# WPCLab/OpenSeg3D

Measured on AMD Instinct MI355X. Metric: points/sec fwd+bwd, Waymo 1-sweep ~180k pts @0.1m voxel; logit parity, higher is better.
Workload: dtype f32 storage/accumulate, bf16x3 products; 1 GPU; waymo_one_sweep (BASELINE configs[1]): synthetic scene, 174633 pts/step/GPU, voxel [0.1, 0.1, 0.1], grid [1440, 1440, 64], fwd (attention dropout p=0.1, DropPath) + criterion (ohem_ce+lovasz on 3 heads) + bwd + SGD step; mode=fwdbwd, segmentor=segformer, voxels=108690, parallelism=dp1

## Files before the change

### __graft_entry__.py

```python
import os
import subprocess
import sys

ROOT = os.path.dirname(os.path.abspath(__file__))
CSRC = os.path.join(ROOT, "openseg3d_amd", "csrc")
LIB = os.path.join(CSRC, "libseg3d_hip.so")
HIP_SOURCES = ["scan.hip", "voxelize.hip", "group.hip", "rulebook.hip", "spconv.hip", "spconv_split.hip", "linear_stream.hip", "linear_x6.hip", "spconv_dma.hip", "spconv_tile.hip", "wgrad_split.hip", "wgrad_dense.hip", "wgrad_dense_lds.hip", "window.hip",
               "attention.hip", "attention_fused.hip", "attention_fused_bwd.hip", "attention_small.hip", "rownorm.hip", "segment.hip", "knn.hip", "knn_attention.hip", "class_context.hip", "loss.hip", "lovasz.hip", "eval.hip"]
HIPCC_FLAGS = ["--offload-arch=gfx950", "-O3", "-std=c++17", "-fPIC", "-ffp-contract=off",
               "-fhip-fp32-correctly-rounded-divide-sqrt", "-Wall", "-Wno-unused-function"]


def _stale(target, deps):
    if not os.path.exists(target):
        return True
    t = os.path.getmtime(target)
    return any(os.path.getmtime(d) > t for d in deps)


def build_hip(force=False, verbose=False):
    hipcc = os.environ.get("HIPCC", "/opt/rocm/bin/hipcc")
    common = [os.path.join(CSRC, "common.hpp"), os.path.join(CSRC, "attn_common.hpp"), os.path.join(CSRC, "attn_dropout.hpp"), os.path.join(CSRC, "attn_fused.hpp"),
              os.path.join(ROOT, "include", "seg3d_hip.h")]
    objs = []
    procs = []
    for src in HIP_SOURCES:
        s = os.path.join(CSRC, src)
        o = os.path.join(CSRC, src.replace(".hip", ".o"))
        objs.append(o)
        if force or _stale(o, [s] + common):
            cmd = [hipcc] + HIPCC_FLAGS + ["-c", s, "-o", o]
            if verbose:
                print(" ".join(cmd))
            procs.append((src, subprocess.Popen(cmd, stdout=subprocess.PIPE, stderr=subprocess.STDOUT)))
    failed = False
    for src, p in procs:
        out, _ = p.communicate()
        if p.returncode != 0:
            failed = True
            sys.stderr.write(f"--- hipcc failed on {src}\n{out.decode()}\n")
        elif verbose and out.strip():
            print(out.decode())
    if failed:
        raise RuntimeError("hipcc failed")
    if force or procs or _stale(LIB, objs):
        subprocess.check_call([hipcc, "--offload-arch=gfx950", "-shared", "-fPIC", "-o", LIB] + objs)
    return LIB


def build():
    build_hip()
    subprocess.check_call(["make", "-C", os.path.join(ROOT, "oracle")], stdout=subprocess.DEVNULL)
    sys.path.insert(0, ROOT)
    import openseg3d_amd
    from openseg3d_amd import _lib
    _lib.load()


def smoke():
    sys.path.insert(0, ROOT)
    from openseg3d_amd import selfcheck
    selfcheck.run_smoke()


if __name__ == "__main__":
    build_hip(force="--force" in sys.argv, verbose=True)
```

### include/seg3d_hip.h

```cpp
#ifndef SEG3D_HIP_H
#define SEG3D_HIP_H

#include <stddef.h>
#include <stdint.h>

#ifdef __cplusplus
extern "C" {
#endif

#define SEG3D_OK 0
#define SEG3D_EINVAL (-1)
#define SEG3D_EWORKSPACE (-2)
#define SEG3D_ELAUNCH (-3)

#define SEG3D_REDUCE_SUM 0
#define SEG3D_REDUCE_MEAN 1
#define SEG3D_REDUCE_MAX 2

int seg3d_abi_version(void);

const char* seg3d_last_error(void);

int seg3d_grid_size(const float* voxel_size, const float* range, int32_t* grid_xyz);

size_t seg3d_voxelize_workspace_bytes(int64_t n_points);
int seg3d_voxelize_f32(const float* points, int64_t n_points, int32_t row_stride, int32_t xyz_col,
                       int32_t batch_col, const float* voxel_size, const float* range,
                       int32_t* voxel_coords, int32_t* point_voxel_ids, int32_t* n_voxels,
                       void* workspace, size_t workspace_bytes, void* stream);
int seg3d_voxelize_f64(const double* points, int64_t n_points, int32_t row_stride, int32_t xyz_col,
                       int32_t batch_col, const float* voxel_size, const float* range,
                       int32_t* voxel_coords, int32_t* point_voxel_ids, int32_t* n_voxels,
                       void* workspace, size_t workspace_bytes, void* stream);

size_t seg3d_voxelize_host_workspace_bytes(int64_t n_points);
int seg3d_voxelize_host_f32(const float* points, int64_t n_points, int32_t row_stride, int32_t xyz_col,
                            int32_t batch_col, const float* voxel_size, const float* range,
                            int32_t* voxel_coords, int32_t* point_voxel_ids, int32_t* n_voxels,
                            void* workspace, size_t workspace_bytes);
int seg3d_voxelize_host_f64(const double* points, int64_t n_points, int32_t row_stride, int32_t xyz_col,
                            int32_t batch_col, const float* voxel_size, const float* range,
                            int32_t* voxel_coords, int32_t* point_voxel_ids, int32_t* n_voxels,
                            void* workspace, size_t workspace_bytes);

int seg3d_cart2polar_f32(const float* points, int64_t n_points, int32_t row_stride, int32_t xyz_col,
                         float* out , void* stream);
int seg3d_cart2polar_f64(const double* points, int64_t n_points, int32_t row_stride, int32_t xyz_col,
                         double* out , void* stream);

size_t seg3d_group_index_workspace_bytes(int64_t n, int64_t n_groups);
int seg3d_group_index(const int32_t* group_ids, int64_t n, int64_t n_groups, int32_t* rank,
                      int32_t* order, int32_t* offsets, void* workspace, size_t workspace_bytes,
                      void* stream);

size_t seg3d_coord_hash_bytes(int64_t m);
int seg3d_coord_hash_build(const int32_t* coords, int64_t m, const int32_t* shape_zyx ,
                           void* table, size_t table_bytes, void* stream);
int seg3d_rulebook_subm(const int32_t* coords, int64_t m, const int32_t* shape_zyx ,
                        const void* table, size_t table_bytes, int32_t* nbr, void* stream);
size_t seg3d_downsample_workspace_bytes(int32_t batch_size, const int32_t* shape_in_zyx );
int seg3d_downsample_coords(const int32_t* coords_in, int64_t m_in,
                            const int32_t* m_in_dev ,
                            int32_t batch_size, const int32_t* shape_in_zyx , int32_t* coords_out,
                            int64_t cap_out, int32_t* m_out , void* workspace, size_t workspace_bytes,
                            void* stream);
int seg3d_rulebook_strided(const int32_t* coords_out, int64_t m_out, int64_t m_in,
                           const int32_t* shape_in_zyx , const void* table_in,
                           size_t table_bytes, int32_t* nbr_fwd, int32_t* nbr_inv, void* stream);

size_t seg3d_spconv_packed_bytes(int32_t cin, int32_t cout, int32_t flags);
int seg3d_spconv_pack_weight(const float* weight, int32_t cin, int32_t cout, int32_t flags,
                             void* w_packed, void* stream);
int seg3d_spconv_fwd(const float* x, const int32_t* nbr, int64_t m_out, int64_t m_in,
                     const void* w_packed, int32_t pack_flags, const float* bias ,
                     int32_t cin, int32_t cout, float* y,
                     const int32_t* row_order ,
                     void* stream);
int seg3d_spconv_fwd_act(const float* x, const int32_t* nbr, int64_t m_out, int64_t m_in, const void* w_packed,
                         int32_t pack_flags, const float* bias , const float* addend ,
                         int32_t relu, int32_t cin, int32_t cout, float* y, const int32_t* row_order ,
                         void* stream);
int seg3d_spconv_fwd_act_bf16(const void* x, int32_t x_bf16, const int32_t* nbr, int64_t m_out, int64_t m_in,
                              const void* w_packed, int32_t pack_flags, const float* bias,
                              const void* addend_bf16, int32_t relu, int32_t cin, int32_t cout, void* y_bf16,
                              const int32_t* row_order, void* stream);
size_t seg3d_spconv_presplit_bytes(int64_t m_in, int32_t cin);
int seg3d_spconv_presplit(const float* x, int64_t m_in, int32_t cin, void* xs, void* stream);
int seg3d_spconv_fwd_presplit(const void* xs, const int32_t* nbr, int64_t m_out, int64_t m_in, const void* w_packed,
                              int32_t pack_flags, const float* bias , const float* addend ,
                              int32_t relu, int32_t cin, int32_t cout, float* y,
                              const int32_t* row_order , void* stream);
size_t seg3d_conv_plan_bytes(int64_t m_out);
size_t seg3d_conv_plan_workspace_bytes(int64_t m_out);
int seg3d_conv_plan_build(const int32_t* coords, const int32_t* nbr, int64_t m_out, void* plan, void* workspace,
                          size_t workspace_bytes, void* stream);
int32_t seg3d_spconv_tiled_supported(int32_t cin, int32_t cout);
int seg3d_spconv_fwd_tiled(const float* x, const int32_t* nbr, const void* plan, int64_t m_out, int64_t m_in,
                           const void* w_packed, int32_t pack_flags, const float* bias ,
                           const float* addend , int32_t relu, int32_t cin, int32_t cout, float* y, void* stream);
int seg3d_spconv_fwd_tiled_bf16(const void* x, int32_t x_bf16, const int32_t* nbr, const void* plan, int64_t m_out,
                                int64_t m_in, const void* w_packed, int32_t pack_flags, const float* bias ,
                                const void* addend_bf16 , int32_t relu, int32_t cin, int32_t cout, void* y_bf16,
                                void* stream);
int seg3d_debug_set_conv_nbt(int32_t nbt);
int seg3d_debug_set_linear_stream(int32_t on);
size_t seg3d_spconv_wgrad_workspace_bytes(int64_t m_out, int32_t cin, int32_t cout);
int seg3d_spconv_wgrad(const float* x, const float* dy, const int32_t* nbr, int64_t m_out,
                       int64_t m_in, int32_t cin, int32_t cout, int32_t flags ,
                       float* dw, void* workspace, size_t workspace_bytes, void* stream);

int seg3d_spconv_wgrad_partials(const float* x, const float* dy, const int32_t* nbr, int64_t m_out, int64_t m_in,
                                int32_t cin, int32_t cout, void* workspace, size_t workspace_bytes, int32_t* chunks,
                                void* stream);
int seg3d_spconv_wgrad_partials_xbf16(const uint16_t* x_bf16, const float* dy, const int32_t* nbr, int64_t m_out,
                                      int64_t m_in, int32_t cin, int32_t cout, void* workspace, size_t workspace_bytes,
                                      int32_t* chunks, void* stream);

size_t seg3d_linear_wgrad_workspace_bytes(int64_t m, int32_t cin, int32_t cout);
int seg3d_linear_wgrad(const float* x, const float* dy, int64_t m, int32_t cin, int32_t cout, float* dw,
                       float* db , void* workspace, size_t workspace_bytes, void* stream);
int seg3d_linear_wgrad_partials(const float* x, const float* dy, int64_t m, int32_t cin, int32_t cout, int32_t with_bias,
                                void* workspace, size_t workspace_bytes, int32_t* chunks, void* stream);
int seg3d_linear_wgrad_partials_xbf16(const uint16_t* x_bf16, const float* dy, int64_t m, int32_t cin, int32_t cout,
                                      int32_t with_bias, void* workspace, size_t workspace_bytes, int32_t* chunks,
                                      void* stream);
int seg3d_debug_set_wgrad_lds(int32_t on);
int seg3d_reduce_partials(const float* part, int32_t chunks, int64_t n, int64_t nw, float* dw, float* db, void* stream);
int seg3d_reduce_partials_batched(const void* jobs, int32_t n_jobs, int64_t total_blocks, void* stream);
size_t seg3d_linear_packed_bytes_f32(int32_t cin, int32_t cout);
int seg3d_linear_pack_weight_f32(const float* weight, int32_t cin, int32_t cout, int32_t transpose,
                                 void* w_packed, void* stream);
int seg3d_linear_fwd_f32(const float* x, int64_t m, const void* w_packed, const float* bias ,
                         int32_t cin, int32_t cout, float* y, void* stream);
size_t seg3d_linear_packed_bytes_x6(int32_t cin, int32_t cout);
int seg3d_linear_pack_weight_x6(const float* weight, int32_t cin, int32_t cout, int32_t transpose, void* w_packed,
                                void* stream);
int seg3d_linear_fwd_x6(const float* x, int64_t m, const void* w_packed, const float* bias ,
                        const float* scale , const float* shift , int32_t relu, int32_t cin,
                        int32_t cout, float* y, void* stream);

typedef struct {
  const float* src;
  void* dst;
  int32_t cin, cout;
  int32_t kk, transpose, flip, reserved;
  int64_t first_block;
} seg3d_pack_job;
int seg3d_pack_weights_batched(const void* jobs, int32_t n_jobs, int64_t total_blocks, void* stream);

size_t seg3d_linear_packed_bytes(int32_t cin, int32_t cout, int32_t transpose);
int seg3d_linear_pack_weight(const float* weight, int32_t cin, int32_t cout, int32_t transpose,
                             void* w_packed, void* stream);
int seg3d_linear_fwd(const float* x, int64_t m, const void* w_packed, const float* bias ,
                     const float* addend , int32_t cin, int32_t cout,
                     float* y, void* stream);
int seg3d_linear_fwd_sum(const float* x, const float* x_add, int64_t m, const void* w_packed, const float* bias,
                         int32_t cin, int32_t cout, float* y, void* stream);
int seg3d_linear_layernorm_fwd(const float* x, int64_t m, const void* w_packed, const float* bias, const float* res,
                               const float* gamma, const float* beta, float eps, int32_t cin, int32_t cout, float* y,
                               void* stream);
int seg3d_linear_fwd_mul(const float* x, int64_t m, const void* w_packed, const float* factor, int32_t cin, int32_t cout,
                         float* y, void* stream);

size_t seg3d_window_partition_workspace_bytes(int64_t m, int32_t batch_size, const int32_t* nwin_xyz);
int seg3d_window_partition(const int32_t* coords, int64_t m, int32_t batch_size,
                           const int32_t* win_xyz, const int32_t* nwin_xyz, const int32_t* shift_xyz,
                           int32_t n_levels, const int32_t* level_lo, const int32_t* level_hi,
                           const int32_t* level_cap, int32_t* win_id, int32_t* in_win, int32_t* rank,
                           int32_t* level, int32_t* slot, int32_t* tok, int32_t* win_start,
                           int32_t* win_count, int32_t* win_tile0, int32_t* tile_item,
                           int32_t* qg_item, int32_t* counts, void* workspace,
                           size_t workspace_bytes, void* stream);

int seg3d_pos_embed(const int32_t* in_win, int64_t m, const int32_t* win_xyz ,
                    const float* inv_freq, int32_t c, float* pos, void* stream);

int seg3d_window_attn_supported(int32_t heads, int32_t dh);
size_t seg3d_window_attn_workspace_bytes(int64_t m, int32_t n_tiles, int32_t heads, int32_t dh);
int seg3d_window_attn_fwd(const float* q, const float* k, const float* v, int32_t ldq, int32_t ldk,
                          int32_t ldv, const int32_t* tok, const int32_t* win_start,
                          const int32_t* win_count, const int32_t* win_tile0,
                          const int32_t* tile_item, int32_t n_tiles, const int32_t* qg_item,
                          int32_t n_qgroups, int64_t m, int32_t n_windows, int32_t heads, int32_t dh,
                          const float* tau, float tau_min, float dropout_p, uint64_t dropout_seed, float* out,
                          float* lse, void* workspace, size_t workspace_bytes, void* stream);
int seg3d_window_attn_bwd(const float* q, const float* k, const float* v, int32_t ldq, int32_t ldk,
                          int32_t ldv, const float* out, const float* dout, const float* lse,
                          const int32_t* tok, const int32_t* win_start, const int32_t* win_count,
                          const int32_t* win_tile0, const int32_t* tile_item, int32_t n_tiles,
                          const int32_t* qg_item, int32_t n_qgroups, int64_t m, int32_t n_windows,
                          int32_t heads, int32_t dh, const float* tau,
                          float tau_min, float dropout_p, uint64_t dropout_seed, float* dq, float* dk,
                          float* dv, int32_t lddq, int32_t lddk,
                          int32_t lddv, float* dtau, void* workspace, size_t workspace_bytes,
                          void* stream);

int seg3d_layernorm_fwd(const float* x, const float* res, const float* gamma, const float* beta,
                        const float* rowscale, float eps, int64_t m, int32_t c, float* y, float* mean,
                        float* rstd, void* stream);
size_t seg3d_layernorm_bwd_workspace_bytes(int64_t m, int32_t c);
int seg3d_layernorm_bwd(const float* dy, const float* x, const float* mean, const float* rstd,
                        const float* gamma, const float* rowscale, int64_t m, int32_t c, float* dx,
                        float* dgamma, float* dbeta, void* workspace, size_t workspace_bytes, void* stream);
int seg3d_layernorm_bwd_partials(const float* dy, const float* x, const float* mean, const float* rstd,
                                 const float* gamma, const float* rowscale, int64_t m, int32_t c, float* dx,
                                 void* workspace, size_t workspace_bytes, int32_t* nblocks, void* stream);
size_t seg3d_batchnorm_workspace_bytes(int64_t m, int32_t c);
int seg3d_colstats(const float* x, int64_t m, int32_t c, float* sums, void* workspace, size_t workspace_bytes,
                   void* stream);
int seg3d_batchnorm_stats(const float* x, int64_t m, int32_t c, float eps, const float* gamma, const float* beta,
                          float momentum, float* running_mean, float* running_var, float* stats, void* workspace,
                          size_t workspace_bytes, void* stream);
int seg3d_gelu_fwd(const float* h, int64_t n, float* g, float* gp, void* stream);
int seg3d_affine_act(const float* x, const float* res, const float* scale, const float* shift, int32_t relu,
                     int64_t m, int32_t c, float* y, void* stream);
int seg3d_batchnorm_bwd(const float* dy, const float* y, const float* x, const float* mean, const float* rstd,
                        const float* gamma, int32_t relu, int64_t m, int32_t c, float* dx, float* dres,
                        float* sums, void* workspace, size_t workspace_bytes, void* stream);
int seg3d_batchnorm_bwd_reduce(const float* dy, const float* y, const float* x, const float* mean,
                               const float* rstd, int32_t relu, int64_t m, int32_t c, float* sums,
                               void* workspace, size_t workspace_bytes, void* stream);
int seg3d_batchnorm_bwd_apply(const float* dy, const float* y, const float* x, const float* mean,
                              const float* rstd, const float* gamma, const float* sums, const float* inv_count,
                              int32_t relu, int64_t m, int32_t c, float* dx, float* dres, void* stream);

int seg3d_segment_reduce_fwd(const float* x, int32_t c, const int32_t* order, const int32_t* offsets,
                             int64_t n_seg, int32_t mode, float* out, int32_t* argmax, void* stream);
int seg3d_segment_reduce_bwd(const float* dout, int32_t c, const int32_t* seg_of_row, int64_t n,
                             const int32_t* offsets, const int32_t* argmax, int64_t n_seg,
                             int32_t mode, float* dx, void* stream);

int seg3d_knn_attention_fwd(const float* q, const float* k, const float* v, const int32_t* idx,
                            const uint8_t* invalid, const float* keep, int64_t n, int64_t n_src,
                            int32_t n_neighbors, int32_t d, float scale, float* out, float* prob, void* stream);
int seg3d_knn_attention_bwd(const float* q, const float* k, const float* v, const int32_t* idx, const float* keep,
                            const float* prob, const float* dout, const int32_t* pair_order,
                            const int32_t* pair_offsets, int64_t n, int64_t n_src, int32_t n_neighbors, int32_t d,
                            float scale, float* dq, float* dk, float* dv, float* scratch, void* stream);

int seg3d_class_context_fwd(const float* feats, const float* probs, const int32_t* offsets, const int32_t* chunks,
                            const int32_t* chunk_offsets, int32_t n_chunks, int32_t batch, int64_t m,
                            int32_t classes, int32_t c, float scale, float* weights, float* partials, float* stats,
                            float* context, void* stream);
int seg3d_class_context_bwd(const float* feats, const float* weights, const float* dcontext,
                            const int32_t* offsets, const int32_t* chunks, const int32_t* chunk_offsets,
                            int32_t n_chunks, int32_t batch, int64_t m, int32_t classes, int32_t c, float scale,
                            float* dfeats, float* dprobs, float* scratch, void* stream);

int seg3d_gather_rows(const float* feats, const int32_t* ids, int64_t n, int32_t c, float* out,
                      void* stream);

int seg3d_knn_query(const float* xyz, int64_t n, const float* new_xyz, int64_t m, const int32_t* offset,
                    const int32_t* new_offset, int32_t batch_size, int32_t k, int32_t* idx, float* dist2,
                    void* stream);

size_t seg3d_knn_level_workspace_bytes(int64_t n);
int seg3d_knn_level_build(const float* xyz, int64_t n, const int32_t* offset, int32_t batch_size, float cell,
                          float* sorted_xyz, int32_t* src_index, int32_t* cell_end, void* table_keys, int32_t* table_vals,
                          int64_t capacity, void* workspace, size_t workspace_bytes, void* stream);
int seg3d_knn_query_order(const float* new_xyz, int64_t m, const int32_t* new_offset, int32_t batch_size, float cell,
                          int32_t* order, void* workspace, size_t workspace_bytes, void* stream);
int seg3d_parity_order(const int32_t* coords, int64_t m, int32_t* order, void* workspace, size_t workspace_bytes,
                       void* stream);
typedef struct {
  const float* sorted_xyz;
  const int32_t* src_index;
  const int32_t* cell_end;
  const void* table_keys;
  const int32_t* table_vals;
  int64_t capacity;
// ... 52 lines not shown
```

### openseg3d_amd/_lib.py

```python
import ctypes
import os
import re

_HERE = os.path.dirname(os.path.abspath(__file__))
LIB_PATH = os.path.join(_HERE, "csrc", "libseg3d_hip.so")
HEADER_PATH = os.path.join(os.path.dirname(_HERE), "include", "seg3d_hip.h")

OK, EINVAL, EWORKSPACE, ELAUNCH = 0, -1, -2, -3
REDUCE_SUM, REDUCE_MEAN, REDUCE_MAX = 0, 1, 2
ABI_VERSION = 41

_p, _i32, _i64, _sz, _f = ctypes.c_void_p, ctypes.c_int32, ctypes.c_int64, ctypes.c_size_t, ctypes.c_float
_u64 = ctypes.c_uint64

SIGNATURES = {
    "seg3d_abi_version": (ctypes.c_int, []),
    "seg3d_last_error": (ctypes.c_char_p, []),
    "seg3d_grid_size": (ctypes.c_int, [_p, _p, _p]),
    "seg3d_voxelize_workspace_bytes": (_sz, [_i64]),
    "seg3d_voxelize_f32": (ctypes.c_int, [_p, _i64, _i32, _i32, _i32, _p, _p, _p, _p, _p, _p, _sz, _p]),
    "seg3d_voxelize_f64": (ctypes.c_int, [_p, _i64, _i32, _i32, _i32, _p, _p, _p, _p, _p, _p, _sz, _p]),
    "seg3d_voxelize_host_workspace_bytes": (_sz, [_i64]),
    "seg3d_voxelize_host_f32": (ctypes.c_int, [_p, _i64, _i32, _i32, _i32, _p, _p, _p, _p, _p, _p, _sz]),
    "seg3d_voxelize_host_f64": (ctypes.c_int, [_p, _i64, _i32, _i32, _i32, _p, _p, _p, _p, _p, _p, _sz]),
    "seg3d_cart2polar_f32": (ctypes.c_int, [_p, _i64, _i32, _i32, _p, _p]),
    "seg3d_cart2polar_f64": (ctypes.c_int, [_p, _i64, _i32, _i32, _p, _p]),
    "seg3d_group_index_workspace_bytes": (_sz, [_i64, _i64]),
    "seg3d_group_index": (ctypes.c_int, [_p, _i64, _i64, _p, _p, _p, _p, _sz, _p]),
    "seg3d_coord_hash_bytes": (_sz, [_i64]),
    "seg3d_coord_hash_build": (ctypes.c_int, [_p, _i64, _p, _p, _sz, _p]),
    "seg3d_rulebook_subm": (ctypes.c_int, [_p, _i64, _p, _p, _sz, _p, _p]),
    "seg3d_downsample_workspace_bytes": (_sz, [_i32, _p]),
    "seg3d_downsample_coords": (ctypes.c_int, [_p, _i64, _p, _i32, _p, _p, _i64, _p, _p, _sz, _p]),
    "seg3d_rulebook_strided": (ctypes.c_int, [_p, _i64, _i64, _p, _p, _sz, _p, _p, _p]),
    "seg3d_spconv_packed_bytes": (_sz, [_i32, _i32, _i32]),
    "seg3d_spconv_pack_weight": (ctypes.c_int, [_p, _i32, _i32, _i32, _p, _p]),
    "seg3d_spconv_fwd": (ctypes.c_int, [_p, _p, _i64, _i64, _p, _i32, _p, _i32, _i32, _p, _p, _p]),
    "seg3d_spconv_fwd_act": (ctypes.c_int, [_p, _p, _i64, _i64, _p, _i32, _p, _p, _i32, _i32, _i32, _p, _p, _p]),
    "seg3d_spconv_fwd_act_bf16": (ctypes.c_int, [_p, _i32, _p, _i64, _i64, _p, _i32, _p, _p, _i32, _i32, _i32, _p, _p, _p]),
    "seg3d_spconv_presplit_bytes": (_sz, [_i64, _i32]),
    "seg3d_spconv_presplit": (ctypes.c_int, [_p, _i64, _i32, _p, _p]),
    "seg3d_spconv_fwd_presplit": (ctypes.c_int, [_p, _p, _i64, _i64, _p, _i32, _p, _p, _i32, _i32, _i32, _p, _p, _p]),
    "seg3d_conv_plan_bytes": (_sz, [_i64]),
    "seg3d_conv_plan_workspace_bytes": (_sz, [_i64]),
    "seg3d_conv_plan_build": (ctypes.c_int, [_p, _p, _i64, _p, _p, _sz, _p]),
    "seg3d_spconv_tiled_supported": (_i32, [_i32, _i32]),
    "seg3d_spconv_fwd_tiled": (ctypes.c_int, [_p, _p, _p, _i64, _i64, _p, _i32, _p, _p, _i32, _i32, _i32, _p, _p]),
    "seg3d_spconv_fwd_tiled_bf16": (ctypes.c_int, [_p, _i32, _p, _p, _i64, _i64, _p, _i32, _p, _p, _i32, _i32, _i32, _p, _p]),
    "seg3d_debug_set_conv_nbt": (ctypes.c_int, [_i32]),
    "seg3d_debug_set_linear_stream": (ctypes.c_int, [_i32]),
    "seg3d_spconv_wgrad_workspace_bytes": (_sz, [_i64, _i32, _i32]),
    "seg3d_spconv_wgrad": (ctypes.c_int, [_p, _p, _p, _i64, _i64, _i32, _i32, _i32, _p, _p, _sz, _p]),
    "seg3d_spconv_wgrad_partials": (ctypes.c_int, [_p, _p, _p, _i64, _i64, _i32, _i32, _p, _sz, _p, _p]),
    "seg3d_spconv_wgrad_partials_xbf16": (ctypes.c_int, [_p, _p, _p, _i64, _i64, _i32, _i32, _p, _sz, _p, _p]),
    "seg3d_linear_wgrad_partials_xbf16": (ctypes.c_int, [_p, _p, _i64, _i32, _i32, _i32, _p, ctypes.c_size_t, _p, _p]),
    "seg3d_linear_packed_bytes_f32": (ctypes.c_size_t, [_i32, _i32]),
    "seg3d_linear_pack_weight_f32": (ctypes.c_int, [_p, _i32, _i32, _i32, _p, _p]),
    "seg3d_linear_fwd_f32": (ctypes.c_int, [_p, _i64, _p, _p, _i32, _i32, _p, _p]),
    "seg3d_debug_set_wgrad_lds": (ctypes.c_int, [_i32]),
    "seg3d_linear_packed_bytes_x6": (ctypes.c_size_t, [_i32, _i32]),
    "seg3d_linear_pack_weight_x6": (ctypes.c_int, [_p, _i32, _i32, _i32, _p, _p]),
    "seg3d_linear_fwd_x6": (ctypes.c_int, [_p, _i64, _p, _p, _p, _p, _i32, _i32, _i32, _p, _p]),
    "seg3d_pack_weights_batched": (ctypes.c_int, [_p, _i32, _i64, _p]),
    "seg3d_linear_wgrad_workspace_bytes": (ctypes.c_size_t, [_i64, _i32, _i32]),
    "seg3d_linear_wgrad": (ctypes.c_int, [_p, _p, _i64, _i32, _i32, _p, _p, _p, ctypes.c_size_t, _p]),
    "seg3d_linear_wgrad_partials": (ctypes.c_int, [_p, _p, _i64, _i32, _i32, _i32, _p, ctypes.c_size_t, _p, _p]),
    "seg3d_reduce_partials": (ctypes.c_int, [_p, _i32, _i64, _i64, _p, _p, _p]),
    "seg3d_reduce_partials_batched": (ctypes.c_int, [_p, _i32, _i64, _p]),
    "seg3d_linear_packed_bytes": (_sz, [_i32, _i32, _i32]),
    "seg3d_linear_pack_weight": (ctypes.c_int, [_p, _i32, _i32, _i32, _p, _p]),
    "seg3d_linear_fwd": (ctypes.c_int, [_p, _i64, _p, _p, _p, _i32, _i32, _p, _p]),
    "seg3d_linear_fwd_sum": (ctypes.c_int, [_p, _p, _i64, _p, _p, _i32, _i32, _p, _p]),
    "seg3d_linear_fwd_mul": (ctypes.c_int, [_p, _i64, _p, _p, _i32, _i32, _p, _p]),
    "seg3d_linear_layernorm_fwd": (ctypes.c_int, [_p, _i64, _p, _p, _p, _p, _p, ctypes.c_float, _i32, _i32, _p, _p]),
    "seg3d_window_partition_workspace_bytes": (_sz, [_i64, _i32, _p]),
    "seg3d_window_partition": (ctypes.c_int, [_p, _i64, _i32, _p, _p, _p, _i32, _p, _p, _p,
                                              _p, _p, _p, _p, _p, _p, _p, _p, _p, _p, _p, _p, _p, _sz, _p]),
    "seg3d_pos_embed": (ctypes.c_int, [_p, _i64, _p, _p, _i32, _p, _p]),
    "seg3d_window_attn_supported": (ctypes.c_int, [_i32, _i32]),
    "seg3d_window_attn_workspace_bytes": (_sz, [_i64, _i32, _i32, _i32]),
    "seg3d_window_attn_fwd": (ctypes.c_int, [_p, _p, _p, _i32, _i32, _i32, _p, _p, _p, _p, _p, _i32, _p, _i32,
                                             _i64, _i32, _i32, _i32, _p, _f, _f, _u64, _p, _p, _p, _sz, _p]),
    "seg3d_window_attn_bwd": (ctypes.c_int, [_p, _p, _p, _i32, _i32, _i32, _p, _p, _p, _p, _p, _p, _p, _p, _i32, _p,
                                             _i32, _i64, _i32, _i32, _i32, _p, _f, _f, _u64, _p, _p, _p, _i32, _i32, _i32,
                                             _p, _p, _sz, _p]),
    "seg3d_layernorm_fwd": (ctypes.c_int, [_p, _p, _p, _p, _p, _f, _i64, _i32, _p, _p, _p, _p]),
    "seg3d_layernorm_bwd_workspace_bytes": (ctypes.c_size_t, [_i64, _i32]),
    "seg3d_layernorm_bwd": (ctypes.c_int, [_p, _p, _p, _p, _p, _p, _i64, _i32, _p, _p, _p, _p, ctypes.c_size_t, _p]),
    "seg3d_layernorm_bwd_partials": (ctypes.c_int, [_p, _p, _p, _p, _p, _p, _i64, _i32, _p, _p, ctypes.c_size_t, _p, _p]),
    "seg3d_batchnorm_workspace_bytes": (ctypes.c_size_t, [_i64, _i32]),
    "seg3d_colstats": (ctypes.c_int, [_p, _i64, _i32, _p, _p, ctypes.c_size_t, _p]),
    "seg3d_batchnorm_stats": (ctypes.c_int, [_p, _i64, _i32, _f, _p, _p, _f, _p, _p, _p, _p, ctypes.c_size_t, _p]),
    "seg3d_affine_act": (ctypes.c_int, [_p, _p, _p, _p, _i32, _i64, _i32, _p, _p]),
    "seg3d_gelu_fwd": (ctypes.c_int, [_p, _i64, _p, _p, _p]),
    "seg3d_batchnorm_bwd": (ctypes.c_int, [_p, _p, _p, _p, _p, _p, _i32, _i64, _i32, _p, _p, _p, _p, ctypes.c_size_t, _p]),
    "seg3d_batchnorm_bwd_reduce": (ctypes.c_int, [_p, _p, _p, _p, _p, _i32, _i64, _i32, _p, _p, ctypes.c_size_t, _p]),
    "seg3d_batchnorm_bwd_apply": (ctypes.c_int, [_p, _p, _p, _p, _p, _p, _p, _p, _i32, _i64, _i32, _p, _p, _p]),
    "seg3d_segment_reduce_fwd": (ctypes.c_int, [_p, _i32, _p, _p, _i64, _i32, _p, _p, _p]),
    "seg3d_segment_reduce_bwd": (ctypes.c_int, [_p, _i32, _p, _i64, _p, _p, _i64, _i32, _p, _p]),
    "seg3d_voxel_majority_labels": (ctypes.c_int, [_p, _p, _p, _i64, _i32, _p, _p]),
    "seg3d_cross_entropy_workspace_bytes": (ctypes.c_size_t, [_i64]),
    "seg3d_cross_entropy_fwd": (ctypes.c_int, [_p, _p, _i64, _i32, _i64, _f, _p, _p, _p, ctypes.c_size_t, _p]),
    "seg3d_cross_entropy_bwd": (ctypes.c_int, [_p, _p, _p, _p, _p, _i64, _i32, _p, _p]),
    "seg3d_lovasz_workspace_bytes": (ctypes.c_size_t, [_i64, _i32]),
    "seg3d_lovasz_softmax_fwd": (ctypes.c_int, [_p, _p, _i64, _i32, _i64, _i32, _p, _p, _p, _p, _p, ctypes.c_size_t, _p]),
    "seg3d_lovasz_softmax_bwd": (ctypes.c_int, [_p, _p, _p, _p, _i64, _i32, _p, _p]),
    "seg3d_knn_level_workspace_bytes": (ctypes.c_size_t, [_i64]),
    "seg3d_knn_level_build": (ctypes.c_int, [_p, _i64, _p, _i32, _f, _p, _p, _p, _p, _p, _i64, _p, ctypes.c_size_t, _p]),
    "seg3d_parity_order": (ctypes.c_int, [_p, _i64, _p, _p, ctypes.c_size_t, _p]),
    "seg3d_knn_query_order": (ctypes.c_int, [_p, _i64, _p, _i32, _f, _p, _p, ctypes.c_size_t, _p]),
    "seg3d_knn_grid_query": (ctypes.c_int, [_p, _i32, _p, _p, _i64, _p, _p, _i32, _i32, _p, _p, _p]),
    "seg3d_knn_query": (ctypes.c_int, [_p, _i64, _p, _i64, _p, _p, _i32, _i32, _p, _p, _p]),
    "seg3d_gather_rows": (ctypes.c_int, [_p, _p, _i64, _i32, _p, _p]),
    "seg3d_class_context_fwd": (ctypes.c_int, [_p, _p, _p, _p, _p, _i32, _i32, _i64, _i32, _i32, _f, _p, _p, _p, _p, _p]),
    "seg3d_class_context_bwd": (ctypes.c_int, [_p, _p, _p, _p, _p, _p, _i32, _i32, _i64, _i32, _i32, _f, _p, _p, _p, _p]),
    "seg3d_knn_attention_fwd": (ctypes.c_int, [_p, _p, _p, _p, _p, _p, _i64, _i64, _i32, _i32, _f, _p, _p, _p]),
    "seg3d_knn_attention_bwd": (ctypes.c_int, [_p, _p, _p, _p, _p, _p, _p, _p, _p, _i64, _i64, _i32, _i32, _f, _p, _p, _p, _p, _p]),
    "seg3d_tta_views_f32": (ctypes.c_int, [_p, _i64, _i32, _p, _p, _p]),
    "seg3d_tta_views_host_f32": (ctypes.c_int, [_p, _i64, _i32, _p, _p]),
    "seg3d_softmax_accumulate_f32": (ctypes.c_int, [_p, _i64, _i32, _i32, _i32, _p, _p]),
    "seg3d_argmax_confusion": (ctypes.c_int, [_p, _p, _i64, _i32, _i32, _p, _i32, _p, _p, _p]),
}

_ERR = {EINVAL: "SEG3D_EINVAL (bad argument)", EWORKSPACE: "SEG3D_EWORKSPACE (workspace too small)",
        ELAUNCH: "SEG3D_ELAUNCH (HIP launch/runtime error)"}

_lib = None


class Seg3dError(RuntimeError):
    pass


def header_symbols():
    with open(HEADER_PATH) as f:
        text = f.read()
    text = re.sub(r"/\*.*?\*/", "", text, flags=re.S)
    return sorted(set(re.findall(r"\b(seg3d_[a-z0-9_]+)\s*\(", text)))


def load():
    global _lib
    if _lib is not None:
        return _lib
    if not os.path.exists(LIB_PATH):
        raise Seg3dError(
            f"{LIB_PATH} not found: the HIP library is required (no CPU fallback). "
            "Build it with `python __graft_entry__.py`.")
    import torch
    lib = ctypes.CDLL(LIB_PATH)
    for name, (res, args) in SIGNATURES.items():
        fn = getattr(lib, name)
        fn.restype = res
        fn.argtypes = args
    if lib.seg3d_abi_version() != ABI_VERSION:
        raise Seg3dError(f"libseg3d_hip.so ABI {lib.seg3d_abi_version()} != binding {ABI_VERSION}")
    _lib = lib
    return lib


def call(name, *args):
    lib = load()
    rc = getattr(lib, name)(*args)
    if rc != OK:
        detail = ""
        if rc == ELAUNCH:
            text = lib.seg3d_last_error()
            detail = f": {text.decode(errors='replace')}" if text else ""
        raise Seg3dError(f"{name} failed: {_ERR.get(rc, rc)}{detail}")


def query(name, *args):
    return int(getattr(load(), name)(*args))
```

### openseg3d_amd/csrc/spconv.hip

```cpp
#include "common.hpp"

size_t spconv_split_packed_bytes(int cin_op, int cout_op, int kk);
int spconv_split_pack(const float* weight, int cin, int cout, int kk, int transpose, int flip, void* w_packed,
                      hipStream_t st);
int spconv_split_fwd_io(const void* x, const int32_t* nbr, int64_t m_out, const void* wp, const float* bias,
                        const void* addend, const int32_t* row_order, int cin, int cout, void* y, int relu, int io,
                        hipStream_t st, const float* x_add);
int spconv_split_fwd(const float* x, const int32_t* nbr, int64_t m_out, const void* wp, const float* bias,
                     const float* addend, const int32_t* row_order, int cin, int cout, float* y, int relu, hipStream_t st);
size_t wgrad_split_sparse_workspace_bytes(int64_t m_out, int cin, int cout);
int wgrad_split_sparse(const void* x, const float* dy, const int32_t* nbr, int64_t m_out, int cin, int cout, float* dw,
                       void* workspace, size_t workspace_bytes, hipStream_t st, int32_t* chunks_out, bool x_bf16);

namespace {

typedef float f32x4 __attribute__((ext_vector_type(4)));

constexpr int kWaves = 4;
constexpr int kThreads = kWaves * 64;
constexpr int kRowsPerWave = 16;
constexpr int kRowsPerBlock = kWaves * kRowsPerWave;

__global__ __launch_bounds__(256) void pack_weight(const float* __restrict__ w, int cin_src, int cout_src, int kk,
                                                   int transpose, int flip, float* __restrict__ wp) {
    const int64_t total = (int64_t)kk * cin_src * cout_src;
    const int64_t t = (int64_t)blockIdx.x * 256 + threadIdx.x;
    if (t >= total) return;
    const int cin_op = transpose ? cout_src : cin_src;
    const int cout_op = transpose ? cin_src : cout_src;
    const int cb_n = cin_op / 16, nb_n = cout_op / 16;
    int64_t r = t;
    const int j = (int)(r & 3); r >>= 2;
    const int lane = (int)(r & 63); r >>= 6;
    const int nb = (int)(r % nb_n); r /= nb_n;
    const int cb = (int)(r % cb_n); r /= cb_n;
    const int kp = (int)r;
    const int ci_op = cb * 16 + (lane >> 4) * 4 + j;
    const int co_op = nb * 16 + (lane & 15);
    const int k = flip ? kk - 1 - kp : kp;
    const int ci = transpose ? co_op : ci_op;
    const int co = transpose ? ci_op : co_op;
    wp[t] = w[((int64_t)co * kk + k) * cin_src + ci];
}

template <int NBT, bool DENSE>
__global__ __launch_bounds__(kThreads) void spconv_fwd_kernel(const float* __restrict__ x, const int32_t* __restrict__ nbr,
                                                              int64_t m_out, const float* __restrict__ wp,
                                                              const float* __restrict__ bias, int cin, int cout,
                                                              float* __restrict__ y) {
    const int lane = threadIdx.x & 63;
    const int wave = threadIdx.x >> 6;
    const int64_t row0 = (int64_t)blockIdx.x * kRowsPerBlock + wave * kRowsPerWave;
    if (row0 >= m_out) return;
    const int nb0 = blockIdx.y * NBT;
    const int cb_n = cin >> 4, nb_n = cout >> 4;
    const int64_t my_row = row0 + (lane & 15);
    const bool row_ok = my_row < m_out;
    const int64_t my_row_c = row_ok ? my_row : m_out - 1;

    f32x4 acc[NBT];
#pragma unroll
    for (int n = 0; n < NBT; ++n) {
        const float b = bias ? bias[(nb0 + n) * 16 + (lane & 15)] : 0.0f;
        acc[n] = (f32x4){b, b, b, b};
    }

    for (int k = 0; k < (DENSE ? 1 : 27); ++k) {
        const int32_t raw = DENSE ? (int32_t)my_row_c : nbr[(int64_t)k * m_out + my_row_c];
        const int32_t idx = row_ok ? raw : -1;
        if (__ballot(idx >= 0) == 0ull) continue;
        const float* xrow = x + (int64_t)(idx >= 0 ? idx : 0) * cin + (lane >> 4) * 4;
        const float* wk = wp + ((int64_t)k * cb_n * nb_n + nb0) * 256 + lane * 4;
        for (int cb = 0; cb < cb_n; ++cb) {
            const f32x4 ld = *reinterpret_cast<const f32x4*>(xrow + cb * 16);
            const f32x4 a = idx >= 0 ? ld : (f32x4){0.f, 0.f, 0.f, 0.f};
            f32x4 b[NBT];
#pragma unroll
            for (int n = 0; n < NBT; ++n)
                b[n] = *reinterpret_cast<const f32x4*>(wk + ((int64_t)cb * nb_n + n) * 256);
#pragma unroll
            for (int j = 0; j < 4; ++j) {
#pragma unroll
                for (int n = 0; n < NBT; ++n)
                    acc[n] = __builtin_amdgcn_mfma_f32_16x16x4f32(a[j], b[n][j], acc[n], 0, 0, 0);
            }
        }
    }

#pragma unroll
    for (int r = 0; r < 4; ++r) {
        const int64_t orow = row0 + (lane >> 4) * 4 + r;
        if (orow < m_out) {
            float* yr = y + orow * cout + nb0 * 16 + (lane & 15);
#pragma unroll
            for (int n = 0; n < NBT; ++n) yr[n * 16] = acc[n][r];
        }
    }
}

template <int NBT>
int launch_fwd(const float* x, const int32_t* nbr, int64_t m_out, const float* wp, const float* bias, int cin, int cout,
               float* y, hipStream_t st) {
    dim3 grid((unsigned)ceil_div64(m_out, kRowsPerBlock), (unsigned)((cout / 16) / NBT));
    if (nbr == nullptr)
        hipLaunchKernelGGL((spconv_fwd_kernel<NBT, true>), grid, dim3(kThreads), 0, st, x, nbr, m_out, wp, bias, cin, cout, y);
    else
        hipLaunchKernelGGL((spconv_fwd_kernel<NBT, false>), grid, dim3(kThreads), 0, st, x, nbr, m_out, wp, bias, cin, cout, y);
    SEG3D_CHECK_LAUNCH();
    return SEG3D_OK;
}

template <int J>
struct VecLoad;
template <>
struct VecLoad<1> {
    static __device__ __forceinline__ void load(const float* p, float* v) { v[0] = p[0]; }
};
template <>
struct VecLoad<2> {
    static __device__ __forceinline__ void load(const float* p, float* v) {
        const float2 t = *reinterpret_cast<const float2*>(p);
        v[0] = t.x; v[1] = t.y;
    }
};
template <>
struct VecLoad<3> {
    static __device__ __forceinline__ void load(const float* p, float* v) { v[0] = p[0]; v[1] = p[1]; v[2] = p[2]; }
};
template <>
struct VecLoad<4> {
    static __device__ __forceinline__ void load(const float* p, float* v) {
        const float4 t = *reinterpret_cast<const float4*>(p);
        v[0] = t.x; v[1] = t.y; v[2] = t.z; v[3] = t.w;
    }
};

constexpr int kWgradRowsPerWave = 512;

template <int JA, int JB>
__global__ __launch_bounds__(kThreads) void spconv_wgrad_kernel(const float* __restrict__ x, const float* __restrict__ dy,
                                                                const int32_t* __restrict__ nbr, int64_t m_out, int cin,
                                                                int cout, float* __restrict__ dw) {
    __shared__ int32_t pair_row[kWaves][64];
    __shared__ int32_t pair_in[kWaves][64];
    __shared__ float stage[kWaves][16 * JB * (16 * JA + 1)];
    const int lane = threadIdx.x & 63;
    const int wave = threadIdx.x >> 6;
    const int k = blockIdx.y;
    const int ca_n = cin / (16 * JA);
    const int ca = blockIdx.z % ca_n, cbk = blockIdx.z / ca_n;
    const int ci0 = ca * 16 * JA, co0 = cbk * 16 * JB;
    const int64_t r_begin = ((int64_t)blockIdx.x * kWaves + wave) * kWgradRowsPerWave;
    if (r_begin >= m_out) return;
    const int64_t r_end = r_begin + kWgradRowsPerWave < m_out ? r_begin + kWgradRowsPerWave : m_out;

    f32x4 acc[JA][JB];
#pragma unroll
    for (int a = 0; a < JA; ++a)
#pragma unroll
        for (int b = 0; b < JB; ++b) acc[a][b] = (f32x4){0.f, 0.f, 0.f, 0.f};

    const int32_t* nk = nbr + (int64_t)k * m_out;
    for (int64_t r0 = r_begin; r0 < r_end; r0 += 64) {
        const int64_t r = r0 + lane;
        const int32_t idx = r < r_end ? nk[r] : -1;
// ... 57 lines not shown

template <int JA, int JB>
int launch_wgrad(const float* x, const float* dy, const int32_t* nbr, int64_t m_out, int cin, int cout, float* dw,
                 hipStream_t st) {
    dim3 grid((unsigned)ceil_div64(m_out, (int64_t)kWaves * kWgradRowsPerWave), 27,
              (unsigned)((cin / (16 * JA)) * (cout / (16 * JB))));
    hipLaunchKernelGGL((spconv_wgrad_kernel<JA, JB>), grid, dim3(kThreads), 0, st, x, dy, nbr, m_out, cin, cout, dw);
    SEG3D_CHECK_LAUNCH();
    return SEG3D_OK;
}

template <int JA>
int launch_wgrad_b(int jb, const float* x, const float* dy, const int32_t* nbr, int64_t m_out, int cin, int cout,
                   float* dw, hipStream_t st) {
    switch (jb) {
        case 4: return launch_wgrad<JA, 4>(x, dy, nbr, m_out, cin, cout, dw, st);
        case 3: return launch_wgrad<JA, 3>(x, dy, nbr, m_out, cin, cout, dw, st);
        case 2: return launch_wgrad<JA, 2>(x, dy, nbr, m_out, cin, cout, dw, st);
        default: return launch_wgrad<JA, 1>(x, dy, nbr, m_out, cin, cout, dw, st);
    }
}

int dispatch_fwd_f32(const float* x, const int32_t* nbr, int64_t m_out, const float* w_packed, const float* bias, int cin,
                     int cout, float* y, hipStream_t st) {
    const int nb = cout / 16;
    if (nb % 12 == 0) return launch_fwd<12>(x, nbr, m_out, w_packed, bias, cin, cout, y, st);
    if (nb % 8 == 0) return launch_fwd<8>(x, nbr, m_out, w_packed, bias, cin, cout, y, st);
    if (nb % 6 == 0) return launch_fwd<6>(x, nbr, m_out, w_packed, bias, cin, cout, y, st);
    if (nb % 4 == 0) return launch_fwd<4>(x, nbr, m_out, w_packed, bias, cin, cout, y, st);
    if (nb % 3 == 0) return launch_fwd<3>(x, nbr, m_out, w_packed, bias, cin, cout, y, st);
    if (nb % 2 == 0) return launch_fwd<2>(x, nbr, m_out, w_packed, bias, cin, cout, y, st);
    return launch_fwd<1>(x, nbr, m_out, w_packed, bias, cin, cout, y, st);
}

}

extern "C" {

size_t seg3d_spconv_packed_bytes(int32_t cin, int32_t cout, int32_t flags) {
    if (cin <= 0 || cout <= 0) return 0;
    const int cin_op = (flags & 1) ? cout : cin, cout_op = (flags & 1) ? cin : cout;
    if (flags & 4) return spconv_split_packed_bytes(cin_op, cout_op, 27);
    return (size_t)27 * cin * cout * sizeof(float);
}

int seg3d_spconv_pack_weight(const float* weight, int32_t cin, int32_t cout, int32_t flags, void* w_packed,
                             void* stream) {
    if (!weight || !w_packed || cin <= 0 || cout <= 0 || (cin & 15) || (cout & 15)) return SEG3D_EINVAL;
    hipStream_t st = as_stream(stream);
    if (flags & 4) return spconv_split_pack(weight, cin, cout, 27, flags & 1, (flags >> 1) & 1, w_packed, st);
    const int64_t total = (int64_t)27 * cin * cout;
    hipLaunchKernelGGL(pack_weight, dim3((unsigned)ceil_div64(total, 256)), dim3(256), 0, st, weight, cin, cout, 27,
                       flags & 1, (flags >> 1) & 1, static_cast<float*>(w_packed));
    SEG3D_CHECK_LAUNCH();
    return SEG3D_OK;
}

int seg3d_spconv_fwd(const float* x, const int32_t* nbr, int64_t m_out, int64_t m_in, const void* w_packed_v,
                     int32_t pack_flags, const float* bias, int32_t cin, int32_t cout, float* y, const int32_t* row_order,
                     void* stream) {
    if (m_out < 0 || m_in < 0 || cin <= 0 || cout <= 0 || (cin & 15) || (cout & 15) || !w_packed_v) return SEG3D_EINVAL;
    if (m_out == 0) return SEG3D_OK;
    if (!x || !nbr || !y) return SEG3D_EINVAL;
    hipStream_t st = as_stream(stream);
    if (pack_flags & 4) return spconv_split_fwd(x, nbr, m_out, w_packed_v, bias, nullptr, row_order, cin, cout, y, 0, st);
    return dispatch_fwd_f32(x, nbr, m_out, static_cast<const float*>(w_packed_v), bias, cin, cout, y, st);
}

int seg3d_spconv_fwd_act(const float* x, const int32_t* nbr, int64_t m_out, int64_t m_in, const void* w_packed_v,
                         int32_t pack_flags, const float* bias, const float* addend, int32_t relu, int32_t cin,
                         int32_t cout, float* y, const int32_t* row_order, void* stream) {
    if (m_out < 0 || m_in < 0 || cin <= 0 || cout <= 0 || (cin & 15) || (cout & 15) || !w_packed_v || !(pack_flags & 4))
        return SEG3D_EINVAL;
    if (m_out == 0) return SEG3D_OK;
    if (!x || !nbr || !y) return SEG3D_EINVAL;
    return spconv_split_fwd(x, nbr, m_out, w_packed_v, bias, addend, row_order, cin, cout, y, relu ? 1 : 0, as_stream(stream));
}

int seg3d_spconv_fwd_act_bf16(const void* x, int32_t x_bf16, const int32_t* nbr, int64_t m_out, int64_t m_in,
                              const void* w_packed_v, int32_t pack_flags, const float* bias, const void* addend_bf16,
                              int32_t relu, int32_t cin, int32_t cout, void* y_bf16, const int32_t* row_order,
                              void* stream) {
    if (m_out < 0 || m_in < 0 || cin <= 0 || cout <= 0 || (cin & 15) || (cout & 15) || !w_packed_v || !(pack_flags & 4))
        return SEG3D_EINVAL;
    if (m_out == 0) return SEG3D_OK;
    if (!x || !nbr || !y_bf16) return SEG3D_EINVAL;
    return spconv_split_fwd_io(x, nbr, m_out, w_packed_v, bias, addend_bf16, row_order, cin, cout, y_bf16, relu ? 1 : 0,
                               x_bf16 ? 2 : 1, as_stream(stream), nullptr);
}

size_t seg3d_linear_packed_bytes_f32(int32_t cin, int32_t cout) {
    return cin > 0 && cout > 0 ? (size_t)cin * cout * sizeof(float) : 0;
}

int seg3d_linear_pack_weight_f32(const float* weight, int32_t cin, int32_t cout, int32_t transpose, void* w_packed,
                                 void* stream) {
    if (!weight || !w_packed || cin <= 0 || cout <= 0 || (cin & 15) || (cout & 15)) return SEG3D_EINVAL;
    const int64_t total = (int64_t)cin * cout;
    hipLaunchKernelGGL(pack_weight, dim3((unsigned)ceil_div64(total, 256)), dim3(256), 0, as_stream(stream), weight, cin,
                       cout, 1, transpose ? 1 : 0, 0, static_cast<float*>(w_packed));
    SEG3D_CHECK_LAUNCH();
    return SEG3D_OK;
}

int seg3d_linear_fwd_f32(const float* x, int64_t m, const void* w_packed, const float* bias, int32_t cin, int32_t cout,
                         float* y, void* stream) {
    if (m < 0 || cin <= 0 || cout <= 0 || (cin & 15) || (cout & 15) || !w_packed) return SEG3D_EINVAL;
    if (m == 0) return SEG3D_OK;
    if (!x || !y) return SEG3D_EINVAL;
    return dispatch_fwd_f32(x, nullptr, m, static_cast<const float*>(w_packed), bias, cin, cout, y, as_stream(stream));
}

size_t seg3d_spconv_wgrad_workspace_bytes(int64_t m_out, int32_t cin, int32_t cout) {
    if (m_out < 0 || cin <= 0 || cout <= 0) return 0;
    return wgrad_split_sparse_workspace_bytes(m_out, cin, cout);
}

int seg3d_spconv_wgrad(const float* x, const float* dy, const int32_t* nbr, int64_t m_out, int64_t m_in, int32_t cin,
                       int32_t cout, int32_t flags, float* dw, void* workspace, size_t workspace_bytes, void* stream) {
    if (m_out < 0 || m_in < 0 || cin <= 0 || cout <= 0 || (cin & 15) || (cout & 15) || !dw) return SEG3D_EINVAL;
    hipStream_t st = as_stream(stream);
    if (m_out > 0 && (!x || !dy || !nbr)) return SEG3D_EINVAL;
    if (m_out > 0 && (flags & 4)) return wgrad_split_sparse(x, dy, nbr, m_out, cin, cout, dw, workspace, workspace_bytes, st, nullptr, false);
    SEG3D_CHECK_HIP(hipMemsetAsync(dw, 0, (size_t)27 * cin * cout * sizeof(float), st));
    if (m_out == 0) return SEG3D_OK;
    const int ja = pick_j(cin), jb = pick_j(cout);
    switch (ja) {
        case 4: return launch_wgrad_b<4>(jb, x, dy, nbr, m_out, cin, cout, dw, st);
        case 3: return launch_wgrad_b<3>(jb, x, dy, nbr, m_out, cin, cout, dw, st);
        case 2: return launch_wgrad_b<2>(jb, x, dy, nbr, m_out, cin, cout, dw, st);
        default: return launch_wgrad_b<1>(jb, x, dy, nbr, m_out, cin, cout, dw, st);
    }
}

int seg3d_spconv_wgrad_partials(const float* x, const float* dy, const int32_t* nbr, int64_t m_out, int64_t m_in, int32_t cin,
                                int32_t cout, void* workspace, size_t workspace_bytes, int32_t* chunks, void* stream) {
    if (m_out < 0 || m_in < 0 || cin <= 0 || cout <= 0 || (cin & 15) || (cout & 15) || !chunks) return SEG3D_EINVAL;
    *chunks = 0;
    if (m_out == 0) return SEG3D_OK;
    if (!x || !dy || !nbr) return SEG3D_EINVAL;
    return wgrad_split_sparse(x, dy, nbr, m_out, cin, cout, nullptr, workspace, workspace_bytes, as_stream(stream), chunks, false);
}

int seg3d_spconv_wgrad_partials_xbf16(const uint16_t* x_bf16, const float* dy, const int32_t* nbr, int64_t m_out, int64_t m_in,
                                      int32_t cin, int32_t cout, void* workspace, size_t workspace_bytes, int32_t* chunks,
                                      void* stream) {
    if (m_out < 0 || m_in < 0 || cin <= 0 || cout <= 0 || (cin & 15) || (cout & 15) || !chunks) return SEG3D_EINVAL;
    *chunks = 0;
    if (m_out == 0) return SEG3D_OK;
    if (!x_bf16 || !dy || !nbr) return SEG3D_EINVAL;
    return wgrad_split_sparse(x_bf16, dy, nbr, m_out, cin, cout, nullptr, workspace, workspace_bytes, as_stream(stream), chunks, true);
}

}
```

### openseg3d_amd/csrc/voxelize.hip

```cpp
#include <cstdio>

#include "common.hpp"

namespace {

constexpr int kThreads = 256;

struct VoxParams {
    int32_t grid[3];
    int32_t row_stride, xyz_col, batch_col;
};

template <typename T>
struct VoxConst {
    T lo[3];
    T vs[3];
};

__device__ __forceinline__ float floor_t(float v) { return floorf(v); }
__device__ __forceinline__ double floor_t(double v) { return floor(v); }

template <typename T>
__global__ __launch_bounds__(kThreads) void vox_insert(const T* __restrict__ pts, int64_t n, VoxParams p,
                                                       VoxConst<T> c, HashView h, uint32_t* __restrict__ slot_of) {
// ... 97 lines not shown
                  int32_t* n_voxels, void* workspace, size_t workspace_bytes, void* stream) {
    if (n < 0 || n >= (int64_t)0x7F000000 || !voxel_size || !range || !voxel_coords || !n_voxels || !workspace ||
        row_stride < 3 || xyz_col < 0 || xyz_col + 3 > row_stride || batch_col >= row_stride)
        return SEG3D_EINVAL;
    if (n > 0 && (!points || !point_voxel_ids)) return SEG3D_EINVAL;
    if (workspace_bytes < ws_bytes(n)) return SEG3D_EWORKSPACE;
    hipStream_t st = as_stream(stream);
    VoxParams p;
    if (seg3d_grid_size(voxel_size, range, p.grid) != SEG3D_OK) return SEG3D_EINVAL;
    p.row_stride = row_stride;
    p.xyz_col = xyz_col;
    p.batch_col = batch_col;
    VoxConst<T> c;
    for (int j = 0; j < 3; ++j) {
        c.lo[j] = (T)range[j];
        c.vs[j] = (T)voxel_size[j];
    }
    VoxWs w = carve(workspace, n);
    HashView h = hash_view(w.table, w.cap);
    SEG3D_CHECK_HIP(hipMemsetAsync(h.keys, 0xFF, w.cap * 8, st));
    SEG3D_CHECK_HIP(hipMemsetAsync(h.vals, 0x7F, w.cap * 4, st));
    if (n == 0) {
        SEG3D_CHECK_HIP(hipMemsetAsync(n_voxels, 0, 4, st));
        return SEG3D_OK;
    }
    const unsigned nb = (unsigned)ceil_div64(n, kThreads);
    hipLaunchKernelGGL(vox_insert<T>, dim3(nb), dim3(kThreads), 0, st, points, n, p, c, h, w.slot_of);
    SEG3D_CHECK_LAUNCH();
    hipLaunchKernelGGL(vox_flag, dim3(nb), dim3(kThreads), 0, st, w.slot_of, n, h, w.flag);
    SEG3D_CHECK_LAUNCH();
    int rc = scan_exclusive_u32(w.flag, w.rank, n, reinterpret_cast<uint32_t*>(n_voxels), w.tmp, st);
    if (rc != SEG3D_OK) return rc;
    hipLaunchKernelGGL(vox_emit, dim3(nb), dim3(kThreads), 0, st, w.slot_of, w.rank, n, h, p, voxel_coords,
                       point_voxel_ids);
    SEG3D_CHECK_LAUNCH();
    return SEG3D_OK;
}

__device__ __forceinline__ float atan2_t(float y, float x) { return (float)atan2((double)y, (double)x); }
__device__ __forceinline__ double atan2_t(double y, double x) { return atan2(y, x); }
__device__ __forceinline__ float sqrt_t(float v) { return sqrtf(v); }
__device__ __forceinline__ double sqrt_t(double v) { return sqrt(v); }

template <typename T>
__global__ __launch_bounds__(kThreads) void cart2polar_rows(const T* __restrict__ pts, int64_t n, int row_stride, int xyz_col,
                                                            T* __restrict__ out) {
    const int64_t i = (int64_t)blockIdx.x * kThreads + threadIdx.x;
    if (i >= n) return;
    const T* row = pts + i * row_stride;
    T* o = out + i * (row_stride + 2);
    for (int j = 0; j < xyz_col; ++j) o[j] = row[j];
    const T x = row[xyz_col], y = row[xyz_col + 1], z = row[xyz_col + 2];
    o[xyz_col] = sqrt_t(x * x + y * y);
    o[xyz_col + 1] = atan2_t(y, x);
    o[xyz_col + 2] = z;
    o[xyz_col + 3] = x;
    o[xyz_col + 4] = y;
    for (int j = xyz_col + 3; j < row_stride; ++j) o[j + 2] = row[j];
}

template <typename T>
int cart2polar_impl(const T* points, int64_t n, int32_t row_stride, int32_t xyz_col, T* out, void* stream) {
    if (n < 0 || row_stride < 3 || xyz_col < 0 || xyz_col + 3 > row_stride) return SEG3D_EINVAL;
    if (n == 0) return SEG3D_OK;
    if (!points || !out) return SEG3D_EINVAL;
    hipLaunchKernelGGL(cart2polar_rows<T>, dim3((unsigned)ceil_div64(n, kThreads)), dim3(kThreads), 0, as_stream(stream), points, n,
                       row_stride, xyz_col, out);
    SEG3D_CHECK_LAUNCH();
    return SEG3D_OK;
}


inline float floor_h(float v) { return __builtin_floorf(v); }
inline double floor_h(double v) { return __builtin_floor(v); }

inline uint64_t host_capacity(int64_t n) {
    uint64_t cap = 64;
    while (cap < (uint64_t)(2 * n + 2)) cap <<= 1;
    return cap;
}

template <typename T>
int voxelize_host_impl(const T* points, int64_t n, int32_t row_stride, int32_t xyz_col, int32_t batch_col,
                       const float* voxel_size, const float* range, int32_t* voxel_coords, int32_t* point_voxel_ids,
                       int32_t* n_voxels, void* workspace, size_t workspace_bytes) {
    if (n < 0 || n >= (int64_t)0x7F000000 || !voxel_size || !range || !n_voxels || row_stride < 3 || xyz_col < 0 ||
        xyz_col + 3 > row_stride || batch_col >= row_stride)
        return SEG3D_EINVAL;
    if (n > 0 && (!points || !point_voxel_ids || !voxel_coords || !workspace)) return SEG3D_EINVAL;
    const uint64_t cap = host_capacity(n);
    if (n > 0 && workspace_bytes < cap * 12) return SEG3D_EWORKSPACE;
    int32_t grid[3];
    if (seg3d_grid_size(voxel_size, range, grid) != SEG3D_OK) return SEG3D_EINVAL;
    *n_voxels = 0;
    if (n == 0) return SEG3D_OK;
    uint64_t* keys = static_cast<uint64_t*>(workspace);
    int32_t* vals = reinterpret_cast<int32_t*>(keys + cap);
    for (uint64_t s = 0; s < cap; ++s) keys[s] = ~0ull;
    T lo[3], vs[3];
    for (int j = 0; j < 3; ++j) {
        lo[j] = (T)range[j];
        vs[j] = (T)voxel_size[j];
    }
    int32_t count = 0;
    for (int64_t i = 0; i < n; ++i) {
        const T* row = points + i * row_stride;
        int32_t cc[3];
        bool ok = true;
        for (int j = 0; j < 3 && ok; ++j) {
            volatile T d = row[xyz_col + j] - lo[j];
            volatile T q = d / vs[j];
            const T v = floor_h((T)q);
            if (!(v >= (T)0) || v >= (T)grid[j]) ok = false;
            else cc[j] = (int32_t)v;
        }
        if (!ok) {
            point_voxel_ids[i] = -1;
            continue;
        }
        const int64_t b = batch_col >= 0 ? (int64_t)row[batch_col] : 0;
        const uint64_t key = (uint64_t)(((b * grid[2] + cc[2]) * grid[1] + cc[1]) * (int64_t)grid[0] + cc[0]);
        uint64_t h = key * 0x9E3779B97F4A7C15ull;
        uint64_t s = (h ^ (h >> 29)) & (cap - 1);
        while (keys[s] != key && keys[s] != ~0ull) s = (s + 1) & (cap - 1);
        if (keys[s] == ~0ull) {
            keys[s] = key;
            vals[s] = count;
            int32_t* o = voxel_coords + 4 * (int64_t)count;
            o[0] = (int32_t)b;
            o[1] = cc[2];
            o[2] = cc[1];
            o[3] = cc[0];
            ++count;
        }
        point_voxel_ids[i] = vals[s];
    }
    *n_voxels = count;
    return SEG3D_OK;
}

}

extern "C" {

int seg3d_cart2polar_f32(const float* points, int64_t n_points, int32_t row_stride, int32_t xyz_col, float* out, void* stream) {
    return cart2polar_impl<float>(points, n_points, row_stride, xyz_col, out, stream);
}

int seg3d_cart2polar_f64(const double* points, int64_t n_points, int32_t row_stride, int32_t xyz_col, double* out,
                         void* stream) {
    return cart2polar_impl<double>(points, n_points, row_stride, xyz_col, out, stream);
}

int seg3d_abi_version(void) { return 41; }

namespace {
thread_local char g_last_error[320] = "";
}

const char* seg3d_last_error(void) { return g_last_error; }

int seg3d_grid_size(const float* voxel_size, const float* range, int32_t* grid_xyz) {
    if (!voxel_size || !range || !grid_xyz) return SEG3D_EINVAL;
    for (int j = 0; j < 3; ++j) {
        volatile float span = range[3 + j] - range[j];
        volatile float g = span / voxel_size[j];
        grid_xyz[j] = (int32_t)__builtin_rintf(g);
        if (grid_xyz[j] <= 0) return SEG3D_EINVAL;
    }
    return SEG3D_OK;
}

size_t seg3d_voxelize_workspace_bytes(int64_t n_points) { return ws_bytes(n_points < 0 ? 0 : n_points); }

int seg3d_voxelize_f32(const float* points, int64_t n_points, int32_t row_stride, int32_t xyz_col, int32_t batch_col,
                       const float* voxel_size, const float* range, int32_t* voxel_coords, int32_t* point_voxel_ids,
                       int32_t* n_voxels, void* workspace, size_t workspace_bytes, void* stream) {
    return voxelize_impl<float>(points, n_points, row_stride, xyz_col, batch_col, voxel_size, range, voxel_coords,
                                point_voxel_ids, n_voxels, workspace, workspace_bytes, stream);
}

int seg3d_voxelize_f64(const double* points, int64_t n_points, int32_t row_stride, int32_t xyz_col, int32_t batch_col,
                       const float* voxel_size, const float* range, int32_t* voxel_coords, int32_t* point_voxel_ids,
                       int32_t* n_voxels, void* workspace, size_t workspace_bytes, void* stream) {
    return voxelize_impl<double>(points, n_points, row_stride, xyz_col, batch_col, voxel_size, range, voxel_coords,
                                 point_voxel_ids, n_voxels, workspace, workspace_bytes, stream);
}

size_t seg3d_voxelize_host_workspace_bytes(int64_t n_points) { return (size_t)host_capacity(n_points < 0 ? 0 : n_points) * 12; }

int seg3d_voxelize_host_f32(const float* points, int64_t n_points, int32_t row_stride, int32_t xyz_col, int32_t batch_col,
                            const float* voxel_size, const float* range, int32_t* voxel_coords, int32_t* point_voxel_ids,
                            int32_t* n_voxels, void* workspace, size_t workspace_bytes) {
    return voxelize_host_impl<float>(points, n_points, row_stride, xyz_col, batch_col, voxel_size, range, voxel_coords,
                                     point_voxel_ids, n_voxels, workspace, workspace_bytes);
}

int seg3d_voxelize_host_f64(const double* points, int64_t n_points, int32_t row_stride, int32_t xyz_col, int32_t batch_col,
                            const float* voxel_size, const float* range, int32_t* voxel_coords, int32_t* point_voxel_ids,
                            int32_t* n_voxels, void* workspace, size_t workspace_bytes) {
    return voxelize_host_impl<double>(points, n_points, row_stride, xyz_col, batch_col, voxel_size, range, voxel_coords,
                                      point_voxel_ids, n_voxels, workspace, workspace_bytes);
}

}

void seg3d_note_hip_error(int code, const char* file, int line) {
    const char* base = file;
    for (const char* p = file; *p; ++p)
        if (*p == '/') base = p + 1;
    snprintf(g_last_error, sizeof(g_last_error), "%s (%s) at %s:%d", hipGetErrorString((hipError_t)code),
             hipGetErrorName((hipError_t)code), base, line);
}
```

### openseg3d_amd/csrc/wgrad_split.hip

```cpp
#include <cstdlib>

#include "attn_common.hpp"

int wgrad_chunk_reduce(const float* part, int chunks, int64_t n, int64_t nw, float* dw, float* db, hipStream_t st);

#ifdef SEG3D_WGRAD_STAMP
__device__ unsigned long long* g_wgrad_stamp_buf = nullptr;
extern "C" int seg3d_debug_wgrad_stamps(void* buf) {
    unsigned long long* p = static_cast<unsigned long long*>(buf);
    return hipMemcpyToSymbol(HIP_SYMBOL(g_wgrad_stamp_buf), &p, sizeof(p)) == hipSuccess ? 0 : 2;
}
#define WSTAMP(i)                                                    \
    do {                                                             \
        __builtin_amdgcn_sched_barrier(0);                           \
        const unsigned long long t_ = __builtin_amdgcn_s_memtime();  \
        __builtin_amdgcn_sched_barrier(0);                           \
        st_acc[i] += t_ - st_last;                                   \
        st_last = t_;                                                \
    } while (0)
#else
#define WSTAMP(i) do {} while (0)
#endif

namespace {

using namespace attn;

constexpr int kWaves = 4;
constexpr int kThreads = 64 * kWaves;
constexpr int kRing = 128;

__device__ __forceinline__ bf16x8 frag_from_bf16_rows(const uint2* q, int comp) {
    u32x4 h;
#pragma unroll
    for (int j = 0; j < 4; ++j) {
        const uint32_t a = (comp & 2) ? q[2 * j].y : q[2 * j].x, b = (comp & 2) ? q[2 * j + 1].y : q[2 * j + 1].x;
        h[j] = (comp & 1) ? ((a >> 16) | (b & 0xFFFF0000u)) : ((a & 0xFFFFu) | (b << 16));
    }
    return __builtin_bit_cast(bf16x8, h);
}

__device__ __forceinline__ f32x4 mfma2(const bf16x8& a_hi, const bf16x8& a_lo, const bf16x8& b, f32x4 acc) {
    acc = __builtin_amdgcn_mfma_f32_16x16x32_bf16(a_lo, b, acc, 0, 0, 0);
    acc = __builtin_amdgcn_mfma_f32_16x16x32_bf16(a_hi, b, acc, 0, 0, 0);
    return acc;
}

struct Plan {
    int nbo, nbi;
    int chunks;
    int64_t rows;
};

__device__ __forceinline__ void unit_to_chunk_offset(int unit, int n_chunks, int* chunk, int* k) {
    if (unit < n_chunks) {
        *chunk = unit;
        *k = 13;
    } else {
        const int u = unit - n_chunks;
        const int kk = u % 26;
        *chunk = u / 26;
        *k = kk + (kk >= 13 ? 1 : 0);
    }
}

Plan plan(int64_t m, int cin, int cout) {
    Plan p{(cout + 63) / 64, (cin + 63) / 64, 0, 64};
    if (m <= 0) return p;
    const int tiles = p.nbo * p.nbi;
    static const int rows_target = [] {
        const char* e = getenv("SEG3D_WGRAD_SPARSE_ROWS");
        const int v = e ? atoi(e) : 3072;
        return v >= 64 ? v : 3072;
    }();
    int64_t chunks = m / rows_target;
    const int64_t need = (1024 + 27 * tiles - 1) / (27 * tiles);
    if (chunks < need) chunks = need;
    if (chunks < 1) chunks = 1;
    int64_t rows = (m + chunks - 1) / chunks;
    rows = (rows + 63) / 64 * 64;
    p.rows = rows;
    p.chunks = (int)((m + rows - 1) / rows);
    return p;
}

template <bool XB>
__global__ __launch_bounds__(kThreads, 2) void wgrad_sparse_kernel(const void* __restrict__ x_v, const float* __restrict__ dy,
                                                                    const int32_t* __restrict__ nbr, int64_t m_rows,
                                                                    int cin, int cout, int rows_per_chunk, int nbi,
                                                                    int tiles, int units, float* __restrict__ part,
                                                                    int center_first) {
    const float* x = static_cast<const float*>(x_v);
    __shared__ __attribute__((aligned(16))) float red[64 * 64];
    __shared__ int2 ring[kWaves][kRing];
    const int lane = threadIdx.x & 63, wave = threadIdx.x >> 6;
    const int cq = lane & 15, rg = lane >> 4;
    const int xcd = blockIdx.x & 7, j = blockIdx.x >> 3;
    const int xb = (center_first >> 8) > 0 ? (center_first >> 8) : 1;
    const int qs = j / tiles, tile = j % tiles;
    const int unit = ((qs / xb) * 8 + xcd) * xb + qs % xb;
    if (unit >= units) return;
    int chunk = unit / 27, k = unit % 27;
    if (center_first & 1) unit_to_chunk_offset(unit, units / 27, &chunk, &k);
    const int bi = tile % nbi, bo = tile / nbi;
    const int ci0 = bi * 64, co0 = bo * 64;
    const int64_t r_begin = (int64_t)chunk * rows_per_chunk;
    const int64_t r_end = r_begin + rows_per_chunk < m_rows ? r_begin + rows_per_chunk : m_rows;
    const int32_t* nk = nbr + (int64_t)k * m_rows;
    const float* px = x + (ci0 + 4 * cq < cin ? ci0 + 4 * cq : 0);
    const uint16_t* pxb = static_cast<const uint16_t*>(x_v) + (ci0 + 4 * cq < cin ? ci0 + 4 * cq : 0);
    const float* py = dy + (co0 + 4 * cq < cout ? co0 + 4 * cq : 0);
    int2* my = ring[wave];

    f32x4 acc[4][4];
#pragma unroll
    for (int a = 0; a < 4; ++a)
#pragma unroll
        for (int b = 0; b < 4; ++b) acc[a][b] = (f32x4){0.f, 0.f, 0.f, 0.f};

    constexpr int kAhead = 4;
    int head = 0, tail = 0;
    int64_t g_row = r_begin + 64 * (int64_t)wave;
    int32_t idxq[kAhead];
#pragma unroll
    for (int j = 0; j < kAhead; ++j) {
        const int64_t r = g_row + (int64_t)j * 64 * kWaves + lane;
        idxq[j] = r < r_end ? nk[r] : -1;
    }
    auto scan_group = [&]() {
        const int32_t idx = idxq[0];
        const int64_t row = g_row + lane;
        g_row += 64 * kWaves;
#pragma unroll
        for (int j = 0; j + 1 < kAhead; ++j) idxq[j] = idxq[j + 1];
        const int64_t rn = g_row + (int64_t)(kAhead - 1) * 64 * kWaves + lane;
        idxq[kAhead - 1] = rn < r_end ? nk[rn] : -1;
        const unsigned long long mask = __ballot(idx >= 0);
        if (idx >= 0) {
            const int p = tail + __popcll(mask & ((1ull << lane) - 1ull));
            my[p & (kRing - 1)] = make_int2(idx, (int)row);
        }
        tail += __popcll(mask);
    };
    auto refill = [&]() {
        while (tail - head < 32 && g_row < r_end) scan_group();
        __builtin_amdgcn_wave_barrier();
    };

    f32x4 xr[XB ? 1 : 8], yr[8];
    uint2 xq[XB ? 8 : 1];
    bf16x8 b_hi[4], b_lo[XB ? 1 : 4];
    auto load_x = [&](int h0, int valid) {
#pragma unroll
        for (int i = 0; i < 8; ++i) {
            const int e = 8 * rg + i;
            const int2 p = my[(h0 + (e < valid ? e : 0)) & (kRing - 1)];
            if constexpr (XB) xq[i] = *reinterpret_cast<const uint2*>(pxb + (int64_t)p.x * cin);
            else xr[i] = *reinterpret_cast<const f32x4*>(px + (int64_t)p.x * cin);
        }
        if (valid < 32) {
#pragma unroll
            for (int i = 0; i < 8; ++i)
                if (8 * rg + i >= valid) {
                    if constexpr (XB) xq[i] = make_uint2(0u, 0u);
                    else xr[i] = (f32x4){0.f, 0.f, 0.f, 0.f};
                }
        }
    };
    auto load_y = [&](int h0, int valid) {
#pragma unroll
        for (int i = 0; i < 8; ++i) {
            const int e = 8 * rg + i;
            const int2 p = my[(h0 + (e < valid ? e : 0)) & (kRing - 1)];
            yr[i] = *reinterpret_cast<const f32x4*>(py + (int64_t)p.y * cout);
        }
        if (valid < 32) {
#pragma unroll
            for (int i = 0; i < 8; ++i)
                if (8 * rg + i >= valid) yr[i] = (f32x4){0.f, 0.f, 0.f, 0.f};
        }
    };
    auto make_b = [&]() {
#pragma unroll
        for (int b = 0; b < 4; ++b) {
            if constexpr (XB) {
                b_hi[b] = frag_from_bf16_rows(xq, b);
            } else {
                float v[8];
#pragma unroll
                for (int i = 0; i < 8; ++i) v[i] = xr[i][b];
                split_frag(v, &b_hi[b], &b_lo[b]);
            }
        }
    };
    auto multiply = [&]() {
#pragma unroll
        for (int a = 0; a < 4; ++a) {
            float v[8];
#pragma unroll
            for (int i = 0; i < 8; ++i) v[i] = yr[i][a];
            bf16x8 a_hi, a_lo;
            split_frag(v, &a_hi, &a_lo);
#pragma unroll
            for (int b = 0; b < 4; ++b) {
                if constexpr (XB) acc[a][b] = mfma2(a_hi, a_lo, b_hi[b], acc[a][b]);
                else acc[a][b] = mfma3(a_hi, a_lo, b_hi[b], b_lo[b], acc[a][b]);
            }
        }
    };

    refill();
    int valid = tail - head < 32 ? tail - head : 32;
    if (valid > 0) {
        load_x(head, valid);
        load_y(head, valid);
    }
    while (valid > 0) {
        head += valid;
        refill();
        const int next = tail - head < 32 ? tail - head : 32;
        make_b();
        if (next > 0) load_x(head, next);
        multiply();
        if (next > 0) load_y(head, next);
        valid = next;
    }

    for (int w = 0; w < kWaves; ++w) {
        if (wave == w) {
#pragma unroll
            for (int a = 0; a < 4; ++a)
#pragma unroll
                for (int r = 0; r < 4; ++r) {
                    f32x4* slot = reinterpret_cast<f32x4*>(&red[(4 * (4 * rg + r) + a) * 64 + 4 * cq]);
                    f32x4 v = {acc[a][0][r], acc[a][1][r], acc[a][2][r], acc[a][3][r]};
                    if (w > 0) v += *slot;
                    *slot = v;
                }
        }
        __syncthreads();
    }
    float* pw = part + (int64_t)chunk * ((int64_t)cout * 27 * cin);
    for (int e = threadIdx.x; e < 64 * 16; e += kThreads) {
        const int row = e >> 4, q = e & 15;
        const int co = co0 + row, ci = ci0 + 4 * q;
        if (co < cout && ci < cin)
            *reinterpret_cast<f32x4*>(pw + ((int64_t)co * 27 + k) * cin + ci) =
                *reinterpret_cast<const f32x4*>(&red[row * 64 + 4 * q]);
    }
}

constexpr int kRing2 = 512;

template <bool XB, int DEPTH, bool SB = false>
__global__ __launch_bounds__(kThreads, SB ? 3 : 2) void wgrad_sparse_wide_kernel(const void* __restrict__ x_v, const float* __restrict__ dy,
                                                                         const int32_t* __restrict__ nbr, int64_t m_rows,
                                                                         int cin, int cout, int rows_per_chunk, int nbi,
                                                                         int tiles, int units, float* __restrict__ part,
                                                                         int center_first) {
    const float* x = static_cast<const float*>(x_v);
    __shared__ __attribute__((aligned(16))) uint4 img[SB ? 1 : 2][4][2][4][64];
    __shared__ int2 ring[kRing2];
    __shared__ int wave_cnt[2][kWaves];
    const int lane = threadIdx.x & 63, wave = threadIdx.x >> 6;
    const int cq = lane & 15, rg = lane >> 4;
    const int wa = wave >> 1, wb = wave & 1;
    const int xcd = blockIdx.x & 7, j = blockIdx.x >> 3;
    const int xb = (center_first >> 8) > 0 ? (center_first >> 8) : 1;
    const int qs = j / tiles, tile = j % tiles;
    const int unit = ((qs / xb) * 8 + xcd) * xb + qs % xb;
    if (unit >= units) return;
    int chunk = unit / 27, k = unit % 27;
    if (center_first & 1) unit_to_chunk_offset(unit, units / 27, &chunk, &k);
    const int bi = tile % nbi, bo = tile / nbi;
    const int ci0 = bi * 128, co0 = bo * 128;
    const int64_t r_begin = (int64_t)chunk * rows_per_chunk;
    const int64_t r_end = r_begin + rows_per_chunk < m_rows ? r_begin + rows_per_chunk : m_rows;
    const int32_t* nk = nbr + (int64_t)k * m_rows;
    const bool stage_dy = wave < 2;
    const int ld = stage_dy ? cout : cin;
    const int ch = (stage_dy ? co0 : ci0) + 64 * (wave & 1) + 4 * cq;
    const float* src = (stage_dy ? dy : x) + (ch < ld ? ch : 0);
    const uint16_t* srcb = static_cast<const uint16_t*>(x_v) + (ch < ld ? ch : 0);

    f32x4 acc[4][4];
#pragma unroll
    for (int a = 0; a < 4; ++a)
#pragma unroll
        for (int b = 0; b < 4; ++b) acc[a][b] = (f32x4){0.f, 0.f, 0.f, 0.f};

    int head = 0, tail = 0, round = 0;
    int64_t g_row = r_begin;
    int32_t idx_n1 = g_row + 64 * wave + lane < r_end ? nk[g_row + 64 * wave + lane] : -1;
    int32_t idx_n2 = g_row + 64 * (kWaves + wave) + lane < r_end ? nk[g_row + 64 * (kWaves + wave) + lane] : -1;
    auto scan_round = [&]() {
        const int64_t row = g_row + 64 * wave + lane;
        const int32_t idx = idx_n1;
        idx_n1 = idx_n2;
        {
            const int64_t rn = row + 2 * 64 * kWaves;
            idx_n2 = rn < r_end ? nk[rn] : -1;
        }
        const unsigned long long mask = __ballot(idx >= 0);
        const int mine = __popcll(mask);
        int* cnt = wave_cnt[round & 1];
        if (lane == 0) cnt[wave] = mine;
        __syncthreads();
        int before = 0, total = 0;
#pragma unroll
        for (int w = 0; w < kWaves; ++w) {
            const int c = cnt[w];
            before += w < wave ? c : 0;
            total += c;
        }
        if (idx >= 0) {
            const int p = tail + before + __popcll(mask & ((1ull << lane) - 1ull));
            ring[p & (kRing2 - 1)] = make_int2(idx, (int)row);
        }
        tail += total;
        g_row += 64 * kWaves;
        ++round;
    };
    auto refill = [&]() {
        while (tail - head < 32 && g_row < r_end) scan_round();
        __syncthreads();
    };

    f32x4 raw[8], raw2[DEPTH == 2 ? 8 : 1];
    uint2 rawb[XB ? 8 : 1], rawb2[(XB && DEPTH == 2) ? 8 : 1];
    auto load_into = [&](f32x4* r, uint2* rb, int h0, int valid) {
        int32_t rows[8];
#pragma unroll
        for (int i = 0; i < 8; ++i) {
            const int e = 8 * rg + i;
            const int2 p = ring[(h0 + (e < valid ? e : 0)) & (kRing2 - 1)];
            rows[i] = stage_dy ? p.y : p.x;
        }
        if (XB && !stage_dy) {
            if constexpr (XB) {
#pragma unroll
                for (int i = 0; i < 8; ++i) rb[i] = *reinterpret_cast<const uint2*>(srcb + (int64_t)rows[i] * ld);
                if (valid < 32) {
#pragma unroll
                    for (int i = 0; i < 8; ++i)
                        if (8 * rg + i >= valid) rb[i] = make_uint2(0u, 0u);
                }
            }
        } else {
#pragma unroll
            for (int i = 0; i < 8; ++i) r[i] = *reinterpret_cast<const f32x4*>(src + (int64_t)rows[i] * ld);
            if (valid < 32) {
#pragma unroll
                for (int i = 0; i < 8; ++i)
                    if (8 * rg + i >= valid) r[i] = (f32x4){0.f, 0.f, 0.f, 0.f};
            }
        }
    };
    auto stash_from = [&](const f32x4* r, const uint2* rb, int buf) {
        if (XB && !stage_dy) {
            if constexpr (XB) {
#pragma unroll
                for (int jj = 0; jj < 4; ++jj)
                    img[buf][wave][0][rg][jj * 16 + cq] = __builtin_bit_cast(uint4, frag_from_bf16_rows(rb, jj));
            }
            return;
        }
#pragma unroll
        for (int jj = 0; jj < 4; ++jj) {
            float v[8];
#pragma unroll
            for (int i = 0; i < 8; ++i) v[i] = r[i][jj];
            bf16x8 hi, lo;
            split_frag(v, &hi, &lo);
            img[buf][wave][0][rg][jj * 16 + cq] = __builtin_bit_cast(uint4, hi);
            img[buf][wave][1][rg][jj * 16 + cq] = __builtin_bit_cast(uint4, lo);
        }
    };
    auto load_slab = [&](int h0, int valid) { load_into(raw, rawb, h0, valid); };
    auto stash = [&](int buf) { stash_from(raw, rawb, buf); };
    auto multiply = [&](int buf) {
        bf16x8 b_hi[4], b_lo[XB ? 1 : 4];
#pragma unroll
        for (int b = 0; b < 4; ++b) {
            b_hi[b] = __builtin_bit_cast(bf16x8, img[buf][2 + wb][0][rg][b * 16 + cq]);
            if constexpr (!XB) b_lo[b] = __builtin_bit_cast(bf16x8, img[buf][2 + wb][1][rg][b * 16 + cq]);
        }
#pragma unroll
        for (int a = 0; a < 4; ++a) {
            const bf16x8 a_hi = __builtin_bit_cast(bf16x8, img[buf][wa][0][rg][a * 16 + cq]);
            const bf16x8 a_lo = __builtin_bit_cast(bf16x8, img[buf][wa][1][rg][a * 16 + cq]);
#pragma unroll
            for (int b = 0; b < 4; ++b) {
                if constexpr (XB) acc[a][b] = mfma2(a_hi, a_lo, b_hi[b], acc[a][b]);
                else acc[a][b] = mfma3(a_hi, a_lo, b_hi[b], b_lo[b], acc[a][b]);
            }
        }
    };

    int buf = 0;
#ifdef SEG3D_WGRAD_STAMP
    unsigned long long st_acc[8] = {0, 0, 0, 0, 0, 0, 0, 0};
    unsigned long long st_last = __builtin_amdgcn_s_memtime();
    const unsigned long long st_begin = st_last;
#endif
    if constexpr (DEPTH == 1) {
        refill();
        int valid = tail - head < 32 ? tail - head : 32;
        if (valid > 0) {
            load_slab(head, valid);
            stash(0);
        }
        WSTAMP(7);
        while (valid > 0) {
            head += valid;
            refill();
            WSTAMP(0);
            const int next = tail - head < 32 ? tail - head : 32;
            if (next > 0) load_slab(head, next);
            WSTAMP(1);
            multiply(buf);
            WSTAMP(2);
            if constexpr (SB) {
                __syncthreads();
                if (next > 0) stash(0);
            } else {
                if (next > 0) stash(buf ^ 1);
                buf ^= 1;
            }
            WSTAMP(3);
            valid = next;
#ifdef SEG3D_WGRAD_STAMP
            st_acc[5] += 1;
#endif
        }
    } else {
        auto fetch = [&](f32x4* r, uint2* rb) {
            refill();
            const int v = tail - head < 32 ? tail - head : 32;
            if (v > 0) load_into(r, rb, head, v);
            head += v;
            return v;
        };
        int va = fetch(raw, rawb);
        int vb = va > 0 ? fetch(raw2, rawb2) : 0;
        if (va > 0) stash_from(raw, rawb, 0);
        while (va > 0) {
            va = vb > 0 ? fetch(raw, rawb) : (refill(), 0);
            multiply(buf);
            if (vb > 0) stash_from(raw2, rawb2, buf ^ 1);
            buf ^= 1;
            if (vb == 0) break;
            vb = va > 0 ? fetch(raw2, rawb2) : (refill(), 0);
            multiply(buf);
            if (va > 0) stash_from(raw, rawb, buf ^ 1);
            buf ^= 1;
        }
    }
    __syncthreads();

    if constexpr (SB) {
        float* pw = part + (int64_t)chunk * ((int64_t)cout * 27 * cin);
#pragma unroll
        for (int a = 0; a < 4; ++a)
#pragma unroll
            for (int r = 0; r < 4; ++r) {
                const int co = co0 + 64 * wa + 4 * (4 * rg + r) + a, ci = ci0 + 64 * wb + 4 * cq;
                if (co < cout && ci < cin)
                    *reinterpret_cast<f32x4*>(pw + ((int64_t)co * 27 + k) * cin + ci) =
                        (f32x4){acc[a][0][r], acc[a][1][r], acc[a][2][r], acc[a][3][r]};
            }
        return;
    }
    float* st = reinterpret_cast<float*>(&img[0][0][0][0][0]) + wave * 4096;
#pragma unroll
    for (int a = 0; a < 4; ++a)
#pragma unroll
        for (int r = 0; r < 4; ++r)
            *reinterpret_cast<f32x4*>(&st[(4 * (4 * rg + r) + a) * 64 + 4 * cq]) =
                (f32x4){acc[a][0][r], acc[a][1][r], acc[a][2][r], acc[a][3][r]};
    __builtin_amdgcn_wave_barrier();
    float* pw = part + (int64_t)chunk * ((int64_t)cout * 27 * cin);
    for (int e = lane; e < 64 * 16; e += 64) {
        const int row = e >> 4, q = e & 15;
        const int co = co0 + 64 * wa + row, ci = ci0 + 64 * wb + 4 * q;
        if (co < cout && ci < cin)
            *reinterpret_cast<f32x4*>(pw + ((int64_t)co * 27 + k) * cin + ci) =
                *reinterpret_cast<const f32x4*>(&st[row * 64 + 4 * q]);
    }
#ifdef SEG3D_WGRAD_STAMP
    if constexpr (DEPTH == 1) {
        asm volatile("s_waitcnt vmcnt(0)" ::: "memory");
        WSTAMP(4);
        if (g_wgrad_stamp_buf && lane == 0) {
            st_acc[6] = __builtin_amdgcn_s_memtime() - st_begin;
            unsigned long long* o = g_wgrad_stamp_buf + (k == 13 ? 8 : 0);
            for (int i = 0; i < 8; ++i) atomicAdd(o + i, st_acc[i]);
            atomicAdd(g_wgrad_stamp_buf + 16 + (k == 13 ? 1 : 0), 1ull);
        }
    }
#endif
}

}

size_t wgrad_split_sparse_workspace_bytes(int64_t m_out, int cin, int cout) {
    const Plan p = plan(m_out, cin, cout);
    return ((size_t)p.chunks * 27 * (size_t)cin * cout + 64) * sizeof(float);
}

int wgrad_split_sparse(const void* x, const float* dy, const int32_t* nbr, int64_t m_out, int cin, int cout, float* dw,
                       void* workspace, size_t workspace_bytes, hipStream_t st, int32_t* chunks_out, bool x_bf16) {
    if (workspace_bytes < wgrad_split_sparse_workspace_bytes(m_out, cin, cout) || !workspace) return SEG3D_EINVAL;
    const Plan p = plan(m_out, cin, cout);
    float* part = static_cast<float*>(workspace);
    const int units = p.chunks * 27;
    static const bool narrow_only = getenv("SEG3D_WGRAD_NARROW") != nullptr;
    static const int center_first = [] {
        const char* e = getenv("SEG3D_WGRAD_CENTER_FIRST");
        const int cf = (e && atoi(e) == 0) ? 0 : 1;
        const char* b = getenv("SEG3D_WGRAD_XCD_BLOCK");
        int xb = b ? atoi(b) : 1;
        if (xb < 1 || xb > 64) xb = 1;
        return cf | (xb << 8);
    }();
    const int xcd_block = center_first >> 8;
    const int unit_slots = (units + 8 * xcd_block - 1) / (8 * xcd_block) * (8 * xcd_block);
    const bool fits128 = ((cin + 127) / 128) * 2 == (cin + 63) / 64 && ((cout + 127) / 128) * 2 == (cout + 63) / 64;
    static const int wide_min = [] {
        const char* e = getenv("SEG3D_WGRAD_WIDE_MIN");
        return e ? atoi(e) : 0;
    }();
    const int cmin = cin < cout ? cin : cout, cmax = cin < cout ? cout : cin;
    const bool wide_padded = (wide_min > 0 && cmin >= wide_min) || (cin != cout && cmin >= 96 && cmax >= 192);
    if ((fits128 || wide_padded) && !narrow_only) {
        const int nbo = (cout + 127) / 128, nbi = (cin + 127) / 128, tiles = nbo * nbi;
        const unsigned blocks = (unsigned)unit_slots * (unsigned)tiles;
        static const int depth = [] {
            const char* e = getenv("SEG3D_WGRAD_DEPTH");
            const int v = e ? atoi(e) : 1;
            return v == 2 ? 2 : 1;
        }();
#define SEG3D_LAUNCH_WIDE(XB_, D_)                                                                                             \
    hipLaunchKernelGGL((wgrad_sparse_wide_kernel<XB_, D_>), dim3(blocks), dim3(kThreads), 0, st, x, dy, nbr, m_out, cin, cout, \
                       (int)p.rows, nbi, tiles, units, part, center_first)
        static const bool single = [] {
            const char* e = getenv("SEG3D_WGRAD_SB");
            return !(e && atoi(e) == 0);
        }();
#define SEG3D_LAUNCH_WIDE_SB(XB_)                                                                                                   \
    hipLaunchKernelGGL((wgrad_sparse_wide_kernel<XB_, 1, true>), dim3(blocks), dim3(kThreads), 0, st, x, dy, nbr, m_out, cin, cout, \
                       (int)p.rows, nbi, tiles, units, part, center_first)
        if (single && depth == 1) {
            if (x_bf16) SEG3D_LAUNCH_WIDE_SB(true);
            else SEG3D_LAUNCH_WIDE_SB(false);
        } else if (x_bf16) {
            SEG3D_LAUNCH_WIDE(true, 1);
        } else {
            if (depth == 2) SEG3D_LAUNCH_WIDE(false, 2);
            else SEG3D_LAUNCH_WIDE(false, 1);
        }
#undef SEG3D_LAUNCH_WIDE_SB
#undef SEG3D_LAUNCH_WIDE
    } else {
        const int tiles = p.nbo * p.nbi;
        const unsigned blocks = (unsigned)unit_slots * (unsigned)tiles;
        if (x_bf16)
            hipLaunchKernelGGL(wgrad_sparse_kernel<true>, dim3(blocks), dim3(kThreads), 0, st, x, dy, nbr, m_out, cin, cout,
                               (int)p.rows, p.nbi, tiles, units, part, center_first);
        else
            hipLaunchKernelGGL(wgrad_sparse_kernel<false>, dim3(blocks), dim3(kThreads), 0, st, x, dy, nbr, m_out, cin, cout,
                               (int)p.rows, p.nbi, tiles, units, part, center_first);
    }
    SEG3D_CHECK_LAUNCH();
    if (chunks_out) *chunks_out = p.chunks;
    if (!dw) return SEG3D_OK;
    const int64_t n = (int64_t)27 * cin * cout;
    return wgrad_chunk_reduce(part, p.chunks, n, n, dw, nullptr, st);
}
```

### openseg3d_amd/ops.py

```python
import ctypes
import weakref
import os

import numpy as np
import torch

from . import _lib
from ._lib import REDUCE_MAX, REDUCE_MEAN, REDUCE_SUM

_F3 = ctypes.c_float * 3
_F6 = ctypes.c_float * 6
_I3 = ctypes.c_int32 * 3


def _need_gpu(*tensors):
    for t in tensors:
        if t is not None and not t.is_cuda:
            raise _lib.Seg3dError("openseg3d_amd ops run on the GPU only (no CPU fallback); got a CPU tensor")


def _ptr(t):
    return None if t is None else ctypes.c_void_p(t.data_ptr())


# ... 297 lines not shown
            ok = all(a is not None and torch.equal(a, b) for a, b in zip(got, want))
    except Exception as e:
        ok = False
        import warnings
        warnings.warn(f"openseg3d_amd: deferred weight-gradient join probe raised {type(e).__name__}: {e}")
    pr["ok"] = bool(ok)
    if not ok:
        WGRAD_DEFER = False
        import warnings
        warnings.warn("openseg3d_amd: the deferred weight-gradient join did not reproduce the joined gradients on this "
                      "torch build; falling back to per-function joins (SEG3D_WGRAD_DEFER=0)")
    return pr["ok"]


def _i3(v):
    return _I3(*[int(x) for x in v])


def _f32c(t):
    return t.contiguous() if t.dtype == torch.float32 else t.float().contiguous()


def _i32c(t):
    return t.contiguous() if t.dtype == torch.int32 else t.to(torch.int32).contiguous()


def grid_size(voxel_size, point_cloud_range):
    out = _I3()
    _lib.call("seg3d_grid_size", _F3(*[float(v) for v in voxel_size]),
              _F6(*[float(v) for v in point_cloud_range]), out)
    return [int(v) for v in out]


def voxelize(points, voxel_size, point_cloud_range, xyz_col=0, batch_col=-1):
    _need_gpu(points)
    if points.dim() != 2 or points.dtype not in (torch.float32, torch.float64):
        raise _lib.Seg3dError("points must be a float32/float64 [N, D] tensor")
    points = points.contiguous()
    n, d = points.shape
    dev = points.device
    coords = torch.empty((max(n, 1), 4), dtype=torch.int32, device=dev)
    ids = torch.empty((n,), dtype=torch.int32, device=dev)
    count = torch.zeros((1,), dtype=torch.int32, device=dev)
    nbytes = _lib.query("seg3d_voxelize_workspace_bytes", n)
    ws = _workspace(nbytes, dev)
    fn = "seg3d_voxelize_f32" if points.dtype == torch.float32 else "seg3d_voxelize_f64"
    _lib.call(fn, _ptr(points), n, d, int(xyz_col), int(batch_col), _F3(*[float(v) for v in voxel_size]),
              _F6(*[float(v) for v in point_cloud_range]), _ptr(coords), _ptr(ids), _ptr(count), _ptr(ws),
              ws.numel(), _stream())
    m = int(count.item())
    return coords[:m], ids


def voxelize_host(points, voxel_size, point_cloud_range, xyz_col=0, batch_col=-1):
    import numpy as np
    pts = np.ascontiguousarray(points)
    if pts.ndim != 2 or pts.dtype not in (np.float32, np.float64):
        raise _lib.Seg3dError("points must be a float32/float64 [N, D] array")
    n, d = pts.shape
    coords = np.empty((max(n, 1), 4), dtype=np.int32)
    ids = np.empty((n,), dtype=np.int32)
    count = np.zeros((1,), dtype=np.int32)
    ws = np.empty((max(int(_lib.query("seg3d_voxelize_host_workspace_bytes", n)), 8),), dtype=np.uint8)

    def host(a):
        return ctypes.c_void_p(a.ctypes.data)

    fn = "seg3d_voxelize_host_f32" if pts.dtype == np.float32 else "seg3d_voxelize_host_f64"
    _lib.call(fn, host(pts), n, d, int(xyz_col), int(batch_col), _F3(*[float(v) for v in voxel_size]),
              _F6(*[float(v) for v in point_cloud_range]), host(coords), host(ids), host(count), host(ws), ws.size)
    return coords[: int(count[0])], ids


def cart2polar(points, xyz_col=0):
    _need_gpu(points)
    if points.dim() != 2 or points.dtype not in (torch.float32, torch.float64):
        raise _lib.Seg3dError("points must be a float32/float64 [N, D] tensor")
    points = points.contiguous()
    n, d = points.shape
    out = torch.empty((n, d + 2), dtype=points.dtype, device=points.device)
    fn = "seg3d_cart2polar_f32" if points.dtype == torch.float32 else "seg3d_cart2polar_f64"
    _lib.call(fn, _ptr(points), n, d, int(xyz_col), _ptr(out), _stream())
    return out


def group_index(group_ids, n_groups, rank=True, order=True, offsets=True):
    _need_gpu(group_ids)
    g = _i32c(group_ids)
    n, dev = g.shape[0], g.device
    r = torch.empty((n,), dtype=torch.int32, device=dev) if rank else None
    o = torch.empty((n,), dtype=torch.int32, device=dev) if order else None
    off = torch.empty((n_groups + 1,), dtype=torch.int32, device=dev) if offsets else None
    ws = _workspace(_lib.query("seg3d_group_index_workspace_bytes", n, n_groups), dev)
    _lib.call("seg3d_group_index", _ptr(g), n, int(n_groups), _ptr(r), _ptr(o), _ptr(off), _ptr(ws), ws.numel(),
              _stream())
    return r, o, off


def get_inner_win_inds(group_inds):
    _need_gpu(group_inds)
    if group_inds.numel() == 0:
        return torch.zeros_like(group_inds)
    ng = int(group_inds.max().item()) + 1
    r, _, _ = group_index(group_inds.to(torch.int32), ng, rank=True, order=False, offsets=False)
    return r.to(group_inds.dtype)


class SegmentIndex:

    def __init__(self, ids, n_segments):
        self.ids = _i32c(ids)
        self.n_segments = int(n_segments)
        _, self.order, self.offsets = group_index(self.ids, self.n_segments, rank=False)


class CoordHash:
    def __init__(self, coords, spatial_shape):
        _need_gpu(coords)
        self.coords = _i32c(coords)
        self.shape = [int(s) for s in spatial_shape]
        m = self.coords.shape[0]
        self.table = _workspace(_lib.query("seg3d_coord_hash_bytes", m), coords.device)
        _lib.call("seg3d_coord_hash_build", _ptr(self.coords), m, _i3(self.shape), _ptr(self.table),
                  self.table.numel(), _stream())


def rulebook_subm(h):
    m = h.coords.shape[0]
    nbr = torch.empty((27, m), dtype=torch.int32, device=h.coords.device)
    _lib.call("seg3d_rulebook_subm", _ptr(h.coords), m, _i3(h.shape), _ptr(h.table), h.table.numel(), _ptr(nbr),
              _stream())
    return nbr


CONV_TILED = os.environ.get("SEG3D_CONV_TILED", "1") != "0"
CONV_TILED_MIN_C = int(os.environ.get("SEG3D_CONV_TILED_MIN_C", "0"))


class ConvPlan:

    def __init__(self, coords, nbr):
        _need_gpu(coords, nbr)
        coords = _i32c(coords)
        m = nbr.shape[1]
        if coords.shape[0] != m or nbr.shape[0] != 27 or nbr.dtype != torch.int32 or not nbr.is_contiguous():
            raise _lib.Seg3dError("ConvPlan: coords [m, 4] and a contiguous int32 table [27, m] of the same sites expected")
        self.nbr, self.m = nbr, m
        self.data = torch.empty((max(_lib.query("seg3d_conv_plan_bytes", m), 1),), dtype=torch.uint8, device=nbr.device)
        ws_bytes = _lib.query("seg3d_conv_plan_workspace_bytes", m)
        ws = torch.empty((max(ws_bytes, 1),), dtype=torch.uint8, device=nbr.device)
        _lib.call("seg3d_conv_plan_build", _ptr(coords), _ptr(nbr), m, _ptr(self.data), _ptr(ws), ws_bytes, _stream())


def _tiled_fits(plan, packed, cin, cout):
    return (plan is not None and CONV_TILED and bool(packed.flags & PACK_SPLIT_BF16) and max(cin, cout) >= CONV_TILED_MIN_C
            and bool(_lib.load().seg3d_spconv_tiled_supported(int(cin), int(cout))))


def _conv_tiled(x, plan, packed, bias, addend, relu, cin, cout, y):
    _lib.call("seg3d_spconv_fwd_tiled", _ptr(x), _ptr(plan.nbr), _ptr(plan.data), plan.m, x.shape[0], _ptr(packed.data),
              packed.flags, _ptr(bias), _ptr(addend), int(bool(relu)), cin, cout, _ptr(y), _stream())
    return y


def downsample_launch(coords, batch_size, spatial_shape, rows_dev=None):
    _need_gpu(coords)
    coords = _i32c(coords)
    m, dev = coords.shape[0], coords.device
    shape_out = [(int(s) + 2 - 3) // 2 + 1 for s in spatial_shape]
    cells = int(batch_size) * shape_out[0] * shape_out[1] * shape_out[2]
    cap = max(min(8 * m, cells), 1)
    out = torch.empty((cap, 4), dtype=torch.int32, device=dev)
    count = torch.zeros((1,), dtype=torch.int32, device=dev)
    ws = _workspace(_lib.query("seg3d_downsample_workspace_bytes", int(batch_size), _i3(spatial_shape)), dev)
    _lib.call("seg3d_downsample_coords", _ptr(coords), m, _ptr(rows_dev), int(batch_size), _i3(spatial_shape), _ptr(out), cap,
              _ptr(count), _ptr(ws), ws.numel(), _stream())
    return out, count, shape_out


def downsample_coords(coords, batch_size, spatial_shape):
    out, count, shape_out = downsample_launch(coords, batch_size, spatial_shape)
    return out[: int(count.item())], shape_out


def downsample_chain(coords, batch_size, spatial_shape, levels):
    bufs, counts, shapes = [], [], []
    cur, cur_shape, rows = coords, spatial_shape, None
    for _ in range(levels):
        out, count, shape_out = downsample_launch(cur, batch_size, cur_shape, rows)
        bufs.append(out), counts.append(count), shapes.append(shape_out)
        cur, cur_shape, rows = out, shape_out, count
    ns = torch.cat(counts).tolist()
    return [(b[: int(n)], sh) for b, n, sh in zip(bufs, ns, shapes)]


def parity_order(coords):
    _need_gpu(coords)
    coords = _i32c(coords)
    m = coords.shape[0]
    order = torch.empty((m,), dtype=torch.int32, device=coords.device)
    ws_bytes = _lib.query("seg3d_knn_level_workspace_bytes", m)
    ws = _workspace(ws_bytes, coords.device)
    _lib.call("seg3d_parity_order", _ptr(coords), m, _ptr(order), _ptr(ws), ws_bytes, _stream())
    return order


def rulebook_strided(h_in, coords_out):
    m_in, m_out = h_in.coords.shape[0], coords_out.shape[0]
    dev = coords_out.device
    fwd = torch.empty((27, m_out), dtype=torch.int32, device=dev)
    inv = torch.empty((27, m_in), dtype=torch.int32, device=dev)
    _lib.call("seg3d_rulebook_strided", _ptr(coords_out), m_out, m_in, _i3(h_in.shape), _ptr(h_in.table),
              h_in.table.numel(), _ptr(fwd), _ptr(inv), _stream())
    return fwd, inv


PACK_FWD, PACK_T, PACK_T_FLIP = 0, 1, 3
PACK_SPLIT_BF16 = 4

CONV_PRECISION = os.environ.get("SEG3D_CONV_PRECISION", "bf16x3")


def _precision_flag():
    if CONV_PRECISION == "bf16x3":
        return PACK_SPLIT_BF16
    if CONV_PRECISION == "fp32":
        return 0
    raise _lib.Seg3dError(f"SEG3D_CONV_PRECISION must be 'bf16x3' or 'fp32', got {CONV_PRECISION!r}")


_WEIGHT_EPOCH = [0]


def invalidate_weight_caches():
    _WEIGHT_EPOCH[0] += 1


def _stamp(t):
    return (t._version, _WEIGHT_EPOCH[0])


def _register_optimizer_hook():
    from torch.optim.optimizer import register_optimizer_step_post_hook
    register_optimizer_step_post_hook(lambda *_: invalidate_weight_caches())


_register_optimizer_hook()


class _PackJob:
    __slots__ = ("owner", "src_ptr", "out", "cin", "cout", "kk", "transpose", "flip", "version", "blocks")


_PACK_JOBS = {}
_PACK_DESC = {}


def _cached_pack(weight, kk, transpose, flip):
    owner = weight._base if weight._base is not None else weight
    key = (id(owner), weight.storage_offset(), tuple(weight.shape), kk, transpose, flip)
    job = _PACK_JOBS.get(key)
    if job is None or job.owner() is not owner or job.src_ptr != weight.data_ptr():
        cout, cin = weight.shape[0], weight.shape[-1]
        job = _PackJob()
        job.owner, job.src_ptr = weakref.ref(owner), weight.data_ptr()
        job.cin, job.cout, job.kk, job.transpose, job.flip = cin, cout, kk, int(transpose), int(flip)
        nbytes = (_lib.query("seg3d_spconv_packed_bytes", cin, cout, 4 | job.transpose) if kk == 27
                  else _lib.query("seg3d_linear_packed_bytes", cin, cout, job.transpose))
        job.out = torch.empty((nbytes,), dtype=torch.uint8, device=weight.device)
        job.blocks = (nbytes // 32 + 255) // 256
        job.version = None
        _PACK_JOBS[key] = job
        _PACK_DESC.clear()
    if job.version != _stamp(owner):
        _refresh_packs(weight.device)
    return job.out


def _refresh_packs(device):
    stale, dead = [], []
    for key, job in _PACK_JOBS.items():
        owner = job.owner()
        if owner is None:
            dead.append(key)
        elif job.version != _stamp(owner) and job.out.device == device:
            stale.append((key, job, owner))
    for key in dead:
        del _PACK_JOBS[key]
    if dead:
        _PACK_DESC.clear()
    if not stale:
        return
    ident = tuple(k for k, _, _ in stale)
    hit = _PACK_DESC.get(ident)
    if hit is None:
        import numpy as np
        rec = np.zeros((len(stale),), dtype=np.dtype([("src", "<u8"), ("dst", "<u8"), ("cin", "<i4"), ("cout", "<i4"),
                                                       ("kk", "<i4"), ("transpose", "<i4"), ("flip", "<i4"),
                                                       ("reserved", "<i4"), ("first_block", "<i8")]))
        first = 0
        for i, (_, job, _) in enumerate(stale):
            rec[i] = (job.src_ptr, job.out.data_ptr(), job.cin, job.cout, job.kk, job.transpose, job.flip, 0, first)
            first += job.blocks
        desc = torch.from_numpy(rec.view(np.uint8).copy()).to(device)
        hit = (desc, first)
        if len(_PACK_DESC) > 8:
            _PACK_DESC.clear()
        _PACK_DESC[ident] = hit
    _lib.call("seg3d_pack_weights_batched", _ptr(hit[0]), len(stale), hit[1], _stream())
    for _, job, owner in stale:
        job.version = _stamp(owner)


def _registry_ok(weight):
    return (CONV_PRECISION == "bf16x3" and weight.is_cuda and weight.dtype == torch.float32 and weight.is_contiguous()
            and not weight.is_inference())


class PackedWeight:
    __slots__ = ("data", "flags")

    def __init__(self, data, flags):
        self.data, self.flags = data, flags


def pack_weight(weight, flags, use_registry=True):
    flags = int(flags) | _precision_flag()
    if use_registry and _registry_ok(weight) and (weight if weight._base is None else weight._base).is_leaf and weight.shape[-1] % 16 == 0:
        return PackedWeight(_cached_pack(weight, 27, flags & 1, (flags >> 1) & 1), flags)
    w = _f32c(weight)
    cout, cin = w.shape[0], w.shape[-1]
    nbytes = _lib.query("seg3d_spconv_packed_bytes", cin, cout, flags)
    out = torch.empty((nbytes,), dtype=torch.uint8, device=w.device)
    _lib.call("seg3d_spconv_pack_weight", _ptr(w), cin, cout, flags, _ptr(out), _stream())
    return PackedWeight(out, flags)


def debug_set_conv_nbt(nbt):
    _lib.call("seg3d_debug_set_conv_nbt", int(nbt))


CONV_DMA = os.environ.get("SEG3D_CONV_DMA", "0") == "1"


def _conv_dma_fits(packed, cin, cout):
    return CONV_DMA and (packed.flags & PACK_SPLIT_BF16) and cin >= 192 and cin % 32 == 0 and cout % 96 == 0


def _conv_dma(x, nbr, packed, bias, addend, relu, cin, cout, order, y):
    m_in, m_out = x.shape[0], nbr.shape[1]
    xs = torch.empty((_lib.query("seg3d_spconv_presplit_bytes", m_in, cin),), dtype=torch.uint8, device=x.device)
    _lib.call("seg3d_spconv_presplit", _ptr(x), m_in, cin, _ptr(xs), _stream())
    _lib.call("seg3d_spconv_fwd_presplit", _ptr(xs), _ptr(nbr), m_out, m_in, _ptr(packed.data), packed.flags, _ptr(bias),
              _ptr(addend), int(bool(relu)), cin, cout, _ptr(y), _ptr(order), _stream())
    return y


def _conv_apply(x, nbr, packed, bias, cin, cout, order=None, plan=None):
    m_out = nbr.shape[1]
    y = torch.empty((m_out, cout), dtype=torch.float32, device=x.device)
    if _tiled_fits(plan, packed, cin, cout):
        return _conv_tiled(x, plan, packed, bias, None, False, cin, cout, y)
    if _conv_dma_fits(packed, cin, cout):
        return _conv_dma(x, nbr, packed, bias, None, False, cin, cout, order, y)
    _lib.call("seg3d_spconv_fwd", _ptr(x), _ptr(nbr), m_out, x.shape[0], _ptr(packed.data), packed.flags, _ptr(bias),
              cin, cout, _ptr(y), _ptr(order), _stream())
    return y


STORAGE = os.environ.get("SEG3D_STORAGE", "fp32")
STORAGE_ROUND_INPUTS = os.environ.get("SEG3D_STORAGE_ROUND_INPUTS", "1") != "0"


TRAIN_STORAGE = os.environ.get("SEG3D_TRAIN_STORAGE", "fp32")


def _saved_rows(x):
    if TRAIN_STORAGE not in ("fp32", "bf16"):
        raise _lib.Seg3dError(f"SEG3D_TRAIN_STORAGE must be 'fp32' or 'bf16', got {TRAIN_STORAGE!r}")
    if not (TRAIN_STORAGE == "bf16" and CONV_PRECISION == "bf16x3" and x.dtype == torch.float32 and x.is_cuda):
        return x
    if not WGRAD_STREAM:
        return x.to(torch.bfloat16)
    main, side = torch.cuda.current_stream(x.device), side_stream(x.device)
    ev = torch.cuda.Event()
    ev.record(main)
    side.wait_event(ev)
    with torch.cuda.stream(side):
        y = x.to(torch.bfloat16)
    x.record_stream(side)
    return y


def conv_storage_bf16():
    if STORAGE not in ("fp32", "bf16"):
        raise _lib.Seg3dError(f"SEG3D_STORAGE must be 'fp32' or 'bf16', got {STORAGE!r}")
    return STORAGE == "bf16" and CONV_PRECISION == "bf16x3" and not torch.is_grad_enabled()


def conv_act(x, nbr, packed, bias, cin, cout, order=None, addend=None, relu=True, plan=None):
    if conv_storage_bf16() and not _conv_dma_fits(packed, cin, cout):
        if x.dtype == torch.float32 and STORAGE_ROUND_INPUTS:
            xin = x.to(torch.bfloat16).contiguous()
        else:
            xin = x.contiguous() if x.dtype in (torch.float32, torch.bfloat16) else x.float().contiguous()
        m_out = nbr.shape[1]
        y = torch.empty((m_out, cout), dtype=torch.bfloat16, device=x.device)
        res = None if addend is None else addend.to(torch.bfloat16).contiguous()
        if _tiled_fits(plan, packed, cin, cout):
            _lib.call("seg3d_spconv_fwd_tiled_bf16", _ptr(xin), int(xin.dtype == torch.bfloat16), _ptr(plan.nbr), _ptr(plan.data),
                      plan.m, xin.shape[0], _ptr(packed.data), packed.flags, _ptr(bias), _ptr(res), int(bool(relu)), cin, cout,
                      _ptr(y), _stream())
            return y
        _lib.call("seg3d_spconv_fwd_act_bf16", _ptr(xin), int(xin.dtype == torch.bfloat16), _ptr(nbr), m_out, xin.shape[0],
                  _ptr(packed.data), packed.flags, _ptr(bias), _ptr(res), int(bool(relu)), cin, cout, _ptr(y), _ptr(order),
                  _stream())
        return y
    x = _f32c(x)
    m_out = nbr.shape[1]
    y = torch.empty((m_out, cout), dtype=torch.float32, device=x.device)
    addend = None if addend is None else _f32c(addend)
    if _tiled_fits(plan, packed, cin, cout):
        return _conv_tiled(x, plan, packed, bias, addend, relu, cin, cout, y)
    if _conv_dma_fits(packed, cin, cout):
        return _conv_dma(x, nbr, packed, bias, addend, relu, cin, cout, order, y)
    _lib.call("seg3d_spconv_fwd_act", _ptr(x), _ptr(nbr), m_out, x.shape[0], _ptr(packed.data), packed.flags, _ptr(bias),
              _ptr(addend), int(bool(relu)), cin, cout, _ptr(y), _ptr(order), _stream())
    return y


class _SparseConvFn(torch.autograd.Function):

    @staticmethod
    def forward(ctx, x, weight, bias, nbr, nbr_t, t_flags, packed, order, order_t, plan=None, plan_t=None):
        x = _f32c(x)
        cout, cin = weight.shape[0], weight.shape[-1]
        if packed is None:
            packed = pack_weight(weight, PACK_FWD)
        y = _conv_apply(x, nbr, packed, None if bias is None else _f32c(bias), cin, cout, order, plan)
        ctx.save_for_backward(_saved_rows(x) if (ctx.needs_input_grad[1] and cin % 16 == 0 and cout % 16 == 0) else x, weight)
        ctx.nbr, ctx.nbr_t, ctx.t_flags, ctx.has_bias, ctx.order_t = nbr, nbr_t, t_flags, bias is not None, order_t
        ctx.plan_t = plan_t
        ctx.bias_param = bias
        return y

    @staticmethod
    def backward(ctx, dy):
        x, weight = ctx.saved_tensors
        dy = _f32c(dy)
        cout, cin = weight.shape[0], weight.shape[-1]
        dx = dw = db = None
        fk = _WgradFork(dy.device)
        if ctx.needs_input_grad[1]:
            dw = torch.empty_like(weight, dtype=torch.float32)
            ws_bytes = _lib.query("seg3d_spconv_wgrad_workspace_bytes", dy.shape[0], cin, cout)
            ws = torch.empty((ws_bytes,), dtype=torch.uint8, device=dy.device)
            if _precision_flag() & PACK_SPLIT_BF16:
                chunks = ctypes.c_int32(0)
                _lib.call("seg3d_spconv_wgrad_partials_xbf16" if x.dtype == torch.bfloat16 else "seg3d_spconv_wgrad_partials",
                          _ptr(x), _ptr(dy), _ptr(ctx.nbr), dy.shape[0], x.shape[0], cin, cout,
                          _ptr(ws), ws_bytes, ctypes.byref(chunks), fk.fork(ws, dy, x, ctx.nbr))
                n = 27 * cin * cout
                fk.add_reduce(ws, chunks.value, n, n, dw.data_ptr(), 0, ws)
            else:
                x = _f32c(x)
                _lib.call("seg3d_spconv_wgrad", _ptr(x), _ptr(dy), _ptr(ctx.nbr), dy.shape[0], x.shape[0], cin, cout,
                          _precision_flag(), _ptr(dw), _ptr(ws), ws_bytes, fk.fork(ws, dy, x, ctx.nbr))
        if ctx.needs_input_grad[0]:
            wt = pack_weight(weight, ctx.t_flags)
            dx = _conv_apply(dy, ctx.nbr_t, wt, None, cout, cin, ctx.order_t, ctx.plan_t)
        if ctx.has_bias and ctx.needs_input_grad[2]:
            if fk.on:
                fk.fork(dy)
                with torch.cuda.stream(fk.side):
                    db = dy.sum(0)
            else:
                db = dy.sum(0)
        fk.join((weight, dw), (ctx.bias_param, db))
        return dx, dw, db, None, None, None, None, None, None, None, None


def sparse_conv(x, weight, bias, nbr, nbr_t, t_flags, packed=None, order=None, order_t=None, plan=None, plan_t=None):
    _need_gpu(x, weight, nbr)
    return _SparseConvFn.apply(x, weight, bias, nbr, nbr_t, t_flags, packed, order, order_t, plan, plan_t)


def _linear_pack(weight, transpose):
    if _registry_ok(weight) and (weight if weight._base is None else weight._base).is_leaf:
        return _cached_pack(weight, 1, int(transpose), 0)
    w = _f32c(weight)
    cout, cin = w.shape
    out = torch.empty((_lib.query("seg3d_linear_packed_bytes", cin, cout, int(transpose)),), dtype=torch.uint8,
                      device=w.device)
    _lib.call("seg3d_linear_pack_weight", _ptr(w), cin, cout, int(transpose), _ptr(out), _stream())
    return out


def _linear_pack_f32(weight, transpose):
    cache = weight.__dict__.setdefault("_seg3d_f32_packs", {})
    hit = cache.get(int(transpose))
    if hit is not None and hit[0] == (_stamp(weight), weight.data_ptr()):
        return hit[1]
    w = _f32c(weight)
    cout, cin = w.shape
    out = torch.empty((_lib.query("seg3d_linear_packed_bytes_f32", cin, cout),), dtype=torch.uint8, device=w.device)
    _lib.call("seg3d_linear_pack_weight_f32", _ptr(w), cin, cout, int(transpose), _ptr(out), _stream())
    cache[int(transpose)] = ((_stamp(weight), weight.data_ptr()), out)
    return out


def _linear_apply_f32(x, packed, bias, cin, cout):
    y = torch.empty((x.shape[0], cout), dtype=torch.float32, device=x.device)
    _lib.call("seg3d_linear_fwd_f32", _ptr(x), x.shape[0], _ptr(packed), _ptr(bias), cin, cout, _ptr(y), _stream())
    return y


POINT_MLP = os.environ.get("SEG3D_POINT_MLP", "x6")


def _x6_fits(cin, cout):
    return POINT_MLP == "x6" and CONV_PRECISION == "bf16x3" and cin % 32 == 0 and cout % 64 == 0


def _linear_pack_x6(weight):
    cache = weight.__dict__.setdefault("_seg3d_x6_packs", {})
    hit = cache.get(0)
    if hit is not None and hit[0] == (_stamp(weight), weight.data_ptr()):
        return hit[1]
    w = _f32c(weight)
    cout, cin = w.shape
    out = torch.empty((_lib.query("seg3d_linear_packed_bytes_x6", cin, cout),), dtype=torch.uint8, device=w.device)
    _lib.call("seg3d_linear_pack_weight_x6", _ptr(w), cin, cout, 0, _ptr(out), _stream())
    cache[0] = ((_stamp(weight), weight.data_ptr()), out)
    return out


def _linear_apply_x6(x, packed, bias, cin, cout, scale=None, shift=None, relu=False):
    y = torch.empty((x.shape[0], cout), dtype=torch.float32, device=x.device)
    _lib.call("seg3d_linear_fwd_x6", _ptr(x), x.shape[0], _ptr(packed), _ptr(bias), _ptr(scale), _ptr(shift), int(relu),
              cin, cout, _ptr(y), _stream())
    return y


LINEAR_LN_FUSED = os.environ.get("SEG3D_LINEAR_LN", "1") != "0"


def _linear_layernorm(x, packed, bias, res, gamma, beta, eps, cin, cout):
    y = torch.empty((x.shape[0], cout), dtype=torch.float32, device=x.device)
    _lib.call("seg3d_linear_layernorm_fwd", _ptr(x), x.shape[0], _ptr(packed), _ptr(bias), _ptr(res), _ptr(gamma), _ptr(beta),
              float(eps), cin, cout, _ptr(y), _stream())
    return y


def _linear_apply(x, packed, bias, cin, cout, addend=None):
    y = torch.empty((x.shape[0], cout), dtype=torch.float32, device=x.device)
    _lib.call("seg3d_linear_fwd", _ptr(x), x.shape[0], _ptr(packed), _ptr(bias), _ptr(addend), cin, cout, _ptr(y), _stream())
    return y


class _LinearFn(torch.autograd.Function):

    @staticmethod
    def forward(ctx, x, weight, bias, exact):
        x = _f32c(x)
        cout, cin = weight.shape
        ctx.save_for_backward(_saved_rows(x) if ctx.needs_input_grad[1] else x, weight)
        ctx.has_bias, ctx.exact = bias is not None, exact
        ctx.bias_param = bias
        if exact:
            if _x6_fits(cin, cout):
                return _linear_apply_x6(x, _linear_pack_x6(weight), None if bias is None else _f32c(bias), cin, cout)
            if cin % 16 == 0 and cout % 16 == 0:
                return _linear_apply_f32(x, _linear_pack_f32(weight, 0), None if bias is None else _f32c(bias), cin, cout)
            return torch.nn.functional.linear(x, weight, bias)
        return _linear_apply(x, _linear_pack(weight, 0), None if bias is None else _f32c(bias), cin, cout)

    @staticmethod
    def backward(ctx, dy):
        x, weight = ctx.saved_tensors
        dy = _f32c(dy)
        cout, cin = weight.shape
        dx = dw = db = None
        fk = _WgradFork(dy.device)
        want_db = ctx.has_bias and ctx.needs_input_grad[2]
        if ctx.needs_input_grad[1]:
            dw = torch.empty_like(weight, memory_format=torch.contiguous_format)
            if want_db:
                db = torch.empty((cout,), dtype=torch.float32, device=dy.device)
            _linear_wgrad_into(fk, x, dy, cin, cout, dw.data_ptr(), db.data_ptr() if want_db else 0)
        elif want_db:
            db = dy.sum(0)
        if ctx.needs_input_grad[0]:
            if cout % 8 == 0 and cin % 16 == 0:
                dx = _linear_apply(dy, _linear_pack(weight, 1), None, cout, cin)
            elif ctx.exact and cout % 16 == 0 and cin % 16 == 0:
                dx = _linear_apply_f32(dy, _linear_pack_f32(weight, 1), None, cout, cin)
            else:
                dx = dy @ weight
        fk.join((weight, dw), (ctx.bias_param, db))
        return dx, dw, db, None


class _LinearOddShapeFn(torch.autograd.Function):

    @staticmethod
    def forward(ctx, x, weight, bias):
        x = _f32c(x)
        ctx.save_for_backward(x, weight)
        ctx.has_bias = bias is not None
        ctx.bias_param = bias
        return torch.nn.functional.linear(x, weight, bias)

    @staticmethod
    def backward(ctx, dy):
        x, weight = ctx.saved_tensors
        dy = _f32c(dy)
        cout, cin = weight.shape
        dx = dw = db = None
        fk = _WgradFork(dy.device)
        want_db = ctx.has_bias and ctx.needs_input_grad[2]
        if ctx.needs_input_grad[1]:
            pi, po = (-cin) % 4, (-cout) % 4
            xp = torch.nn.functional.pad(x, (0, pi)) if pi else x
            dyp = torch.nn.functional.pad(dy, (0, po)) if po else dy
            dwp = torch.empty((cout + po, cin + pi), dtype=torch.float32, device=dy.device)
            dbp = torch.empty((cout + po,), dtype=torch.float32, device=dy.device) if want_db else None
            _linear_wgrad_into(fk, xp, dyp, cin + pi, cout + po, dwp.data_ptr(), dbp.data_ptr() if want_db else 0)
            dw = dwp[:cout, :cin]
            if want_db:
                db = dbp[:cout]
        elif want_db:
            db = dy.sum(0)
        if ctx.needs_input_grad[0]:
            dx = dy @ weight
        if (cin % 4) or (cout % 4):
            fk.join()
        else:
# ... 1139 lines not shown
```

### openseg3d_amd/segformer.py

```python
import os
from collections import OrderedDict
from functools import partial

import torch
import torch.nn as nn

from . import ops
from . import spconv
from .swformer import SparseWindowPartitionLayer, SWFormerBlock


PLAN_FIRST = os.environ.get("SEG3D_PLAN_FIRST", "1") != "0"


def replace_feature(out, new_features):
    return out.replace_feature(new_features)


def conv_module(cin, cout, norm_fn, act_fn, conv_type="subm", indice_key=None):
    if conv_type == "subm":
        conv = spconv.SubMConv3d(cin, cout, 3, padding=1, bias=False, indice_key=indice_key)
    elif conv_type == "spconv":
        conv = spconv.SparseConv3d(cin, cout, 3, stride=2, padding=1, bias=False, indice_key=indice_key)
    elif conv_type == "inverseconv":
        conv = spconv.SparseInverseConv3d(cin, cout, 3, bias=False, indice_key=indice_key)
    else:
        raise NotImplementedError(conv_type)
    return ConvBnAct(conv, norm_fn(cout), act_fn)


class ConvBnAct(spconv.SparseSequential):

    def forward(self, x):
        conv, bn = self._modules["0"], self._modules["1"]
        if conv.fusable_with(bn, x):
            return conv.forward_bn_act(x, bn, relu=True)
        y = conv(x)
        return y.replace_feature(ops.batch_norm_act(y.features, bn, relu=True))


class FusedMLP(nn.Sequential):

    def forward(self, x):
        mods = list(self._modules.values())
        i = 0
        while i < len(mods):
            m = mods[i]
            if isinstance(m, RowLinear) and i + 1 < len(mods) and not self.training \
                    and isinstance(mods[i + 1], nn.BatchNorm1d) and not isinstance(mods[i + 1], NarrowBatchNorm1d):
                relu = i + 2 < len(mods) and isinstance(mods[i + 2], nn.ReLU)
                y = ops.linear_bn_act_eval(x, m, mods[i + 1], relu)
                if y is not None:
                    x = y
                    i += 3 if relu else 2
                    continue
            if isinstance(m, (nn.BatchNorm1d, nn.SyncBatchNorm)) and not isinstance(m, NarrowBatchNorm1d) \
                    and m.num_features % 4 == 0:
                relu = i + 1 < len(mods) and isinstance(mods[i + 1], nn.ReLU)
                x = ops.batch_norm_act(x, m, relu=relu)
                i += 2 if relu else 1
            else:
                x = m(x)
                i += 1
        return x


class VFE(nn.Module):

    def __init__(self, voxel_feature_channel, reduce="mean"):
        super().__init__()
        self.voxel_feature_channel = voxel_feature_channel
        self.reduce = reduce

    def forward(self, features, seg):
        return ops.segment_reduce(features, seg, {"mean": ops.REDUCE_MEAN, "max": ops.REDUCE_MAX}[self.reduce])


class FlattenSELayer(nn.Module):

    def __init__(self, channel, reduction=4):
        super().__init__()
        self.fc = nn.Sequential(nn.Linear(channel, channel // reduction, bias=False), nn.ReLU(inplace=True),
                                nn.Linear(channel // reduction, channel, bias=False), nn.Sigmoid())

    def forward(self, x, indices, row_offsets=None):
        if row_offsets is not None:
            starts = [0] + list(row_offsets[:-1])
            spans = [(s, e) for s, e in zip(starts, row_offsets)]
            pooled = ops.span_mean(x, row_offsets)
            gate = self.fc(pooled)
            return torch.cat([x[s:e] * gate[b] for b, (s, e) in enumerate(spans)], dim=0)
        indices = indices.long()
        pooled = ops.scatter(x, indices, reduce="mean")
        return x * self.fc(pooled)[indices]


class SparseBasicBlock(spconv.SparseModule):
    def __init__(self, inplanes, planes, norm_fn, act_fn, indice_key=None):
        super().__init__()
        self.conv1 = spconv.SubMConv3d(inplanes, planes, 3, padding=1, bias=True, indice_key=indice_key)
        self.bn1 = norm_fn(planes)
        self.act = act_fn
        self.conv2 = spconv.SubMConv3d(planes, planes, 3, padding=1, bias=True, indice_key=indice_key)
        self.bn2 = norm_fn(planes)

    def forward(self, x):
        if self.conv1.fusable_with(self.bn1, x) and self.conv2.fusable_with(self.bn2, x):
            y = self.conv1.forward_bn_act(x, self.bn1, relu=True)
            return self.conv2.forward_bn_act(y, self.bn2, relu=True, res=x.features)
        y = self.conv1(x)
        y = y.replace_feature(ops.batch_norm_act(y.features, self.bn1, relu=True))
        y = self.conv2(y)
        return y.replace_feature(ops.batch_norm_act(y.features, self.bn2, relu=True, res=x.features))


class UpBlock(spconv.SparseModule):
    def __init__(self, inplanes, planes, norm_fn, act_fn, conv_type, layer_id):
        super().__init__()
        self.transform = SparseBasicBlock(inplanes, inplanes, norm_fn, act_fn, indice_key=f"subm{layer_id}")
        self.bottleneck = conv_module(2 * inplanes, inplanes, norm_fn, act_fn, "subm", f"subm{layer_id}")
        key = f"spconv{layer_id}" if conv_type == "inverseconv" else f"subm{layer_id}"
        self.out = conv_module(inplanes, planes, norm_fn, act_fn, conv_type, key)

    def forward(self, x_bottom, x_lateral):
        t = self.transform(x_lateral)
        cat = torch.cat([x_bottom.features, t.features], dim=1)
        m = self.bottleneck(t.replace_feature(cat)).features
        if cat.shape[1] == 2 * m.shape[1]:
            skip = cat[:, 0::2] + cat[:, 1::2]
        else:
            skip = cat.view(cat.shape[0], m.shape[1], -1).sum(dim=2)
        return self.out(t.replace_feature(m + skip))


class PointTransformer(nn.Module):
    def __init__(self, input_channels, output_channels, grid_size, voxel_size, point_cloud_range, batching_info,
                 window_shape, drop_path_rate, depths, num_classes):
        super().__init__()
        self.sparse_shape = [int(g) for g in grid_size][::-1]
        self.voxel_size, self.point_cloud_range = voxel_size, point_cloud_range
        self.depths = list(depths)
        grid_xyz = [float(g) for g in grid_size]
        self.norm_fn = partial(nn.BatchNorm1d, eps=1e-3, momentum=0.01)
        self.act_fn = nn.ReLU(inplace=True)
        norm_fn, act_fn = self.norm_fn, self.act_fn

        self.conv_input = ConvBnAct(
            spconv.SubMConv3d(input_channels, 48, 3, padding=1, bias=False, indice_key="subm1"), norm_fn(48), act_fn)
        dpr = [x.item() for x in torch.linspace(0, drop_path_rate, sum(self.depths))]
        widths = (48, 96, 192, 384)
        for k, c in enumerate(widths):
            lo, hi = sum(self.depths[:k]), sum(self.depths[:k + 1])
            stage = nn.Sequential(
                SparseWindowPartitionLayer(batching_info[k], window_shape, [g / (2 ** k) for g in grid_xyz]),
                SWFormerBlock(c, 8, depth=self.depths[k], drop_path=dpr[lo:hi]))
            setattr(self, f"swformer_block{k + 1}", stage)
        for k in (1, 2, 3):
            setattr(self, f"conv_down{k}", conv_module(widths[k - 1], widths[k], norm_fn, act_fn, "spconv",
                                                       f"spconv{k + 1}"))
        self.up4 = UpBlock(384, 192, norm_fn, act_fn, "inverseconv", 4)
        self.up3 = UpBlock(192, 96, norm_fn, act_fn, "inverseconv", 3)
        self.up2 = UpBlock(96, 48, norm_fn, act_fn, "inverseconv", 2)
        self.up1 = UpBlock(48, output_channels, norm_fn, act_fn, "subm", 1)
        self.aux_voxel_classifier = nn.Sequential(RowLinear(384, num_classes, bias=False))
        self.voxel_classifier = nn.Sequential(RowLinear(output_channels, num_classes, bias=False))

    def prepare(self, batch_dict):
        level = spconv.SiteLevel(batch_dict["voxel_coords"].int(), self.sparse_shape, batch_dict["batch_size"])
        batch_dict["site_level"] = level
        widths = (48, 96, 192, 384)
        level.seed_chain(3)
        launched = []
        for k in range(4):
            level.subm()
            level.mask_order()
            level.subm_plan()
            part = getattr(self, f"swformer_block{k + 1}")[0]
            if part not in level.window_plans:
                level.window_plans[part] = part.launch_plan(level.coords, level.batch_size, widths[k])
                launched.append(level.window_plans[part])
            if k < 3:
                level.parity_order()
                level = level.down()[0]
        if launched:
            SparseWindowPartitionLayer.finish_plans(launched)
        return batch_dict

    def forward(self, batch_dict):
        x = spconv.SparseConvTensor(features=batch_dict["voxel_features"], indices=batch_dict["voxel_coords"].int(),
                                    spatial_shape=self.sparse_shape, batch_size=batch_dict["batch_size"],
                                    _level=batch_dict.get("site_level"))
        x1 = self.conv_input(x)
        x1 = x1.replace_feature(self.swformer_block1(x1))
        x2 = self.conv_down1(x1)
        x2 = x2.replace_feature(self.swformer_block2(x2))
        x3 = self.conv_down2(x2)
        x3 = x3.replace_feature(self.swformer_block3(x3))
        x4 = self.conv_down3(x3)
        x4 = x4.replace_feature(self.swformer_block4(x4))

        batch_dict["aux_voxel_out"] = self.aux_voxel_classifier(x4.features)
        batch_dict["aux_voxel_coords"] = x4.indices

        y = self.up4(x4, x4)
        y = self.up3(y, x3)
        y = self.up2(y, x2)
        y = self.up1(y, x1)
        batch_dict["voxel_features"] = y.features
        batch_dict["voxel_coords"] = y.indices
        batch_dict["voxel_out"] = self.voxel_classifier(y.features)
        return batch_dict


class NarrowBatchNorm1d(nn.BatchNorm1d):

    def forward(self, x):
        if not self.training or not self.track_running_stats:
            return super().forward(x)
        if x.is_cuda and x.dim() == 2 and x.dtype == torch.float32 and self.affine and x.shape[0] >= 2:
            return ops.narrow_batch_norm(x, self)
        var, mean = torch.var_mean(x, dim=0, unbiased=False)
        with torch.no_grad():
            n = x.shape[0]
            self.num_batches_tracked += 1
            mom = self.momentum if self.momentum is not None else 1.0 / float(self.num_batches_tracked)
            self.running_mean.mul_(1 - mom).add_(mean, alpha=mom)
            self.running_var.mul_(1 - mom).add_(var * (n / max(n - 1, 1)), alpha=mom)
        y = (x - mean) * torch.rsqrt(var + self.eps)
        return y * self.weight + self.bias if self.affine else y


class RowLinear(nn.Linear):

    def forward(self, x):
        if x.dtype == torch.bfloat16:
            x = x.float()
        return ops.linear(x, self.weight, self.bias, exact=True)


def _bn_mlp(dims, first_bn=None, last_plain=False):
    mods = [NarrowBatchNorm1d(first_bn)] if first_bn is not None else []
    n = len(dims) - 1
    for i in range(n):
        if last_plain and i == n - 1:
            mods.append(RowLinear(dims[i], dims[i + 1]))
        else:
            mods += [RowLinear(dims[i], dims[i + 1], bias=False), nn.BatchNorm1d(dims[i + 1]), nn.ReLU(inplace=True)]
    return FusedMLP(*mods)


class DeepFusionBlock(nn.Module):

    def __init__(self, lidar_channel, image_channel, hidden_channel, n_neighbors, attn_pdrop=0.3, faithful_stride=True):
        super().__init__()
        self.n_neighbors, self.faithful_stride = n_neighbors, faithful_stride
        self.q_embedding = nn.Linear(lidar_channel, hidden_channel)
        self.k_embedding = nn.Linear(image_channel, hidden_channel)
        self.v_embedding = nn.Linear(image_channel, hidden_channel)
        self.attn_dropout = nn.Dropout(attn_pdrop)
        self.c_proj = nn.Linear(hidden_channel, image_channel)

    def neighbours(self, points, point_id_offset):
        xyz = points.contiguous() if self.faithful_stride else points[:, :3].contiguous()
        knn_ids, _ = ops.knn_query(self.n_neighbors, xyz, xyz, point_id_offset, point_id_offset)
        return knn_ids

    def forward(self, points, point_id_offset, lidar_features, image_features, knn_ids=None):
        q = self.q_embedding(lidar_features)
        k = self.k_embedding(image_features)
        v = self.v_embedding(image_features)
        if knn_ids is None:
            knn_ids = self.neighbours(points, point_id_offset)
        invalid = image_features.sum(dim=1) == 0
        if q.is_cuda and q.shape[1] == 32 and self.n_neighbors <= 16:
            keep = None
            if self.training and self.attn_dropout.p > 0.0:
                keep = self.attn_dropout(torch.ones(knn_ids.shape, dtype=torch.float32, device=q.device))
            return self.c_proj(ops.knn_attention(q, k, v, knn_ids, invalid, keep))
        knn_ids = knn_ids.long()
        attn = (q.unsqueeze(1) * k[knn_ids]).sum(dim=-1) / (q.shape[-1] ** 0.5)
        attn = attn.masked_fill(invalid[knn_ids], float("-inf"))
        attn = torch.nan_to_num(torch.softmax(attn, dim=-1))
        attn = self.attn_dropout(attn)
        return self.c_proj((attn.unsqueeze(-1) * v[knn_ids]).sum(dim=1))


class Segformer(nn.Module):
    def __init__(self, dataset, batching_info, window_shape, depths, drop_path_rate):
        super().__init__()
        dim_point = dataset.dim_point + (2 if dataset.use_cylinder else 0)
        self.use_multi_sweeps = bool(dataset.use_multi_sweeps)
        self.use_image_feature = bool(dataset.use_image_feature)
        self.point_feature_channel = 64
        self.point_encoder = _bn_mlp([dim_point, 64, 128, 256, self.point_feature_channel], first_bn=dim_point,
                                     last_plain=True)
        self.vfe = VFE(dim_point, reduce="mean") if self.use_multi_sweeps else VFE(self.point_feature_channel, "max")
        self.scatter = VFE(3, reduce="mean")
        self.voxel_feature_channel = 32
        self.point_transformer = PointTransformer(
            self.vfe.voxel_feature_channel, self.voxel_feature_channel, dataset.grid_size, dataset.voxel_size,
            dataset.point_cloud_range, batching_info=batching_info, window_shape=window_shape, depths=depths,
            drop_path_rate=drop_path_rate, num_classes=dataset.num_classes)
        self.image_feature_channel = dataset.dim_image_feature if self.use_image_feature else 0
        if self.use_image_feature:
            self.deep_fusion = DeepFusionBlock(self.point_feature_channel + self.voxel_feature_channel,
                                               self.image_feature_channel, 32, 16)
        self.fusion_feature_channel = 64
        self.fusion_encoder = _bn_mlp([self.point_feature_channel + self.voxel_feature_channel
                                       + self.image_feature_channel, 256, 128, self.fusion_feature_channel])
        self.se = FlattenSELayer(self.fusion_feature_channel)
        self.classifier = FusedMLP(RowLinear(self.fusion_feature_channel, 64, bias=False), nn.BatchNorm1d(64),
                                   nn.ReLU(True), nn.Dropout(0.3),
                                   RowLinear(64, dataset.num_classes, bias=False))
        self.weight_initialization()

    def weight_initialization(self):
        for m in self.modules():
            if isinstance(m, nn.Linear):
                nn.init.kaiming_normal_(m.weight)
                if m.bias is not None:
                    nn.init.constant_(m.bias, 0)
            elif isinstance(m, (nn.BatchNorm1d, nn.LayerNorm)):
                nn.init.constant_(m.weight, 1.0)
                nn.init.constant_(m.bias, 0)

    def prepare_batch(self, batch_dict):
        if "site_level" not in batch_dict:
            self.point_transformer.prepare(batch_dict)
        if self.use_image_feature and "fusion_knn" not in batch_dict:
            cur_points, _ = self._current_sweep(batch_dict)
            batch_dict["fusion_knn"] = self.deep_fusion.neighbours(cur_points, batch_dict["point_id_offset"].int())
        return batch_dict

    def _current_sweep(self, batch_dict):
        points = batch_dict["points"][:, 1:]
# ... 79 lines not shown
```

### openseg3d_amd/spconv.py

```python
import math
import os

import torch
import torch.nn as nn

from . import ops


FUSE_EVAL_BN = os.environ.get("SEG3D_FUSE_EVAL_BN", "1") != "0"
SUBM_ORDER_BUCKET = int(os.environ.get("SEG3D_SUBM_ORDER", "0"))


class SiteLevel:

    def __init__(self, coords, spatial_shape, batch_size):
        self.coords = coords if coords.dtype == torch.int32 else coords.to(torch.int32)
        self.coords = self.coords.contiguous()
        self.shape = [int(s) for s in spatial_shape]
        self.batch_size = int(batch_size)
        self._hash = None
        self._subm = None
        self._down = None
        self._parity = None
        self._mask_order = None
        self._subm_plan = None
        self._coarse = None
        self._offsets = False
        self.window_plans = {}

    def sample_offsets(self):
        if self._offsets is False:
            m = self.coords.shape[0]
            if self.batch_size == 1:
                self._offsets = [m]
            else:
                b = self.coords[:, 0]
                cnt = torch.bincount(b, minlength=self.batch_size)
                ordered = bool((b[1:] >= b[:-1]).all()) if m > 1 else True
                self._offsets = torch.cumsum(cnt, 0).tolist() if ordered and cnt.numel() == self.batch_size else None
        return self._offsets

    @property
    def hash(self):
        if self._hash is None:
            self._hash = ops.CoordHash(self.coords, self.shape)
        return self._hash

    def subm(self):
        if self._subm is None:
            self._subm = ops.rulebook_subm(self.hash)
        return self._subm

    def subm_plan(self):
        if not ops.CONV_TILED or ops.CONV_PRECISION != "bf16x3" or self.coords.shape[0] == 0:
            return None
        if self._subm_plan is None:
            self._subm_plan = ops.ConvPlan(self.coords, self.subm())
        return self._subm_plan

    def mask_order(self):
        if SUBM_ORDER_BUCKET == 0:
            return None
        if self._mask_order is None:
            valid = self.subm() >= 0
            m = valid.shape[1]
            bits = (valid.to(torch.int64) << torch.arange(27, device=valid.device, dtype=torch.int64)[:, None]).sum(0)
            if SUBM_ORDER_BUCKET > 0:
                bits = bits | ((torch.arange(m, device=valid.device, dtype=torch.int64) // SUBM_ORDER_BUCKET) << 27)
            self._mask_order = torch.argsort(bits, stable=True).to(torch.int32)
        return self._mask_order

    def parity_order(self):
        if self._parity is None:
            self._parity = ops.parity_order(self.coords)
        return self._parity

    def seed_chain(self, levels):
        if self._down is None and self._coarse is None:
            chain = ops.downsample_chain(self.coords, self.batch_size, self.shape, levels)
            self._coarse = chain

    def down(self):
        if self._down is None:
            if self._coarse:
                (co, shape_out), rest = self._coarse[0], self._coarse[1:]
            else:
                (co, shape_out), rest = ops.downsample_coords(self.coords, self.batch_size, self.shape), None
            fwd, inv = ops.rulebook_strided(self.hash, co)
            coarse = SiteLevel(co, shape_out, self.batch_size)
            coarse._coarse = rest or None
            self._down = (coarse, fwd, inv)
            self._coarse = None
        return self._down


class SparseConvTensor:
    def __init__(self, features, indices, spatial_shape, batch_size, _level=None, _indice_dict=None):
        self.features = features
        self.spatial_shape = [int(s) for s in spatial_shape]
        self.batch_size = int(batch_size)
        self.level = _level if _level is not None else SiteLevel(indices, self.spatial_shape, batch_size)
        self.indices = self.level.coords
        self.indice_dict = _indice_dict if _indice_dict is not None else {}

    def replace_feature(self, new_features):
        return SparseConvTensor(new_features, self.indices, self.spatial_shape, self.batch_size, self.level,
                                self.indice_dict)

    def on_level(self, features, level):
        return SparseConvTensor(features, level.coords, level.shape, self.batch_size, level, self.indice_dict)


class SparseModule(nn.Module):
    """Marker base class: SparseSequential hands these the SparseConvTensor itself."""


class _Conv3x3x3(SparseModule):
    def __init__(self, in_channels, out_channels, kernel_size=3, stride=1, padding=0, dilation=1, bias=True,
                 indice_key=None):
        super().__init__()
        ks = kernel_size if isinstance(kernel_size, int) else kernel_size[0]
        if ks != 3 or dilation != 1:
            raise NotImplementedError("only 3x3x3, dilation 1 is on the OpenSeg3D path")
        if out_channels % 16:
            raise NotImplementedError("output channels must be a multiple of 16 (MFMA 16x16 tiles)")
        self._pad_in = (-in_channels) % 16
        self.in_channels, self.out_channels = in_channels, out_channels
        self.stride, self.padding, self.indice_key = stride, padding, indice_key
        self.weight = nn.Parameter(torch.empty(out_channels, 3, 3, 3, in_channels))
        self.bias = nn.Parameter(torch.empty(out_channels)) if bias else None
        self._packed = None
        self._folded = None
        self.reset_parameters()

    def reset_parameters(self):
        fan_in = 27 * self.in_channels
        nn.init.kaiming_uniform_(self.weight.view(self.out_channels, -1), a=math.sqrt(5))
        if self.bias is not None:
            bound = 1.0 / math.sqrt(fan_in)
            nn.init.uniform_(self.bias, -bound, bound)

    def _packed_weight(self):
        w = self.weight
        key = (ops._stamp(w), w.data_ptr(), ops.CONV_PRECISION)
        if self._packed is None or self._packed[0] != key:
            with torch.no_grad():
                self._packed = (key, ops.pack_weight(w, ops.PACK_FWD))
        return self._packed[1]

    def _apply_tables(self, feats, nbr, nbr_t, t_flags, order=None, order_t=None, plan=None, plan_t=None):
        if self._pad_in:
            feats = torch.nn.functional.pad(feats, (0, self._pad_in))
            weight = torch.nn.functional.pad(self.weight, (0, self._pad_in))
            return ops.sparse_conv(feats, weight, self.bias, nbr, nbr_t, t_flags, None, order, order_t, plan, plan_t)
        return ops.sparse_conv(feats, self.weight, self.bias, nbr, nbr_t, t_flags, self._packed_weight(), order, order_t,
                               plan, plan_t)

    def plans(self, x):
        return None, None

    def tables(self, x):
        raise NotImplementedError

    def forward(self, x):
        nbr, nbr_t, t_flags, order, order_t, level = self.tables(x)
        plan, plan_t = self.plans(x)
        return x.on_level(self._apply_tables(x.features, nbr, nbr_t, t_flags, order, order_t, plan, plan_t), level)

    def fusable_with(self, bn, x):
        return (FUSE_EVAL_BN and not torch.is_grad_enabled() and not bn.training and bn.track_running_stats and bn.affine
                and not self._pad_in and ops.CONV_PRECISION == "bf16x3" and x.features.is_cuda
                and (x.features.dtype == torch.float32 or (x.features.dtype == torch.bfloat16 and ops.conv_storage_bf16())))

    def forward_bn_act(self, x, bn, relu=True, res=None):
        scale, shift, bn_key = ops.bn_eval_affine(bn)
        w = self.weight
        key = (ops._stamp(w), w.data_ptr(), None if self.bias is None else self.bias._version, bn_key)
        if self._folded is None or self._folded[0] != key:
            with torch.no_grad():
                wf = (w * scale.view(-1, 1, 1, 1, 1)).contiguous()
                bf = shift if self.bias is None else shift + self.bias * scale
                self._folded = (key, ops.pack_weight(wf, ops.PACK_FWD, use_registry=False), bf.contiguous())
        _, packed, bias = self._folded
        nbr, _, _, order, _, level = self.tables(x)
        y = ops.conv_act(x.features, nbr, packed, bias, self.in_channels, self.out_channels, order, addend=res, relu=relu,
                         plan=self.plans(x)[0])
        return x.on_level(y, level)

    def extra_repr(self):
        return f"{self.in_channels}, {self.out_channels}, kernel_size=3, stride={self.stride}, " \
               f"padding={self.padding}, indice_key={self.indice_key!r}"


class SubMConv3d(_Conv3x3x3):
    def tables(self, x):
        nbr = x.level.subm()
        order = x.level.mask_order()
        return nbr, nbr, ops.PACK_T_FLIP, order, order, x.level

    def plans(self, x):
        plan = x.level.subm_plan()
        return plan, plan


class SparseConv3d(_Conv3x3x3):
    def tables(self, x):
        if self.stride != 2 or self.padding != 1:
            raise NotImplementedError("only SparseConv3d(k=3, stride=2, padding=1) is on the OpenSeg3D path")
        coarse, fwd, inv = x.level.down()
        if self.indice_key is not None:
            x.indice_dict[self.indice_key] = x.level
        return fwd, inv, ops.PACK_T, None, x.level.parity_order(), coarse


class SparseInverseConv3d(_Conv3x3x3):
    def __init__(self, in_channels, out_channels, kernel_size=3, bias=True, indice_key=None):
        super().__init__(in_channels, out_channels, kernel_size, bias=bias, indice_key=indice_key)

    def tables(self, x):
        fine = x.indice_dict.get(self.indice_key)
        if fine is None:
            raise KeyError(f"SparseInverseConv3d: no strided conv registered indice_key={self.indice_key!r}")
        coarse, fwd, inv = fine.down()
        if coarse is not x.level:
            raise RuntimeError("SparseInverseConv3d input does not live on the paired strided conv's output sites")
        return inv, fwd, ops.PACK_T, fine.parity_order(), None, fine


class SparseSequential(SparseModule):

    def __init__(self, *mods):
        super().__init__()
        for i, m in enumerate(mods):
            self.add_module(str(i), m)

    def __getitem__(self, idx):
        if not -len(self) <= idx < len(self):
            raise IndexError(f"index {idx} is out of range")
        return list(self._modules.values())[idx]

    def __len__(self):
        return len(self._modules)

    def forward(self, x):
        for m in self._modules.values():
            if isinstance(m, SparseModule):
                x = m(x)
            elif isinstance(x, SparseConvTensor):
                x = x.replace_feature(m(x.features))
            else:
                x = m(x)
        return x
```

### openseg3d_amd/spnet.py

```python
from collections import OrderedDict
from functools import partial

import torch
import torch.nn as nn
import torch.nn.functional as F

from . import ops
from . import segformer as segformer_mod
from . import spconv
from .segformer import (ConvBnAct, DeepFusionBlock, FlattenSELayer, FusedMLP, RowLinear, UpBlock, VFE, _bn_mlp,
                        conv_module)


class SparseBasicBlock(spconv.SparseModule):

    def __init__(self, inplanes, planes, norm_fn, act_fn, with_se=False, indice_key=None):
        super().__init__()
        self.conv1 = spconv.SubMConv3d(inplanes, planes, 3, padding=1, bias=True, indice_key=indice_key)
        self.bn1 = norm_fn(planes)
        self.act = act_fn
        self.conv2 = spconv.SubMConv3d(planes, planes, 3, padding=1, bias=True, indice_key=indice_key)
        self.bn2 = norm_fn(planes)
        self.se = FlattenSELayer(planes) if with_se else None
        self.sa = None

    def forward(self, x):
        if self.se is None and self.conv1.fusable_with(self.bn1, x) and self.conv2.fusable_with(self.bn2, x):
            y = self.conv1.forward_bn_act(x, self.bn1, relu=True)
            return self.conv2.forward_bn_act(y, self.bn2, relu=True, res=x.features)
        y = self.conv1(x)
        y = y.replace_feature(ops.batch_norm_act(y.features, self.bn1, relu=True))
        y = self.conv2(y)
        if self.se is None:
            return y.replace_feature(ops.batch_norm_act(y.features, self.bn2, relu=True, res=x.features))
        f = ops.batch_norm_act(y.features, self.bn2, relu=False)
        f = self.se(f, y.indices[:, 0], y.level.sample_offsets())
        return y.replace_feature(torch.relu(f + x.features))


class SpatialGatherModule(nn.Module):

    def __init__(self, scale):
        super().__init__()
        self.scale = scale

    def forward(self, feats, probs, batch_size, batch_indices, offsets=None):
        if offsets is not None and feats.is_cuda and ops.class_context_fits(probs.shape[1], feats.shape[1]):
            return ops.class_context(feats, probs, offsets[:batch_size], self.scale)
        out = []
        for i in range(batch_size):
            sel = slice(offsets[i - 1] if i else 0, offsets[i]) if offsets is not None else batch_indices == i
            prob = F.softmax(self.scale * probs[sel].t(), dim=1)
            out.append(prob @ feats[sel])
        return torch.stack(out)


class ObjectAttentionBlock(nn.Module):

    def __init__(self, in_channels, key_channels):
        super().__init__()
        self.key_channels = key_channels

        def proj(cin, cout):
            return FusedMLP(nn.Linear(cin, cout, bias=False), nn.BatchNorm1d(cout), nn.ReLU(inplace=True))

        self.query_project = proj(in_channels, key_channels)
        self.key_project = proj(in_channels, key_channels)
        self.value_project = proj(in_channels, key_channels)
        self.bottleneck = proj(key_channels, in_channels)

    def forward(self, x, proxy):
        query = self.query_project(x)
        key = self.key_project(proxy)
        value = self.value_project(proxy)
        sim = F.softmax((self.key_channels ** -0.5) * (query @ key.t()), dim=-1)
        return self.bottleneck(sim @ value)


class OCRLayer(nn.Module):

    def __init__(self, in_channels, mid_channels, key_channels, scale=1.0, drop=0.05):
        super().__init__()
        self.scale = scale
        self.transform_input = ConvBnAct(spconv.SubMConv3d(in_channels, mid_channels, 3, padding=1, bias=False),
                                         nn.BatchNorm1d(mid_channels), nn.ReLU(inplace=True))
        self.spatial_gather_module = SpatialGatherModule(self.scale)
        self.object_context_block = ObjectAttentionBlock(mid_channels, key_channels)
        self.bottleneck = FusedMLP(nn.Linear(mid_channels * 2, in_channels, bias=False), nn.BatchNorm1d(in_channels),
                                   nn.ReLU(inplace=True), nn.Dropout(drop))

    def forward(self, inputs, probs, batch_size):
        inputs = self.transform_input(inputs)
        feats = inputs.features
        batch_indices = inputs.indices[:, 0]
        offsets = inputs.level.sample_offsets()
        context = self.spatial_gather_module(feats, probs, batch_size, batch_indices, offsets)
        pieces, rows = [], []
        for i in range(batch_size):
            if offsets is not None:
                sel = slice(offsets[i - 1] if i else 0, offsets[i])
            else:
                sel = torch.nonzero(batch_indices == i).view(-1)
                rows.append(sel)
            pieces.append(self.object_context_block(feats[sel], context[i]))
        out = torch.cat(pieces) if batch_size > 1 else pieces[0]
        if rows:
            out = torch.empty_like(feats).index_copy(0, torch.cat(rows), out)
        feats = self.bottleneck(torch.cat([out, feats], dim=1))
        return inputs.replace_feature(feats)


class SparseUnet(nn.Module):

    def __init__(self, input_channels, output_channels, grid_size, voxel_size, point_cloud_range, num_classes,
                 use_ocr=True):
        super().__init__()
        self.sparse_shape = grid_size[::-1]
        self.voxel_size, self.point_cloud_range, self.use_ocr = voxel_size, point_cloud_range, use_ocr
        norm_fn = partial(nn.BatchNorm1d, eps=1e-3, momentum=0.01)
        act_fn = nn.ReLU(inplace=True)
        block = partial(SparseBasicBlock, norm_fn=norm_fn, act_fn=act_fn)
        self.conv_input = conv_module(input_channels, 32, norm_fn, act_fn, "subm", "subm1")
        self.conv1 = spconv.SparseSequential(block(32, 32, indice_key="subm1"), block(32, 32, indice_key="subm1"))
        self.conv2 = spconv.SparseSequential(
            conv_module(32, 64, norm_fn, act_fn, "spconv", "spconv2"), block(64, 64, indice_key="subm2"),
            block(64, 64, indice_key="subm2"), block(64, 64, indice_key="subm2"))
        self.conv3 = spconv.SparseSequential(
            conv_module(64, 128, norm_fn, act_fn, "spconv", "spconv3"), block(128, 128, indice_key="subm3"),
            block(128, 128, indice_key="subm3"), block(128, 128, with_se=True, indice_key="subm3"))
        self.conv4 = spconv.SparseSequential(
            conv_module(128, 256, norm_fn, act_fn, "spconv", "spconv4"), block(256, 256, indice_key="subm4"),
            block(256, 256, indice_key="subm4"), block(256, 256, with_se=True, indice_key="subm4"))
        up = partial(_UpBlock, norm_fn=norm_fn, act_fn=act_fn)
        self.up4 = up(256, 128, conv_type="inverseconv", layer_id=4)
        self.up3 = up(128, 64, conv_type="inverseconv", layer_id=3)
        self.up2 = up(64, 32, conv_type="inverseconv", layer_id=2)
        self.up1 = up(32, output_channels, conv_type="subm", layer_id=1)
        if self.use_ocr:
            self.ocr = OCRLayer(256, 128, 64)
        self.aux_voxel_classifier = nn.Sequential(RowLinear(256, num_classes, bias=False))
        self.voxel_classifier = nn.Sequential(RowLinear(output_channels, num_classes, bias=False))

    def prepare(self, batch_dict):
        level = spconv.SiteLevel(batch_dict["voxel_coords"].int(), self.sparse_shape, batch_dict["batch_size"])
        batch_dict["site_level"] = level
        level.seed_chain(3)
        for k in range(4):
            level.subm()
            level.mask_order()
            level.subm_plan()
            if k >= 2:
                level.sample_offsets()
            if k < 3:
                level.parity_order()
                level = level.down()[0]
        return batch_dict

    def forward(self, batch_dict):
        coords = batch_dict["voxel_coords"]
        x = spconv.SparseConvTensor(batch_dict["voxel_features"], coords.int(), self.sparse_shape, batch_dict["batch_size"],
                                    _level=batch_dict.get("site_level"))
        x = self.conv_input(x)
        x1 = self.conv1(x)
        x2 = self.conv2(x1)
        x3 = self.conv3(x2)
        x4 = self.conv4(x3)
        aux = self.aux_voxel_classifier(x4.features)
        batch_dict["aux_voxel_out"], batch_dict["aux_voxel_coords"] = aux, x4.indices
        if self.use_ocr:
            x4 = self.ocr(x4, aux, batch_dict["batch_size"])
        y = self.up4(x4, x4)
        y = self.up3(y, x3)
        y = self.up2(y, x2)
        y = self.up1(y, x1)
        batch_dict["voxel_features"], batch_dict["voxel_coords"] = y.features, y.indices
        batch_dict["voxel_out"] = self.voxel_classifier(y.features)
        return batch_dict


class _UpBlock(UpBlock):

    def __init__(self, inplanes, planes, norm_fn, act_fn, conv_type, layer_id):
        super().__init__(inplanes, planes, norm_fn, act_fn, conv_type, layer_id)
        self.transform = SparseBasicBlock(inplanes, inplanes, norm_fn, act_fn, indice_key=f"subm{layer_id}")


class SPNet(nn.Module):
    def __init__(self, dataset):
        super().__init__()
        dim_point = dataset.dim_point + (2 if dataset.use_cylinder else 0)
        self.use_multi_sweeps = bool(dataset.use_multi_sweeps)
        self.use_image_feature = bool(dataset.use_image_feature)
        self.point_feature_channel = 64
        self.point_encoder = _bn_mlp([dim_point, 64, 128, 256, self.point_feature_channel], first_bn=dim_point,
                                     last_plain=True)
        self.vfe = VFE(dim_point, reduce="mean") if self.use_multi_sweeps else VFE(self.point_feature_channel, "max")
        self.voxel_feature_channel = 64
        self.voxel_encoder = SparseUnet(self.vfe.voxel_feature_channel, self.voxel_feature_channel, dataset.grid_size,
                                        dataset.voxel_size, dataset.point_cloud_range, dataset.num_classes)
        self.image_feature_channel = dataset.dim_image_feature if self.use_image_feature else 0
        if self.use_image_feature:
            self.deep_fusion = DeepFusionBlock(self.point_feature_channel + self.voxel_feature_channel,
                                               self.image_feature_channel, 32, 16)
        self.fusion_feature_channel = 64
        self.fusion_encoder = _bn_mlp([self.point_feature_channel + self.voxel_feature_channel
                                       + self.image_feature_channel, 256, 128, self.fusion_feature_channel])
        self.se = FlattenSELayer(self.fusion_feature_channel)
        self.classifier = FusedMLP(RowLinear(self.fusion_feature_channel, 64, bias=False), nn.BatchNorm1d(64),
                                   nn.ReLU(True), nn.Dropout(0.3), RowLinear(64, dataset.num_classes, bias=False))
        self.weight_initialization()

    def weight_initialization(self):
        for m in self.modules():
            if isinstance(m, nn.Linear):
                nn.init.kaiming_normal_(m.weight)
                if m.bias is not None:
                    nn.init.constant_(m.bias, 0)
            elif isinstance(m, (nn.BatchNorm1d, nn.LayerNorm)):
                nn.init.constant_(m.weight, 1.0)
                nn.init.constant_(m.bias, 0)

    def prepare_batch(self, batch_dict):
        if "site_level" not in batch_dict:
            self.voxel_encoder.prepare(batch_dict)
        return batch_dict

    def forward(self, batch_dict):
        if self.training and torch.is_grad_enabled():
            ops.probe_deferred_join(batch_dict["points"].device)
        with ops.deferred_bn_counters():
            return self._forward(batch_dict)

    def _forward(self, batch_dict):
        points = batch_dict["points"][:, 1:]
        ids = batch_dict["point_voxel_ids"]
        n_voxels = batch_dict["voxel_coords"].shape[0]
        seg = batch_dict.get("point_voxel_index")
        if seg is None:
            seg = ops.SegmentIndex(ids, n_voxels)
        if segformer_mod.PLAN_FIRST and "site_level" not in batch_dict:
            self.voxel_encoder.prepare(batch_dict)
        if self.use_multi_sweeps:
            cur_rows = torch.nonzero(points[:, 3] == 0).view(-1)
            cur_points, cur_ids, cur_seg = points[cur_rows], seg.ids[cur_rows], None
            batch_rows = batch_dict["points"][cur_rows, 0]
        else:
            cur_points, cur_ids, cur_seg, batch_rows = points, seg.ids, seg, batch_dict["points"][:, 0]
        point_features = self.point_encoder(cur_points)
        batch_dict["voxel_features"] = self.vfe(points if self.use_multi_sweeps else point_features, seg)
        batch_dict = self.voxel_encoder(batch_dict)

        point_voxel_features = ops.gather_rows(batch_dict["voxel_features"], cur_ids, cur_seg)
        fused = torch.cat([point_features, point_voxel_features], dim=1)
        if self.use_image_feature:
            img = self.deep_fusion(cur_points, batch_dict["point_id_offset"].int(), fused,
                                   batch_dict["point_image_features"])
            fused = torch.cat([fused, img], dim=1)
        fused = self.fusion_encoder(fused)
        row_offsets = batch_dict.get("point_row_offsets")
        if row_offsets is None and batch_dict.get("point_id_offset") is not None:
            row_offsets = [int(v) for v in batch_dict["point_id_offset"].tolist()]
        fused = fused + self.se(fused, batch_rows, row_offsets)

        result = OrderedDict()
        result["point_out"] = self.classifier(fused)
        result["voxel_out"] = batch_dict["voxel_out"]
        result["aux_voxel_out"] = batch_dict["aux_voxel_out"]
        result["voxel_coords"] = batch_dict["voxel_coords"]
        result["aux_voxel_coords"] = batch_dict["aux_voxel_coords"]
        return result
```

Measured before the change: 4.187 million points/s.

## Build compacted per-offset pair lists for sparse conv weight-gradient

Adds a pair-list builder that compacts the 27-offset neighbour table into contiguous (input,output) pairs per offset, built once per level during prepare in training. The split-bf16 weight-gradient kernel gains a LIST variant that reads these pairs directly with shuffles instead of scanning the dense neighbour table through a per-wave LDS ring. The goal is to drop the wasted scanning of empty neighbour slots and balance work evenly across chunks. In exchange it costs two extra kernels plus a scan per level and more memory for the pair arrays.

After: 4.200 million points/s, median of 6. No clear change (+0.3%).

```diff
diff --git a/__graft_entry__.py b/__graft_entry__.py
--- a/__graft_entry__.py
+++ b/__graft_entry__.py
@@ -5,7 +5,7 @@
 ROOT = os.path.dirname(os.path.abspath(__file__))
 CSRC = os.path.join(ROOT, "openseg3d_amd", "csrc")
 LIB = os.path.join(CSRC, "libseg3d_hip.so")
-HIP_SOURCES = ["scan.hip", "voxelize.hip", "group.hip", "rulebook.hip", "spconv.hip", "spconv_split.hip", "linear_stream.hip", "linear_x6.hip", "spconv_dma.hip", "spconv_tile.hip", "wgrad_split.hip", "wgrad_dense.hip", "wgrad_dense_lds.hip", "window.hip",
+HIP_SOURCES = ["scan.hip", "voxelize.hip", "group.hip", "rulebook.hip", "pairs.hip", "spconv.hip", "spconv_split.hip", "linear_stream.hip", "linear_x6.hip", "spconv_dma.hip", "spconv_tile.hip", "wgrad_split.hip", "wgrad_dense.hip", "wgrad_dense_lds.hip", "window.hip",
                "attention.hip", "attention_fused.hip", "attention_fused_bwd.hip", "attention_small.hip", "rownorm.hip", "segment.hip", "knn.hip", "knn_attention.hip", "class_context.hip", "loss.hip", "lovasz.hip", "eval.hip"]
 HIPCC_FLAGS = ["--offload-arch=gfx950", "-O3", "-std=c++17", "-fPIC", "-ffp-contract=off",
                "-fhip-fp32-correctly-rounded-divide-sqrt", "-Wall", "-Wno-unused-function"]
diff --git a/include/seg3d_hip.h b/include/seg3d_hip.h
--- a/include/seg3d_hip.h
+++ b/include/seg3d_hip.h
@@ -116,6 +116,17 @@
                                       int64_t m_in, int32_t cin, int32_t cout, void* workspace, size_t workspace_bytes,
                                       int32_t* chunks, void* stream);
 
+size_t seg3d_pair_list_bytes(int64_t m_out);
+size_t seg3d_pair_list_workspace_bytes(int64_t m_out);
+int seg3d_pair_list_build(const int32_t* nbr, int64_t m_out, void* out, void* workspace, size_t workspace_bytes, void* stream);
+size_t seg3d_spconv_wgrad_pairs_workspace_bytes(int64_t m_out, int32_t cin, int32_t cout);
+int seg3d_spconv_wgrad_partials_pairs(const float* x, const float* dy, const int32_t* pair_off, const void* pairs,
+                                      int64_t m_out, int64_t m_in, int32_t cin, int32_t cout, void* workspace,
+                                      size_t workspace_bytes, int32_t* chunks, void* stream);
+int seg3d_spconv_wgrad_partials_pairs_xbf16(const uint16_t* x_bf16, const float* dy, const int32_t* pair_off, const void* pairs,
+                                            int64_t m_out, int64_t m_in, int32_t cin, int32_t cout, void* workspace,
+                                            size_t workspace_bytes, int32_t* chunks, void* stream);
+
 size_t seg3d_linear_wgrad_workspace_bytes(int64_t m, int32_t cin, int32_t cout);
 int seg3d_linear_wgrad(const float* x, const float* dy, int64_t m, int32_t cin, int32_t cout, float* dw,
                        float* db , void* workspace, size_t workspace_bytes, void* stream);
diff --git a/openseg3d_amd/_lib.py b/openseg3d_amd/_lib.py
--- a/openseg3d_amd/_lib.py
+++ b/openseg3d_amd/_lib.py
@@ -8,7 +8,7 @@
 
 OK, EINVAL, EWORKSPACE, ELAUNCH = 0, -1, -2, -3
 REDUCE_SUM, REDUCE_MEAN, REDUCE_MAX = 0, 1, 2
-ABI_VERSION = 41
+ABI_VERSION = 42
 
 _p, _i32, _i64, _sz, _f = ctypes.c_void_p, ctypes.c_int32, ctypes.c_int64, ctypes.c_size_t, ctypes.c_float
 _u64 = ctypes.c_uint64
@@ -53,6 +53,12 @@
     "seg3d_spconv_wgrad": (ctypes.c_int, [_p, _p, _p, _i64, _i64, _i32, _i32, _i32, _p, _p, _sz, _p]),
     "seg3d_spconv_wgrad_partials": (ctypes.c_int, [_p, _p, _p, _i64, _i64, _i32, _i32, _p, _sz, _p, _p]),
     "seg3d_spconv_wgrad_partials_xbf16": (ctypes.c_int, [_p, _p, _p, _i64, _i64, _i32, _i32, _p, _sz, _p, _p]),
+    "seg3d_pair_list_bytes": (_sz, [_i64]),
+    "seg3d_pair_list_workspace_bytes": (_sz, [_i64]),
+    "seg3d_pair_list_build": (ctypes.c_int, [_p, _i64, _p, _p, _sz, _p]),
+    "seg3d_spconv_wgrad_pairs_workspace_bytes": (_sz, [_i64, _i32, _i32]),
+    "seg3d_spconv_wgrad_partials_pairs": (ctypes.c_int, [_p, _p, _p, _p, _i64, _i64, _i32, _i32, _p, _sz, _p, _p]),
+    "seg3d_spconv_wgrad_partials_pairs_xbf16": (ctypes.c_int, [_p, _p, _p, _p, _i64, _i64, _i32, _i32, _p, _sz, _p, _p]),
     "seg3d_linear_wgrad_partials_xbf16": (ctypes.c_int, [_p, _p, _i64, _i32, _i32, _i32, _p, ctypes.c_size_t, _p, _p]),
     "seg3d_linear_packed_bytes_f32": (ctypes.c_size_t, [_i32, _i32]),
     "seg3d_linear_pack_weight_f32": (ctypes.c_int, [_p, _i32, _i32, _i32, _p, _p]),
diff --git a/openseg3d_amd/csrc/pairs.hip b/openseg3d_amd/csrc/pairs.hip
--- /dev/null
+++ b/openseg3d_amd/csrc/pairs.hip
@@ -0,0 +1,105 @@
+#include "common.hpp"
+
+namespace {
+
+constexpr int kThreads = 256;
+constexpr int kWavesPerBlock = kThreads / 64;
+constexpr int kSeg = 512;
+constexpr size_t kHeadBytes = 128;
+
+__device__ __forceinline__ bool segment_of(int64_t m, int64_t segs, int64_t n_seg, int64_t* seg, int* k, int64_t* r0) {
+    *seg = (int64_t)blockIdx.x * kWavesPerBlock + (threadIdx.x >> 6);
+    if (*seg >= n_seg) return false;
+    *k = (int)(*seg / segs);
+    *r0 = (*seg % segs) * kSeg;
+    return true;
+}
+
+__global__ __launch_bounds__(kThreads) void pair_count(const int32_t* __restrict__ nbr, int64_t m, int64_t segs, int64_t n_seg,
+                                                        uint32_t* __restrict__ cnt) {
+    int64_t seg, r0;
+    int k;
+    if (!segment_of(m, segs, n_seg, &seg, &k, &r0)) return;
+    const int lane = threadIdx.x & 63;
+    const int32_t* nk = nbr + (int64_t)k * m;
+    uint32_t n = 0;
+#pragma unroll
+    for (int i = 0; i < kSeg / 64; ++i) {
+        const int64_t r = r0 + 64 * i + lane;
+        n += (uint32_t)__popcll(__ballot(r < m && nk[r] >= 0));
+    }
+    if (lane == 0) cnt[seg] = n;
+}
+
+__global__ __launch_bounds__(kThreads) void pair_fill(const int32_t* __restrict__ nbr, int64_t m, int64_t segs, int64_t n_seg,
+                                                       const uint32_t* __restrict__ base, int32_t* __restrict__ pair_off,
+                                                       int2* __restrict__ pairs) {
+    int64_t seg, r0;
+    int k;
+    if (!segment_of(m, segs, n_seg, &seg, &k, &r0)) return;
+    const int lane = threadIdx.x & 63;
+    const int32_t* nk = nbr + (int64_t)k * m;
+    uint32_t at = base[seg];
+    if (r0 == 0 && lane == 0) pair_off[k] = (int32_t)at;
+    int32_t idx[kSeg / 64];
+#pragma unroll
+    for (int i = 0; i < kSeg / 64; ++i) {
+        const int64_t r = r0 + 64 * i + lane;
+        idx[i] = r < m ? nk[r] : -1;
+    }
+#pragma unroll
+    for (int i = 0; i < kSeg / 64; ++i) {
+        const unsigned long long mask = __ballot(idx[i] >= 0);
+        if (idx[i] >= 0) pairs[at + __popcll(mask & ((1ull << lane) - 1ull))] = make_int2(idx[i], (int)(r0 + 64 * i + lane));
+        at += (uint32_t)__popcll(mask);
+    }
+}
+
+int64_t segments(int64_t m_out) { return ceil_div64(m_out, kSeg); }
+
+bool fits(int64_t m_out) { return m_out >= 0 && m_out <= (int64_t)0x7FFFFFFF / 27; }
+
+}
+
+extern "C" {
+
+size_t seg3d_pair_list_bytes(int64_t m_out) {
+    if (!fits(m_out)) return 0;
+    return kHeadBytes + (size_t)27 * (size_t)m_out * sizeof(int2);
+}
+
+size_t seg3d_pair_list_workspace_bytes(int64_t m_out) {
+    if (!fits(m_out)) return 0;
+    const int64_t n_seg = 27 * segments(m_out);
+    WsCarver c(nullptr);
+    c.take<uint32_t>((size_t)n_seg + 1);
+    c.take<uint32_t>(scan_tmp_count(n_seg));
+    return c.off;
+}
+
+int seg3d_pair_list_build(const int32_t* nbr, int64_t m_out, void* out, void* workspace, size_t workspace_bytes, void* stream) {
+    if (!fits(m_out) || !out || (m_out > 0 && !nbr)) return SEG3D_EINVAL;
+    hipStream_t st = as_stream(stream);
+    int32_t* pair_off = static_cast<int32_t*>(out);
+    if (m_out == 0) {
+        SEG3D_CHECK_HIP(hipMemsetAsync(pair_off, 0, kHeadBytes, st));
+        return SEG3D_OK;
+    }
+    if (!workspace) return SEG3D_EINVAL;
+    if (workspace_bytes < seg3d_pair_list_workspace_bytes(m_out)) return SEG3D_EWORKSPACE;
+    const int64_t segs = segments(m_out), n_seg = 27 * segs;
+    WsCarver c(workspace);
+    uint32_t* cnt = c.take<uint32_t>((size_t)n_seg + 1);
+    uint32_t* tmp = c.take<uint32_t>(scan_tmp_count(n_seg));
+    int2* pairs = reinterpret_cast<int2*>(static_cast<char*>(out) + kHeadBytes);
+    const unsigned blocks = (unsigned)ceil_div64(n_seg, kWavesPerBlock);
+    hipLaunchKernelGGL(pair_count, dim3(blocks), dim3(kThreads), 0, st, nbr, m_out, segs, n_seg, cnt);
+    SEG3D_CHECK_LAUNCH();
+    const int rc = scan_exclusive_u32(cnt, cnt, n_seg, reinterpret_cast<uint32_t*>(pair_off + 27), tmp, st);
+    if (rc != SEG3D_OK) return rc;
+    hipLaunchKernelGGL(pair_fill, dim3(blocks), dim3(kThreads), 0, st, nbr, m_out, segs, n_seg, cnt, pair_off, pairs);
+    SEG3D_CHECK_LAUNCH();
+    return SEG3D_OK;
+}
+
+}
diff --git a/openseg3d_amd/csrc/spconv.hip b/openseg3d_amd/csrc/spconv.hip
--- a/openseg3d_amd/csrc/spconv.hip
+++ b/openseg3d_amd/csrc/spconv.hip
@@ -11,6 +11,9 @@
 size_t wgrad_split_sparse_workspace_bytes(int64_t m_out, int cin, int cout);
 int wgrad_split_sparse(const void* x, const float* dy, const int32_t* nbr, int64_t m_out, int cin, int cout, float* dw,
                        void* workspace, size_t workspace_bytes, hipStream_t st, int32_t* chunks_out, bool x_bf16);
+size_t wgrad_split_sparse_pairs_workspace_bytes(int64_t m_out, int cin, int cout);
+int wgrad_split_sparse_pairs(const void* x, const float* dy, const int32_t* pair_off, const void* pairs, int64_t m_out, int cin,
+                             int cout, void* workspace, size_t workspace_bytes, hipStream_t st, int32_t* chunks_out, bool x_bf16);
 
 namespace {
 
@@ -374,4 +377,32 @@
     return wgrad_split_sparse(x_bf16, dy, nbr, m_out, cin, cout, nullptr, workspace, workspace_bytes, as_stream(stream), chunks, true);
 }
 
-}
+size_t seg3d_spconv_wgrad_pairs_workspace_bytes(int64_t m_out, int32_t cin, int32_t cout) {
+    if (m_out < 0 || cin <= 0 || cout <= 0) return 0;
+    return wgrad_split_sparse_pairs_workspace_bytes(m_out, cin, cout);
+}
+
+static int wgrad_pairs_entry(const void* x, const float* dy, const int32_t* pair_off, const void* pairs, int64_t m_out, int64_t m_in,
+                             int32_t cin, int32_t cout, void* workspace, size_t workspace_bytes, int32_t* chunks, void* stream,
+                             bool x_bf16) {
+    if (m_out < 0 || m_in < 0 || cin <= 0 || cout <= 0 || (cin & 15) || (cout & 15) || !chunks) return SEG3D_EINVAL;
+    *chunks = 0;
+    if (m_out == 0) return SEG3D_OK;
+    if (!x || !dy || !pair_off || !pairs) return SEG3D_EINVAL;
+    return wgrad_split_sparse_pairs(x, dy, pair_off, pairs, m_out, cin, cout, workspace, workspace_bytes, as_stream(stream), chunks,
+                                    x_bf16);
+}
+
+int seg3d_spconv_wgrad_partials_pairs(const float* x, const float* dy, const int32_t* pair_off, const void* pairs, int64_t m_out,
+                                      int64_t m_in, int32_t cin, int32_t cout, void* workspace, size_t workspace_bytes,
+                                      int32_t* chunks, void* stream) {
+    return wgrad_pairs_entry(x, dy, pair_off, pairs, m_out, m_in, cin, cout, workspace, workspace_bytes, chunks, stream, false);
+}
+
+int seg3d_spconv_wgrad_partials_pairs_xbf16(const uint16_t* x_bf16, const float* dy, const int32_t* pair_off, const void* pairs,
+                                            int64_t m_out, int64_t m_in, int32_t cin, int32_t cout, void* workspace,
+                                            size_t workspace_bytes, int32_t* chunks, void* stream) {
+    return wgrad_pairs_entry(x_bf16, dy, pair_off, pairs, m_out, m_in, cin, cout, workspace, workspace_bytes, chunks, stream, true);
+}
+
+}
diff --git a/openseg3d_amd/csrc/voxelize.hip b/openseg3d_amd/csrc/voxelize.hip
--- a/openseg3d_amd/csrc/voxelize.hip
+++ b/openseg3d_amd/csrc/voxelize.hip
@@ -273,7 +273,7 @@
     return cart2polar_impl<double>(points, n_points, row_stride, xyz_col, out, stream);
 }
 
-int seg3d_abi_version(void) { return 41; }
+int seg3d_abi_version(void) { return 42; }
 
 namespace {
 thread_local char g_last_error[320] = "";
diff --git a/openseg3d_amd/csrc/wgrad_split.hip b/openseg3d_amd/csrc/wgrad_split.hip
--- a/openseg3d_amd/csrc/wgrad_split.hip
+++ b/openseg3d_amd/csrc/wgrad_split.hip
@@ -84,15 +84,28 @@
     return p;
 }
 
-template <bool XB>
+struct PairSource {
+    const int32_t* nbr;
+    const int32_t* pair_off;
+    const int2* pairs;
+};
+
+__device__ __forceinline__ void unit_pair_range(const int32_t* pair_off, int k, int chunk, int n_chunks, int* begin, int* end) {
+    const int off = pair_off[k], n = pair_off[k + 1] - off;
+    *begin = off + (int)((int64_t)chunk * n / n_chunks);
+    *end = off + (int)((int64_t)(chunk + 1) * n / n_chunks);
+}
+
+template <bool XB, bool LIST = false>
 __global__ __launch_bounds__(kThreads, 2) void wgrad_sparse_kernel(const void* __restrict__ x_v, const float* __restrict__ dy,
-                                                                    const int32_t* __restrict__ nbr, int64_t m_rows,
+                                                                    const PairSource src_pairs, int64_t m_rows,
                                                                     int cin, int cout, int rows_per_chunk, int nbi,
                                                                     int tiles, int units, float* __restrict__ part,
                                                                     int center_first) {
     const float* x = static_cast<const float*>(x_v);
+    const int32_t* nbr = src_pairs.nbr;
     __shared__ __attribute__((aligned(16))) float red[64 * 64];
-    __shared__ int2 ring[kWaves][kRing];
+    __shared__ int2 ring[LIST ? 1 : kWaves][LIST ? 1 : kRing];
     const int lane = threadIdx.x & 63, wave = threadIdx.x >> 6;
     const int cq = lane & 15, rg = lane >> 4;
     const int xcd = blockIdx.x & 7, j = blockIdx.x >> 3;
@@ -110,7 +123,7 @@
     const float* px = x + (ci0 + 4 * cq < cin ? ci0 + 4 * cq : 0);
     const uint16_t* pxb = static_cast<const uint16_t*>(x_v) + (ci0 + 4 * cq < cin ? ci0 + 4 * cq : 0);
     const float* py = dy + (co0 + 4 * cq < cout ? co0 + 4 * cq : 0);
-    int2* my = ring[wave];
+    int2* my = ring[LIST ? 0 : wave];
 
     f32x4 acc[4][4];
 #pragma unroll
@@ -121,11 +134,13 @@
     constexpr int kAhead = 4;
     int head = 0, tail = 0;
     int64_t g_row = r_begin + 64 * (int64_t)wave;
-    int32_t idxq[kAhead];
-#pragma unroll
-    for (int j = 0; j < kAhead; ++j) {
-        const int64_t r = g_row + (int64_t)j * 64 * kWaves + lane;
-        idxq[j] = r < r_end ? nk[r] : -1;
+    int32_t idxq[kAhead] = {};
+    if constexpr (!LIST) {
+#pragma unroll
+        for (int j = 0; j < kAhead; ++j) {
+            const int64_t r = g_row + (int64_t)j * 64 * kWaves + lane;
+            idxq[j] = r < r_end ? nk[r] : -1;
+        }
     }
     auto scan_group = [&]() {
         const int32_t idx = idxq[0];
@@ -146,6 +161,17 @@
         while (tail - head < 32 && g_row < r_end) scan_group();
         __builtin_amdgcn_wave_barrier();
     };
+    int p_pos = 0, p_end = 0;
+    int2 cur = make_int2(0, 0), ahead = make_int2(0, 0);
+    auto list_fetch = [&](int pos) {
+        const int v = p_end - pos, e = lane & 31;
+        return v > 0 ? src_pairs.pairs[pos + (e < v ? e : 0)] : make_int2(0, 0);
+    };
+    auto left = [&]() { return p_end - p_pos < 32 ? (p_end - p_pos > 0 ? p_end - p_pos : 0) : 32; };
+    auto step_pair = [&](int h0, int valid, int e) {
+        if constexpr (LIST) return make_int2(__shfl(cur.x, e, 64), __shfl(cur.y, e, 64));
+        else return my[(h0 + (e < valid ? e : 0)) & (kRing - 1)];
+    };
 
     f32x4 xr[XB ? 1 : 8], yr[8];
     uint2 xq[XB ? 8 : 1];
@@ -153,8 +179,7 @@
     auto load_x = [&](int h0, int valid) {
 #pragma unroll
         for (int i = 0; i < 8; ++i) {
-            const int e = 8 * rg + i;
-            const int2 p = my[(h0 + (e < valid ? e : 0)) & (kRing - 1)];
+            const int2 p = step_pair(h0, valid, 8 * rg + i);
             if constexpr (XB) xq[i] = *reinterpret_cast<const uint2*>(pxb + (int64_t)p.x * cin);
             else xr[i] = *reinterpret_cast<const f32x4*>(px + (int64_t)p.x * cin);
         }
@@ -170,8 +195,7 @@
     auto load_y = [&](int h0, int valid) {
 #pragma unroll
         for (int i = 0; i < 8; ++i) {
-            const int e = 8 * rg + i;
-            const int2 p = my[(h0 + (e < valid ? e : 0)) & (kRing - 1)];
+            const int2 p = step_pair(h0, valid, 8 * rg + i);
             yr[i] = *reinterpret_cast<const f32x4*>(py + (int64_t)p.y * cout);
         }
         if (valid < 32) {
@@ -209,16 +233,34 @@
         }
     };
 
-    refill();
-    int valid = tail - head < 32 ? tail - head : 32;
+    int valid;
+    if constexpr (LIST) {
+        const int n_chunks = units / 27;
+        unit_pair_range(src_pairs.pair_off, k, chunk, n_chunks, &p_pos, &p_end);
+        p_pos += 32 * wave;
+        cur = list_fetch(p_pos);
+        ahead = list_fetch(p_pos + 32 * kWaves);
+        valid = left();
+    } else {
+        refill();
+        valid = tail - head < 32 ? tail - head : 32;
+    }
     if (valid > 0) {
         load_x(head, valid);
         load_y(head, valid);
     }
     while (valid > 0) {
-        head += valid;
-        refill();
-        const int next = tail - head < 32 ? tail - head : 32;
+        int next;
+        if constexpr (LIST) {
+            p_pos += 32 * kWaves;
+            cur = ahead;
+            ahead = list_fetch(p_pos + 32 * kWaves);
+            next = left();
+        } else {
+            head += valid;
+            refill();
+            next = tail - head < 32 ? tail - head : 32;
+        }
         make_b();
         if (next > 0) load_x(head, next);
         multiply();
@@ -252,15 +294,17 @@
 
 constexpr int kRing2 = 512;
 
-template <bool XB, int DEPTH, bool SB = false>
+template <bool XB, int DEPTH, bool SB = false, bool LIST = false>
 __global__ __launch_bounds__(kThreads, SB ? 3 : 2) void wgrad_sparse_wide_kernel(const void* __restrict__ x_v, const float* __restrict__ dy,
-                                                                         const int32_t* __restrict__ nbr, int64_t m_rows,
+                                                                         const PairSource src_pairs, int64_t m_rows,
                                                                          int cin, int cout, int rows_per_chunk, int nbi,
                                                                          int tiles, int units, float* __restrict__ part,
                                                                          int center_first) {
+    static_assert(!(LIST && DEPTH == 2), "the list form keeps one gather step in flight");
     const float* x = static_cast<const float*>(x_v);
+    const int32_t* nbr = src_pairs.nbr;
     __shared__ __attribute__((aligned(16))) uint4 img[SB ? 1 : 2][4][2][4][64];
-    __shared__ int2 ring[kRing2];
+    __shared__ int2 ring[LIST ? 1 : kRing2];
     __shared__ int wave_cnt[2][kWaves];
     const int lane = threadIdx.x & 63, wave = threadIdx.x >> 6;
     const int cq = lane & 15, rg = lane >> 4;
@@ -291,8 +335,11 @@
 
     int head = 0, tail = 0, round = 0;
     int64_t g_row = r_begin;
-    int32_t idx_n1 = g_row + 64 * wave + lane < r_end ? nk[g_row + 64 * wave + lane] : -1;
-    int32_t idx_n2 = g_row + 64 * (kWaves + wave) + lane < r_end ? nk[g_row + 64 * (kWaves + wave) + lane] : -1;
+    int32_t idx_n1 = -1, idx_n2 = -1;
+    if constexpr (!LIST) {
+        idx_n1 = g_row + 64 * wave + lane < r_end ? nk[g_row + 64 * wave + lane] : -1;
+        idx_n2 = g_row + 64 * (kWaves + wave) + lane < r_end ? nk[g_row + 64 * (kWaves + wave) + lane] : -1;
+    }
     auto scan_round = [&]() {
         const int64_t row = g_row + 64 * wave + lane;
         const int32_t idx = idx_n1;
@@ -325,6 +372,14 @@
         while (tail - head < 32 && g_row < r_end) scan_round();
         __syncthreads();
     };
+    int p_pos = 0, p_end = 0;
+    int32_t cur = 0, ahead = 0;
+    auto list_fetch = [&](int pos) {
+        const int v = p_end - pos, e = lane & 31;
+        const int32_t* comp = reinterpret_cast<const int32_t*>(src_pairs.pairs) + (stage_dy ? 1 : 0);
+        return v > 0 ? comp[2 * (int64_t)(pos + (e < v ? e : 0))] : 0;
+    };
+    auto left = [&]() { return p_end - p_pos < 32 ? (p_end - p_pos > 0 ? p_end - p_pos : 0) : 32; };
 
     f32x4 raw[8], raw2[DEPTH == 2 ? 8 : 1];
     uint2 rawb[XB ? 8 : 1], rawb2[(XB && DEPTH == 2) ? 8 : 1];
@@ -333,8 +388,12 @@
 #pragma unroll
         for (int i = 0; i < 8; ++i) {
             const int e = 8 * rg + i;
-            const int2 p = ring[(h0 + (e < valid ? e : 0)) & (kRing2 - 1)];
-            rows[i] = stage_dy ? p.y : p.x;
+            if constexpr (LIST) {
+                rows[i] = __shfl(cur, e, 64);
+            } else {
+                const int2 p = ring[(h0 + (e < valid ? e : 0)) & (kRing2 - 1)];
+                rows[i] = stage_dy ? p.y : p.x;
+            }
         }
         if (XB && !stage_dy) {
             if constexpr (XB) {
@@ -404,18 +463,35 @@
     const unsigned long long st_begin = st_last;
 #endif
     if constexpr (DEPTH == 1) {
-        refill();
-        int valid = tail - head < 32 ? tail - head : 32;
+        int valid;
+        if constexpr (LIST) {
+            unit_pair_range(src_pairs.pair_off, k, chunk, units / 27, &p_pos, &p_end);
+            cur = list_fetch(p_pos);
+            ahead = list_fetch(p_pos + 32);
+            valid = left();
+        } else {
+            refill();
+            valid = tail - head < 32 ? tail - head : 32;
+        }
         if (valid > 0) {
             load_slab(head, valid);
             stash(0);
         }
         WSTAMP(7);
         while (valid > 0) {
-            head += valid;
-            refill();
+            int next;
+            if constexpr (LIST) {
+                p_pos += 32;
+                cur = ahead;
+                ahead = list_fetch(p_pos + 32);
+                __syncthreads();
+                next = left();
+            } else {
+                head += valid;
+                refill();
+                next = tail - head < 32 ? tail - head : 32;
+            }
             WSTAMP(0);
-            const int next = tail - head < 32 ? tail - head : 32;
             if (next > 0) load_slab(head, next);
             WSTAMP(1);
             multiply(buf);
@@ -501,20 +577,27 @@
 #endif
 }
 
-}
-
-size_t wgrad_split_sparse_workspace_bytes(int64_t m_out, int cin, int cout) {
-    const Plan p = plan(m_out, cin, cout);
-    return ((size_t)p.chunks * 27 * (size_t)cin * cout + 64) * sizeof(float);
-}
-
-int wgrad_split_sparse(const void* x, const float* dy, const int32_t* nbr, int64_t m_out, int cin, int cout, float* dw,
-                       void* workspace, size_t workspace_bytes, hipStream_t st, int32_t* chunks_out, bool x_bf16) {
-    if (workspace_bytes < wgrad_split_sparse_workspace_bytes(m_out, cin, cout) || !workspace) return SEG3D_EINVAL;
-    const Plan p = plan(m_out, cin, cout);
-    float* part = static_cast<float*>(workspace);
-    const int units = p.chunks * 27;
+bool routes_wide(int cin, int cout) {
+    const bool fits128 = ((cin + 127) / 128) * 2 == (cin + 63) / 64 && ((cout + 127) / 128) * 2 == (cout + 63) / 64;
+    static const int wide_min = [] {
+        const char* e = getenv("SEG3D_WGRAD_WIDE_MIN");
+        return e ? atoi(e) : 0;
+    }();
+    const int cmin = cin < cout ? cin : cout, cmax = cin < cout ? cout : cin;
+    const bool wide_padded = (wide_min > 0 && cmin >= wide_min) || (cin != cout && cmin >= 96 && cmax >= 192);
     static const bool narrow_only = getenv("SEG3D_WGRAD_NARROW") != nullptr;
+    return (fits128 || wide_padded) && !narrow_only;
+}
+
+bool single_buffer() {
+    static const bool single = [] {
+        const char* e = getenv("SEG3D_WGRAD_SB");
+        return !(e && atoi(e) == 0);
+    }();
+    return single;
+}
+
+int unit_order() {
     static const int center_first = [] {
         const char* e = getenv("SEG3D_WGRAD_CENTER_FIRST");
         const int cf = (e && atoi(e) == 0) ? 0 : 1;
@@ -523,16 +606,27 @@
         if (xb < 1 || xb > 64) xb = 1;
         return cf | (xb << 8);
     }();
+    return center_first;
+}
+
+}
+
+size_t wgrad_split_sparse_workspace_bytes(int64_t m_out, int cin, int cout) {
+    const Plan p = plan(m_out, cin, cout);
+    return ((size_t)p.chunks * 27 * (size_t)cin * cout + 64) * sizeof(float);
+}
+
+int wgrad_split_sparse(const void* x, const float* dy, const int32_t* nbr, int64_t m_out, int cin, int cout, float* dw,
+                       void* workspace, size_t workspace_bytes, hipStream_t st, int32_t* chunks_out, bool x_bf16) {
+    if (workspace_bytes < wgrad_split_sparse_workspace_bytes(m_out, cin, cout) || !workspace) return SEG3D_EINVAL;
+    const Plan p = plan(m_out, cin, cout);
+    float* part = static_cast<float*>(workspace);
+    const int units = p.chunks * 27;
+    const PairSource src{nbr, nullptr, nullptr};
+    const int center_first = unit_order();
     const int xcd_block = center_first >> 8;
     const int unit_slots = (units + 8 * xcd_block - 1) / (8 * xcd_block) * (8 * xcd_block);
-    const bool fits128 = ((cin + 127) / 128) * 2 == (cin + 63) / 64 && ((cout + 127) / 128) * 2 == (cout + 63) / 64;
-    static const int wide_min = [] {
-        const char* e = getenv("SEG3D_WGRAD_WIDE_MIN");
-        return e ? atoi(e) : 0;
-    }();
-    const int cmin = cin < cout ? cin : cout, cmax = cin < cout ? cout : cin;
-    const bool wide_padded = (wide_min > 0 && cmin >= wide_min) || (cin != cout && cmin >= 96 && cmax >= 192);
-    if ((fits128 || wide_padded) && !narrow_only) {
+    if (routes_wide(cin, cout)) {
         const int nbo = (cout + 127) / 128, nbi = (cin + 127) / 128, tiles = nbo * nbi;
         const unsigned blocks = (unsigned)unit_slots * (unsigned)tiles;
         static const int depth = [] {
@@ -541,14 +635,11 @@
             return v == 2 ? 2 : 1;
         }();
 #define SEG3D_LAUNCH_WIDE(XB_, D_)                                                                                             \
-    hipLaunchKernelGGL((wgrad_sparse_wide_kernel<XB_, D_>), dim3(blocks), dim3(kThreads), 0, st, x, dy, nbr, m_out, cin, cout, \
+    hipLaunchKernelGGL((wgrad_sparse_wide_kernel<XB_, D_>), dim3(blocks), dim3(kThreads), 0, st, x, dy, src, m_out, cin, cout, \
                        (int)p.rows, nbi, tiles, units, part, center_first)
-        static const bool single = [] {
-            const char* e = getenv("SEG3D_WGRAD_SB");
-            return !(e && atoi(e) == 0);
-        }();
+        const bool single = single_buffer();
 #define SEG3D_LAUNCH_WIDE_SB(XB_)                                                                                                   \
-    hipLaunchKernelGGL((wgrad_sparse_wide_kernel<XB_, 1, true>), dim3(blocks), dim3(kThreads), 0, st, x, dy, nbr, m_out, cin, cout, \
+    hipLaunchKernelGGL((wgrad_sparse_wide_kernel<XB_, 1, true>), dim3(blocks), dim3(kThreads), 0, st, x, dy, src, m_out, cin, cout, \
                        (int)p.rows, nbi, tiles, units, part, center_first)
         if (single && depth == 1) {
             if (x_bf16) SEG3D_LAUNCH_WIDE_SB(true);
@@ -565,10 +656,10 @@
         const int tiles = p.nbo * p.nbi;
         const unsigned blocks = (unsigned)unit_slots * (unsigned)tiles;
         if (x_bf16)
-            hipLaunchKernelGGL(wgrad_sparse_kernel<true>, dim3(blocks), dim3(kThreads), 0, st, x, dy, nbr, m_out, cin, cout,
+            hipLaunchKernelGGL(wgrad_sparse_kernel<true>, dim3(blocks), dim3(kThreads), 0, st, x, dy, src, m_out, cin, cout,
                                (int)p.rows, p.nbi, tiles, units, part, center_first);
         else
-            hipLaunchKernelGGL(wgrad_sparse_kernel<false>, dim3(blocks), dim3(kThreads), 0, st, x, dy, nbr, m_out, cin, cout,
+            hipLaunchKernelGGL(wgrad_sparse_kernel<false>, dim3(blocks), dim3(kThreads), 0, st, x, dy, src, m_out, cin, cout,
                                (int)p.rows, p.nbi, tiles, units, part, center_first);
     }
     SEG3D_CHECK_LAUNCH();
@@ -577,3 +668,58 @@
     const int64_t n = (int64_t)27 * cin * cout;
     return wgrad_chunk_reduce(part, p.chunks, n, n, dw, nullptr, st);
 }
+
+namespace {
+
+int plan_pairs(int64_t m, int cin, int cout) {
+    if (m <= 0) return 0;
+    const bool wide = routes_wide(cin, cout);
+    const int tiles = wide ? ((cout + 127) / 128) * ((cin + 127) / 128) : ((cout + 63) / 64) * ((cin + 63) / 64);
+    const int rows_target = 3072, floor_wg = wide ? 768 : 512;
+    int64_t chunks = m / rows_target;
+    const int64_t need = (floor_wg + 27 * tiles - 1) / (27 * tiles);
+    if (chunks < need) chunks = need;
+    const int64_t cap = (m + 63) / 64;
+    if (chunks > cap) chunks = cap;
+    if (chunks < 1) chunks = 1;
+    return (int)chunks;
+}
+
+}
+
+size_t wgrad_split_sparse_pairs_workspace_bytes(int64_t m_out, int cin, int cout) {
+    return ((size_t)plan_pairs(m_out, cin, cout) * 27 * (size_t)cin * cout + 64) * sizeof(float);
+}
+
+int wgrad_split_sparse_pairs(const void* x, const float* dy, const int32_t* pair_off, const void* pairs, int64_t m_out, int cin,
+                             int cout, void* workspace, size_t workspace_bytes, hipStream_t st, int32_t* chunks_out, bool x_bf16) {
+    if (workspace_bytes < wgrad_split_sparse_pairs_workspace_bytes(m_out, cin, cout) || !workspace) return SEG3D_EINVAL;
+    const int chunks = plan_pairs(m_out, cin, cout);
+    float* part = static_cast<float*>(workspace);
+    const int units = chunks * 27;
+    const PairSource src{nullptr, pair_off, static_cast<const int2*>(pairs)};
+    const int center_first = unit_order();
+    const int xcd_block = center_first >> 8;
+    const int unit_slots = (units + 8 * xcd_block - 1) / (8 * xcd_block) * (8 * xcd_block);
+#define SEG3D_LAUNCH_LIST(KERNEL_, NBI_, TILES_)                                                                                    \
+    hipLaunchKernelGGL((KERNEL_), dim3((unsigned)unit_slots * (unsigned)(TILES_)), dim3(kThreads), 0, st, x, dy, src, m_out, cin, cout, \
+                       0, NBI_, TILES_, units, part, center_first)
+    if (routes_wide(cin, cout)) {
+        const int nbo = (cout + 127) / 128, nbi = (cin + 127) / 128, tiles = nbo * nbi;
+        if (single_buffer()) {
+            if (x_bf16) SEG3D_LAUNCH_LIST((wgrad_sparse_wide_kernel<true, 1, true, true>), nbi, tiles);
+            else SEG3D_LAUNCH_LIST((wgrad_sparse_wide_kernel<false, 1, true, true>), nbi, tiles);
+        } else {
+            if (x_bf16) SEG3D_LAUNCH_LIST((wgrad_sparse_wide_kernel<true, 1, false, true>), nbi, tiles);
+            else SEG3D_LAUNCH_LIST((wgrad_sparse_wide_kernel<false, 1, false, true>), nbi, tiles);
+        }
+    } else {
+        const int nbo = (cout + 63) / 64, nbi = (cin + 63) / 64, tiles = nbo * nbi;
+        if (x_bf16) SEG3D_LAUNCH_LIST((wgrad_sparse_kernel<true, true>), nbi, tiles);
+        else SEG3D_LAUNCH_LIST((wgrad_sparse_kernel<false, true>), nbi, tiles);
+    }
+#undef SEG3D_LAUNCH_LIST
+    SEG3D_CHECK_LAUNCH();
+    if (chunks_out) *chunks_out = chunks;
+    return SEG3D_OK;
+}
diff --git a/openseg3d_amd/ops.py b/openseg3d_amd/ops.py
--- a/openseg3d_amd/ops.py
+++ b/openseg3d_amd/ops.py
@@ -473,6 +473,35 @@
         _lib.call("seg3d_conv_plan_build", _ptr(coords), _ptr(nbr), m, _ptr(self.data), _ptr(ws), ws_bytes, _stream())
 
 
+WGRAD_PAIRS = os.environ.get("SEG3D_WGRAD_PAIRS", "1") != "0"
+
+
+class PairList:
+
+    HEAD = 128
+
+    def __init__(self, nbr):
+        _need_gpu(nbr)
+        if nbr.dim() != 2 or nbr.shape[0] != 27 or nbr.dtype != torch.int32 or not nbr.is_contiguous():
+            raise _lib.Seg3dError("PairList: a contiguous int32 table [27, m] expected")
+        self.nbr, self.m = nbr, nbr.shape[1]
+        nbytes = _lib.query("seg3d_pair_list_bytes", self.m)
+        if nbytes == 0:
+            raise _lib.Seg3dError(f"PairList: {self.m} rows are more than a pair list can index")
+        self.data = torch.empty((nbytes,), dtype=torch.uint8, device=nbr.device)
+        ws_bytes = _lib.query("seg3d_pair_list_workspace_bytes", self.m)
+        ws = _workspace(ws_bytes, nbr.device)
+        _lib.call("seg3d_pair_list_build", _ptr(nbr), self.m, _ptr(self.data), _ptr(ws), ws_bytes, _stream())
+        self.off = self.data[:self.HEAD].view(torch.int32)[:28]
+        self.pairs = self.data[self.HEAD:].view(torch.int32).view(-1, 2)
+
+
+def pair_list(nbr):
+    if not (WGRAD_PAIRS and CONV_PRECISION == "bf16x3" and nbr.is_cuda):
+        return None
+    return PairList(nbr)
+
+
 def _tiled_fits(plan, packed, cin, cout):
     return (plan is not None and CONV_TILED and bool(packed.flags & PACK_SPLIT_BF16) and max(cin, cout) >= CONV_TILED_MIN_C
             and bool(_lib.load().seg3d_spconv_tiled_supported(int(cin), int(cout))))
@@ -753,7 +782,7 @@
 class _SparseConvFn(torch.autograd.Function):
 
     @staticmethod
-    def forward(ctx, x, weight, bias, nbr, nbr_t, t_flags, packed, order, order_t, plan=None, plan_t=None):
+    def forward(ctx, x, weight, bias, nbr, nbr_t, t_flags, packed, order, order_t, plan=None, plan_t=None, pairs=None):
         x = _f32c(x)
         cout, cin = weight.shape[0], weight.shape[-1]
         if packed is None:
@@ -762,6 +791,7 @@
         ctx.save_for_backward(_saved_rows(x) if (ctx.needs_input_grad[1] and cin % 16 == 0 and cout % 16 == 0) else x, weight)
         ctx.nbr, ctx.nbr_t, ctx.t_flags, ctx.has_bias, ctx.order_t = nbr, nbr_t, t_flags, bias is not None, order_t
         ctx.plan_t = plan_t
+        ctx.pairs = pairs if (pairs is not None and WGRAD_PAIRS and pairs.nbr is nbr) else None
         ctx.bias_param = bias
         return y
 
@@ -774,9 +804,19 @@
         fk = _WgradFork(dy.device)
         if ctx.needs_input_grad[1]:
             dw = torch.empty_like(weight, dtype=torch.float32)
-            ws_bytes = _lib.query("seg3d_spconv_wgrad_workspace_bytes", dy.shape[0], cin, cout)
+            split = bool(_precision_flag() & PACK_SPLIT_BF16)
+            pl = ctx.pairs if split else None
+            ws_bytes = _lib.query("seg3d_spconv_wgrad_pairs_workspace_bytes" if pl is not None else "seg3d_spconv_wgrad_workspace_bytes",
+                                  dy.shape[0], cin, cout)
             ws = torch.empty((ws_bytes,), dtype=torch.uint8, device=dy.device)
-            if _precision_flag() & PACK_SPLIT_BF16:
+            if pl is not None:
+                chunks = ctypes.c_int32(0)
+                _lib.call("seg3d_spconv_wgrad_partials_pairs_xbf16" if x.dtype == torch.bfloat16 else "seg3d_spconv_wgrad_partials_pairs",
+                          _ptr(x), _ptr(dy), _ptr(pl.off), _ptr(pl.pairs), dy.shape[0], x.shape[0], cin, cout,
+                          _ptr(ws), ws_bytes, ctypes.byref(chunks), fk.fork(ws, dy, x, pl.data))
+                n = 27 * cin * cout
+                fk.add_reduce(ws, chunks.value, n, n, dw.data_ptr(), 0, ws)
+            elif split:
                 chunks = ctypes.c_int32(0)
                 _lib.call("seg3d_spconv_wgrad_partials_xbf16" if x.dtype == torch.bfloat16 else "seg3d_spconv_wgrad_partials",
                           _ptr(x), _ptr(dy), _ptr(ctx.nbr), dy.shape[0], x.shape[0], cin, cout,
@@ -798,12 +838,13 @@
             else:
                 db = dy.sum(0)
         fk.join((weight, dw), (ctx.bias_param, db))
-        return dx, dw, db, None, None, None, None, None, None, None, None
-
-
-def sparse_conv(x, weight, bias, nbr, nbr_t, t_flags, packed=None, order=None, order_t=None, plan=None, plan_t=None):
+        return dx, dw, db, None, None, None, None, None, None, None, None, None
+
+
+def sparse_conv(x, weight, bias, nbr, nbr_t, t_flags, packed=None, order=None, order_t=None, plan=None, plan_t=None,
+                pairs=None):
     _need_gpu(x, weight, nbr)
-    return _SparseConvFn.apply(x, weight, bias, nbr, nbr_t, t_flags, packed, order, order_t, plan, plan_t)
+    return _SparseConvFn.apply(x, weight, bias, nbr, nbr_t, t_flags, packed, order, order_t, plan, plan_t, pairs)
 
 
 def _linear_pack(weight, transpose):
diff --git a/openseg3d_amd/segformer.py b/openseg3d_amd/segformer.py
--- a/openseg3d_amd/segformer.py
+++ b/openseg3d_amd/segformer.py
@@ -175,12 +175,16 @@
             level.subm()
             level.mask_order()
             level.subm_plan()
+            if self.training and torch.is_grad_enabled():
+                level.subm_pairs()
             part = getattr(self, f"swformer_block{k + 1}")[0]
             if part not in level.window_plans:
                 level.window_plans[part] = part.launch_plan(level.coords, level.batch_size, widths[k])
                 launched.append(level.window_plans[part])
             if k < 3:
                 level.parity_order()
+                if self.training and torch.is_grad_enabled():
+                    level.down_pairs()
                 level = level.down()[0]
         if launched:
             SparseWindowPartitionLayer.finish_plans(launched)
diff --git a/openseg3d_amd/spconv.py b/openseg3d_amd/spconv.py
--- a/openseg3d_amd/spconv.py
+++ b/openseg3d_amd/spconv.py
@@ -24,6 +24,8 @@
         self._parity = None
         self._mask_order = None
         self._subm_plan = None
+        self._subm_pairs = False
+        self._down_pairs = False
         self._coarse = None
         self._offsets = False
         self.window_plans = {}
@@ -57,6 +59,17 @@
         if self._subm_plan is None:
             self._subm_plan = ops.ConvPlan(self.coords, self.subm())
         return self._subm_plan
+
+    def subm_pairs(self):
+        if self._subm_pairs is False:
+            self._subm_pairs = ops.pair_list(self.subm()) if self.coords.shape[0] else None
+        return self._subm_pairs
+
+    def down_pairs(self):
+        if self._down_pairs is False:
+            _, fwd, inv = self.down()
+            self._down_pairs = (ops.pair_list(fwd) if fwd.shape[1] else None, ops.pair_list(inv) if inv.shape[1] else None)
+        return self._down_pairs
 
     def mask_order(self):
         if SUBM_ORDER_BUCKET == 0:
@@ -148,16 +161,19 @@
                 self._packed = (key, ops.pack_weight(w, ops.PACK_FWD))
         return self._packed[1]
 
-    def _apply_tables(self, feats, nbr, nbr_t, t_flags, order=None, order_t=None, plan=None, plan_t=None):
+    def _apply_tables(self, feats, nbr, nbr_t, t_flags, order=None, order_t=None, plan=None, plan_t=None, pairs=None):
         if self._pad_in:
             feats = torch.nn.functional.pad(feats, (0, self._pad_in))
             weight = torch.nn.functional.pad(self.weight, (0, self._pad_in))
-            return ops.sparse_conv(feats, weight, self.bias, nbr, nbr_t, t_flags, None, order, order_t, plan, plan_t)
+            return ops.sparse_conv(feats, weight, self.bias, nbr, nbr_t, t_flags, None, order, order_t, plan, plan_t, pairs)
         return ops.sparse_conv(feats, self.weight, self.bias, nbr, nbr_t, t_flags, self._packed_weight(), order, order_t,
-                               plan, plan_t)
+                               plan, plan_t, pairs)
 
     def plans(self, x):
         return None, None
+
+    def pairs(self, x):
+        return None
 
     def tables(self, x):
         raise NotImplementedError
@@ -165,7 +181,8 @@
     def forward(self, x):
         nbr, nbr_t, t_flags, order, order_t, level = self.tables(x)
         plan, plan_t = self.plans(x)
-        return x.on_level(self._apply_tables(x.features, nbr, nbr_t, t_flags, order, order_t, plan, plan_t), level)
+        pairs = self.pairs(x) if (torch.is_grad_enabled() and self.weight.requires_grad) else None
+        return x.on_level(self._apply_tables(x.features, nbr, nbr_t, t_flags, order, order_t, plan, plan_t, pairs), level)
 
     def fusable_with(self, bn, x):
         return (FUSE_EVAL_BN and not torch.is_grad_enabled() and not bn.training and bn.track_running_stats and bn.affine
@@ -202,6 +219,9 @@
         plan = x.level.subm_plan()
         return plan, plan
 
+    def pairs(self, x):
+        return x.level.subm_pairs()
+
 
 class SparseConv3d(_Conv3x3x3):
     def tables(self, x):
@@ -211,6 +231,9 @@
         if self.indice_key is not None:
             x.indice_dict[self.indice_key] = x.level
         return fwd, inv, ops.PACK_T, None, x.level.parity_order(), coarse
+
+    def pairs(self, x):
+        return x.level.down_pairs()[0]
 
 
 class SparseInverseConv3d(_Conv3x3x3):
@@ -225,6 +248,9 @@
         if coarse is not x.level:
             raise RuntimeError("SparseInverseConv3d input does not live on the paired strided conv's output sites")
         return inv, fwd, ops.PACK_T, fine.parity_order(), None, fine
+
+    def pairs(self, x):
+        return x.indice_dict[self.indice_key].down_pairs()[1]
 
 
 class SparseSequential(SparseModule):
diff --git a/openseg3d_amd/spnet.py b/openseg3d_amd/spnet.py
--- a/openseg3d_amd/spnet.py
+++ b/openseg3d_amd/spnet.py
@@ -149,10 +149,14 @@
             level.subm()
             level.mask_order()
             level.subm_plan()
+            if self.training and torch.is_grad_enabled():
+                level.subm_pairs()
             if k >= 2:
                 level.sample_offsets()
             if k < 3:
                 level.parity_order()
+                if self.training and torch.is_grad_enabled():
+                    level.down_pairs()
                 level = level.down()[0]
         return batch_dict
 
```
